# AdhavanT/ATRay

Measured on AMD Instinct MI355X. Metric: Mrays/sec on Dragon.obj 1920x1080 @ 1/2/4/8 GPU; % HBM roofline, higher is better.
Workload: dtype f32

## Files before the change

atray_amd/csrc/capi.cpp:

```cpp
#include <hip/hip_runtime.h>

#include <algorithm>
#include <chrono>
#include <cmath>
#include <cstdio>
#include <cstdlib>
#include <cstring>
#include <type_traits>
#include <fcntl.h>
#include <unistd.h>
#include <cerrno>
#include <memory>
#include <mutex>
#include <new>
#include <string>
#include <thread>
#include <vector>

#include "engine.h"
#include "host_scene.h"
#include "launch.h"
#ifdef ATR_DIAG
#include "../../include/atray_diag.h"
#endif
// ... 112 lines not shown
        std::stable_sort(out.begin(), out.end(), [&](const DBlock& a, const DBlock& b) {
            return (cplan[size_t(a.y0 / 8) * size_t(cw) + size_t(a.x0 / 8)] & kPlanClassMask) >
                   (cplan[size_t(b.y0 / 8) * size_t(cw) + size_t(b.x0 / 8)] & kPlanClassMask);
        });
    }
    for (size_t i = 0; i < out.size(); ++i) out[i].base = int32_t(i);
}

int32_t default_parse_threads() {
    const unsigned hw = std::thread::hardware_concurrency();
    return int32_t(std::max(1u, std::min(16u, hw)));
}
#ifndef ATR_MAX_BATCH_LOG2
#define ATR_MAX_BATCH_LOG2 28
#endif
#ifndef ATR_PATH_SPLIT_DEFAULT
#define ATR_PATH_SPLIT_DEFAULT 0
#endif
atr_tuning default_tuning() {
    atr_tuning t;
    std::memset(&t, 0, sizeof(t));
    t.xcd_chunk = 16;
    t.frame_rotate = 0;
    t.hybrid_a = 2;
    t.hybrid_b = 0;
    t.path_batch_log2 = 28;
    t.cluster_size = kMaxClusterSize;
    t.frame_plan = 1;
    t.path_sort_bits = 5;
    t.path_split = ATR_PATH_SPLIT_DEFAULT;
    return t;
}
constexpr int kSchedPaths = 10;
constexpr int kMaxPathBounces = 64;
constexpr int kQueueSlots = 32;
constexpr size_t kTraceBytes = 64 * 128;

}

struct atr_ctx {
    int device = 0;
    hipStream_t own_stream = nullptr;
    hipStream_t last_stream = nullptr;
    hipEvent_t ev_start = nullptr, ev_stop = nullptr, ev_last = nullptr;
    bool have_render = false;
    int32_t last_ntiles = 0;
    std::vector<DevBuf> scene_bufs;
    DScene* d_scene = nullptr;
    int64_t scene_bytes = 0;
    int32_t max_nodes = 0, max_depth = 0, nmodels = 0, max_inner = 0;
    float scene_box[6] = {0.f, 0.f, 0.f, 1.f, 1.f, 1.f};
    atr_tuning tune = default_tuning();
    int64_t nclusters = 0;
    std::vector<uint8_t> cplan;
    int32_t cplan_w = 0, cplan_h = 0;
    uint32_t cplan_gen = 0;
    static constexpr int kBlockSlots = 24;
    BlockSet blocks[kBlockSlots];
    uint64_t block_use[kBlockSlots] = {};
    uint64_t use_clock = 0;
    int32_t* d_error = nullptr;
    int ncu = 256;
    struct PathWS {
        hipStream_t stream = nullptr;
        DevBuf mem;
        int64_t cap = 0;
        int32_t levels = 0;
        int64_t sort_bins = 0;
        bool live = false;
        hipEvent_t ev = nullptr;
        uint64_t last_use = 0;
    };
    static constexpr size_t kMaxPathWS = 4;
    hipStream_t split_stream[2] = {};
    hipEvent_t split_fork = nullptr, split_join[2] = {};
    uint64_t ws_clock = 0;
    std::vector<PathWS> path_ws;
    void* tring = nullptr;
    hipEvent_t tev[kQueueSlots] = {};
    bool tused[kQueueSlots] = {};
    int tnext = 0;
    bool prog_active = false;
    std::vector<DevBuf> prog_blocks;
    std::vector<hipEvent_t> prog_ev;
    std::vector<int32_t> prog_end;
    std::vector<std::pair<hipStream_t, hipEvent_t>> stream_ev;
    int32_t wave_slots = 0;
    hipStream_t plan_side = nullptr;
    static constexpr int kAdaptSlots = 8;
    unsigned long long* adapt_info = nullptr;
    int adapt_next = 0, adapt_last = -1;
    struct PadSlot {
        DevBuf mem;
        uint64_t gen = 0;
        int32_t rows = 0;
        bool wide = false;
        float eye[kMaxFrameCams][3];
        hipEvent_t built = nullptr;
        hipStream_t built_on = nullptr;
        std::vector<std::pair<hipStream_t, hipEvent_t>> readers;
        uint64_t last_use = 0;
    };
    static constexpr int kPadSlots = 4;
    static constexpr size_t kPadMaxBytes = size_t(256) << 20;
    PadSlot pad_slot[kPadSlots];
    uint64_t pad_clock = 0, scene_gen = 0;
    bool camera_pads = true;
    bool facing_fold = true;
    bool wave_cull = true;
    struct QueryWS {
        DevBuf rays, bins;
        int64_t cap = 0, nbins = 0;
        hipEvent_t ev = nullptr;
        hipStream_t stream = nullptr;
        bool used = false;
    } query_ws;
    struct TexelWS {
        DevBuf mesh, map, aux;
    } tex_ws;
    struct ImageWS {
        DevBuf image, flags;
        hipEvent_t ev = nullptr;
        hipStream_t stream = nullptr;
        bool used = false;
    } img_ws;
    struct DenoiseWS {
        DevBuf color, guides;
        hipEvent_t ev = nullptr;
        hipStream_t stream = nullptr;
        bool used = false;
    } dn_ws;
};

namespace {

void apply_tuning(const atr_ctx* c, RenderParams& P) {
    P.xcd_chunk = c->tune.xcd_chunk;
    P.frame_rotate = 0;
    P.hyb_a = c->tune.hybrid_a;
    P.hyb_b = c->tune.hybrid_b;
    P.wave_cull = c->wave_cull ? 1 : 0;
}

int dev_upload(atr_ctx* c, const void* src, size_t bytes, void** out) {
    DevBuf b;
    b.n = bytes ? bytes : 16;
    HIPCHK(hipMalloc(&b.p, b.n));
    if (bytes) {
        const hipError_t e = hipMemcpy(b.p, src, bytes, hipMemcpyHostToDevice);
        if (e != hipSuccess) {
            (void)hipFree(b.p);
            return -(1000 + int(e));
        }
    }
    c->scene_bufs.push_back(b);
    c->scene_bytes += int64_t(b.n);
    *out = b.p;
    return ATR_OK;
}

int32_t shade_records(const HostMesh& M, std::vector<float>& shade) {
    const int32_t smooth = M.normals.empty() ? 0 : 1;
// ... 439 lines not shown
        Q.live.part = Q.live.group + cells;
        Q.live.ctl = reinterpret_cast<PathLiveCtl*>(lb + live_bytes(ws->cap) - 256);
    }
    const int occ_cam = c->tune.path_camera_occ;
    for (int64_t c0 = cbeg; c0 < cend; c0 += cells) {
        Q.cell0 = int32_t(c0);
        Q.ncells = int32_t(std::min<int64_t>(cells, cend - c0));
        if (live && (e = atr_launch_path_live(Q, s)) != hipSuccess) return e;
        if (bl > 0 && spp > 0) {
            if ((e = reset_path_batch(Q, levels, sort_bits, s)) != hipSuccess) return e;
            if ((e = live ? atr_launch_path_camera_adaptive(Q, c->ncu, s) : atr_launch_path_camera(Q, occ_cam, s)) !=
                hipSuccess)
                return e;
            if ((e = launch_bounce_levels(c, Q, bl, sort_bits, s)) != hipSuccess) return e;
        }
        if ((e = live ? atr_launch_path_resolve_adaptive(Q, s) : atr_launch_path_resolve(Q, s)) != hipSuccess) return e;
    }
    return hipEventRecord(ws->ev, s);
}

constexpr int64_t kSplitMinCells = 1024;
hipError_t launch_paths(atr_ctx* c, const RenderParams& P, hipStream_t s) {
    if (P.nblocks <= 0) return hipSuccess;
    const int64_t per_cell = 64 * std::max<int64_t>(P.cam.samples_per_pixel, 1);
    const int64_t batch = std::max<int64_t>(1, (int64_t(1) << c->tune.path_batch_log2) / per_cell);
    if (!c->tune.path_split || P.nblocks > batch || P.nblocks < kSplitMinCells || P.counters || P.block_cost ||
        P.sample_sum)
        return launch_paths_range(c, P, s, 0, P.nblocks);
    hipError_t e;
    if (!c->split_fork) {
        for (int i = 0; i < 2; ++i) {
            if ((e = hipStreamCreateWithFlags(&c->split_stream[i], hipStreamNonBlocking)) != hipSuccess) return e;
            if ((e = hipEventCreateWithFlags(&c->split_join[i], hipEventDisableTiming)) != hipSuccess) return e;
        }
        if ((e = hipEventCreateWithFlags(&c->split_fork, hipEventDisableTiming)) != hipSuccess) return e;
    }
    if ((e = hipEventRecord(c->split_fork, s)) != hipSuccess) return e;
    const int64_t half = (P.nblocks + 1) / 2;
    hipError_t r = hipSuccess;
    for (int i = 0; i < 2; ++i) {
        hipStream_t a = c->split_stream[i];
        if ((e = hipStreamWaitEvent(a, c->split_fork, 0)) != hipSuccess) return e;
        if (r == hipSuccess) r = launch_paths_range(c, P, a, i ? half : 0, i ? P.nblocks : half);
        if ((e = hipEventRecord(c->split_join[i], a)) != hipSuccess) return e;
        if ((e = hipStreamWaitEvent(s, c->split_join[i], 0)) != hipSuccess) return e;
    }
    return r;
}

hipError_t bind_pads(atr_ctx* c, RenderParams& P, int sched, hipStream_t s, atr_ctx::PadSlot** used) {
    *used = nullptr;
    P.pads = nullptr;
    P.pads_stride = 0;
    if (!c->camera_pads || c->nclusters <= 0 || c->nclusters > int64_t(1) << 30 || !atr_render_reads_pads(P, sched))
        return hipSuccess;
    const int32_t rows = P.nfcam > 0 ? P.nfcam : 1;
    if (rows > kMaxFrameCams) return hipSuccess;
    const int32_t stride = int32_t(c->nclusters);
    const bool wide = P.counters != nullptr;
    const size_t bytes = size_t(rows) * size_t(stride) * sizeof(float2_t) * (wide ? 2 : 1);
    if (bytes > atr_ctx::kPadMaxBytes) return hipSuccess;
    PadEyes eyes;
    std::memset(&eyes, 0, sizeof(eyes));
    for (int32_t f = 0; f < rows; ++f) {
        const atr_vec3& e = P.nfcam > 0 ? P.fcam[f].eye : P.cam.eye;
        eyes.e[f][0] = e.x, eyes.e[f][1] = e.y, eyes.e[f][2] = e.z;
    }
    hipError_t e;
    atr_ctx::PadSlot* sl = nullptr;
    atr_ctx::PadSlot* lru = &c->pad_slot[0];
    for (atr_ctx::PadSlot& q : c->pad_slot) {
        if (q.gen == c->scene_gen && q.rows == rows && q.wide == wide && std::memcmp(q.eye, eyes.e, sizeof(float) * 3 * size_t(rows)) == 0) {
            sl = &q;
            break;
        }
        if (q.last_use < lru->last_use) lru = &q;
    }
    if (sl) {
        if (sl->built_on != s && (e = hipStreamWaitEvent(s, sl->built, 0)) != hipSuccess) return e;
    } else {
        sl = lru;
        if (!sl->built && (e = hipEventCreateWithFlags(&sl->built, hipEventDisableTiming)) != hipSuccess) return e;
        if (sl->mem.n < bytes || !sl->mem.p) {
            if (sl->mem.p) {
                if ((e = wait_list(sl->readers)) != hipSuccess) return e;
                if ((e = hipEventSynchronize(sl->built)) != hipSuccess) return e;
                (void)hipFree(sl->mem.p);
            }
            sl->mem = DevBuf();
            sl->gen = 0;
            if (hipMalloc(&sl->mem.p, bytes) != hipSuccess) {
                (void)hipGetLastError();
                sl->mem = DevBuf();
                return hipSuccess;
            }
            sl->mem.n = bytes;
        } else {
            if (sl->gen && sl->built_on != s && (e = hipStreamWaitEvent(s, sl->built, 0)) != hipSuccess) return e;
            for (const auto& se : sl->readers)
                if (se.first != s && (e = hipStreamWaitEvent(s, se.second, 0)) != hipSuccess) return e;
        }
        sl->gen = 0;
        if ((e = atr_launch_camera_pads(c->d_scene, eyes, rows, stride, c->facing_fold, wide, static_cast<float2_t*>(sl->mem.p),
                                        nullptr, nullptr, nullptr, s)) != hipSuccess)
            return e;
        if ((e = hipEventRecord(sl->built, s)) != hipSuccess) return e;
        sl->built_on = s;
        sl->gen = c->scene_gen;
        sl->rows = rows;
        sl->wide = wide;
        std::memcpy(sl->eye, eyes.e, sizeof(eyes.e));
    }
    sl->last_use = ++c->pad_clock;
    P.pads = static_cast<const float2_t*>(sl->mem.p);
    P.pads_stride = stride;
    *used = sl;
    return hipSuccess;
}

hipError_t launch_kernels(atr_ctx* c, RenderParams& P, int sched, hipStream_t s, const PathLive* live = nullptr) {
    if (live) return launch_paths_range(c, P, s, 0, P.nblocks, live);
    if (sched == kSchedPaths) {
        hipError_t e = launch_paths(c, P, s);
        if (e != hipErrorOutOfMemory) return e;
        if (P.traced_rays && (e = hipMemsetAsync(P.traced_rays, 0, kTraceBytes, s)) != hipSuccess) return e;
        sched = sched_of(ATR_KERNEL_FLAT);
    }
    atr_ctx::PadSlot* pads = nullptr;
    hipError_t e = bind_pads(c, P, sched, s, &pads);
    if (e != hipSuccess) return e;
    e = atr_launch_render(P, sched, c->tune.primary_occ, s);
    if (e == hipSuccess && pads) e = note_stream(pads->readers, s);
    return e;
}

hipError_t launch_render(atr_ctx* c, RenderParams& P, int sched, hipStream_t s, hipEvent_t* done,
                         const PathLive* live) {
    if (done) *done = nullptr;
    if (!P.traced_rays) return launch_kernels(c, P, sched, s, live);
    int k = -1;
    unsigned long long* caller = P.traced_rays;
    hipError_t e = ring_take(c, s, k, P.traced_rays);
    if (e != hipSuccess) return e;
    e = launch_kernels(c, P, sched, s, live);
    if (e == hipSuccess) e = atr_launch_traced_finish(P.traced_rays, caller, s);
    P.traced_rays = caller;
    if (e != hipSuccess) return e;
    if ((e = ring_done(c, s, k)) != hipSuccess) return e;
    if (done) *done = c->tev[k];
    return hipSuccess;
}

}

#define ATR_ABI_CATCH                                    \
    catch (const std::bad_alloc&) { return ATR_E_NOMEM; } \
    catch (...) { return ATR_E_INVALID; }

extern "C" {

const char* atr_version(void) { return "atray-mi355x 0.2 (gfx950)"; }

int atr_mesh_parse_obj_threaded(const char* text, size_t len, int32_t threads, atr_mesh** out) try {
    if (!text || !out || threads < 0) return ATR_E_INVALID;
    if (threads == 0) threads = default_parse_threads();
    std::unique_ptr<atr_mesh> own(new (std::nothrow) atr_mesh());
    atr_mesh* m = own.get();
    if (!m) return ATR_E_NOMEM;
// ... 193 lines not shown
    put_le(d + 48, 0x000000FFu, 4);
    put_le(d + 52, 0, 4);
    std::string path;
    int fd = -1;
    for (uint32_t id = 0; id < 100 && fd < 0; ++id) {
        path = std::string(name) + "_" + std::to_string(id) + ".bmp";
        fd = ::open(path.c_str(), O_WRONLY | O_CREAT | O_EXCL, 0644);
        if (fd < 0 && errno != EEXIST) return ATR_E_IO;
    }
    if (fd < 0) return ATR_E_IO;
    bool ok = ::write(fd, hdr, sizeof(hdr)) == ssize_t(sizeof(hdr));
    const uint8_t* src = reinterpret_cast<const uint8_t*>(pixels);
    for (uint64_t off = 0; ok && off < bytes;) {
        const ssize_t w = ::write(fd, src + off, size_t(std::min<uint64_t>(bytes - off, 1ull << 30)));
        ok = w > 0;
        off += ok ? uint64_t(w) : 0;
    }
    ok = (::close(fd) == 0) && ok;
    if (!ok) return ATR_E_IO;
    if (out_path && out_cap > 0) {
        std::strncpy(out_path, path.c_str(), size_t(out_cap) - 1);
        out_path[out_cap - 1] = 0;
    }
    return ATR_OK;
} ATR_ABI_CATCH

int32_t atr_make_tiles(int32_t w, int32_t h, int32_t threads, atr_tile* out, int32_t cap) try {
    return reference_tiles(w, h, threads, out, out ? cap : 0);
} ATR_ABI_CATCH

int32_t atr_make_shard_tiles(int32_t w, int32_t h, int32_t side, int32_t rank, int32_t world, atr_tile* out,
                             int32_t cap) try {
    return shard_tiles(w, h, side, rank, world, out, out ? cap : 0);
} ATR_ABI_CATCH

int32_t atr_balance_shard_tiles(int32_t w, int32_t h, int32_t side, int32_t world, const int64_t* costs,
                                int64_t rank0_extra, int32_t* owner_out) try {
    return balance_shard_tiles(w, h, side, world, costs, rank0_extra, owner_out);
} ATR_ABI_CATCH

int atr_create(int device, atr_ctx** out) try {
    if (!out) return ATR_E_INVALID;
    int n = 0;
    HIPCHK(hipGetDeviceCount(&n));
    if (device < 0 || device >= n) return ATR_E_INVALID;
    HIPCHK(hipSetDevice(device));
    atr_ctx* c = new (std::nothrow) atr_ctx();
    if (!c) return ATR_E_NOMEM;
    struct Owner { atr_ctx* c; ~Owner() { if (c) atr_destroy(c); } } own{c};
    c->device = device;
    if (const char* v = std::getenv("ATR_CAMERA_PADS")) c->camera_pads = !(v[0] == '0' && v[1] == '\0');
    if (const char* v = std::getenv("ATR_WAVE_CULL")) c->wave_cull = !(v[0] == '0' && v[1] == '\0');
    if (const char* v = std::getenv("ATR_FACING_FOLD")) c->facing_fold = !(v[0] == '0' && v[1] == '\0');
    const int rc = [&]() -> int {
        HIPCHK(hipStreamCreateWithFlags(&c->own_stream, hipStreamNonBlocking));
        HIPCHK(hipEventCreate(&c->ev_start));
        HIPCHK(hipEventCreate(&c->ev_stop));
        HIPCHK(hipMalloc(&c->d_error, 16));
        HIPCHK(hipMemset(c->d_error, 0, 16));
        HIPCHK(hipDeviceGetAttribute(&c->ncu, hipDeviceAttributeMultiprocessorCount, device));
        HIPCHK(hipMalloc(&c->tring, kQueueSlots * kTraceBytes));
        HIPCHK(hipMemset(c->tring, 0, kQueueSlots * kTraceBytes));
        for (hipEvent_t& e : c->tev) HIPCHK(hipEventCreate(&e));
        return ATR_OK;
    }();
    if (rc != ATR_OK) return rc;
    own.c = nullptr;
    *out = c;
    return ATR_OK;
} ATR_ABI_CATCH

void atr_default_tuning(atr_tuning* out) {
    if (out) *out = default_tuning();
}

int atr_set_tuning(atr_ctx* c, const atr_tuning* t) try {
    if (!c || !t) return ATR_E_INVALID;
    if (t->xcd_chunk < 0 || t->xcd_chunk > 4096 || t->frame_rotate < 0 || t->frame_rotate > 1024 ||
        t->hybrid_a < -4096 || t->hybrid_a > 4096 || t->hybrid_b < -4096 || t->hybrid_b > 4096 ||
        t->path_batch_log2 < 12 || t->path_batch_log2 > ATR_MAX_BATCH_LOG2 || t->cluster_size < 1 || t->cluster_size > kMaxClusterSize ||
        t->frame_plan < 0 || t->frame_plan > 1 || (t->path_camera_occ != 0 && (t->path_camera_occ < 5 || t->path_camera_occ > 7)) ||
        (t->path_bounce_occ != 0 && (t->path_bounce_occ < 5 || t->path_bounce_occ > 7)) ||
        (t->primary_occ != 0 && (t->primary_occ < 6 || t->primary_occ > 8)) ||
        (t->path_sort_bits != 0 && (t->path_sort_bits < 2 || t->path_sort_bits > kMaxSortBits)) ||
        t->path_split < 0 || t->path_split > 1)
        return ATR_E_INVALID;
    for (int32_t r : t->reserved)
        if (r != 0) return ATR_E_INVALID;
    c->tune = *t;
    return ATR_OK;
} ATR_ABI_CATCH

int atr_get_tuning(atr_ctx* c, atr_tuning* out) try {
    if (!c || !out) return ATR_E_INVALID;
    *out = c->tune;
    return ATR_OK;
} ATR_ABI_CATCH

int atr_destroy(atr_ctx* c) try {
    if (!c) return ATR_E_INVALID;
    (void)hipSetDevice(c->device);
    (void)hipDeviceSynchronize();
    free_scene(c);
    for (BlockSet& b : c->blocks) {
        if (b.dev.p) (void)hipFree(b.dev.p);
        if (b.dev_tiles.p) (void)hipFree(b.dev_tiles.p);
// ... 43 lines not shown
    delete c;
    return ATR_OK;
} ATR_ABI_CATCH

int atr_scene_upload(atr_ctx* c, const atr_material* mats, int32_t nmats, const atr_model* models,
                     int32_t nmodels, const atr_sphere* spheres, int32_t nspheres, const atr_plane* planes,
                     int32_t nplanes) try {
    if (!c || !mats || nmats <= 0 || nmats > kMaxMaterials || nmodels < 0 || nmodels > kMaxModels ||
        (nmodels && !models) || nspheres < 0 || nplanes < 0 || (nspheres && !spheres) || (nplanes && !planes))
        return ATR_E_INVALID;
    for (int32_t i = 0; i < nspheres; ++i)
        if (spheres[i].material < 0 || spheres[i].material >= nmats) return ATR_E_INVALID;
    for (int32_t i = 0; i < nplanes; ++i)
        if (planes[i].material < 0 || planes[i].material >= nmats) return ATR_E_INVALID;
    for (int32_t i = 0; i < nmodels; ++i) {
        const atr_model& md = models[i];
        if (!md.mesh || md.material < 0 || md.material >= nmats) return ATR_E_INVALID;
        if (md.tree) {
            for (int32_t d : md.tree->t.depth)
                if (d >= kMaskLevels) return ATR_E_TREE_DEPTH;
        }
    }
    std::vector<PackedTree> packed(size_t(nmodels), PackedTree{});
    int64_t total_clusters = 0;
    for (int32_t i = 0; i < nmodels; ++i) {
        const atr_model& md = models[i];
        if (md.tree) {
            if (const int rc = pack_tree(md.tree->t, c->tune.cluster_size, packed[size_t(i)])) return rc;
            total_clusters += int64_t(packed[size_t(i)].nclusters);
            if (total_clusters > int64_t(UINT32_MAX)) return ATR_E_INVALID;
        } else {
            const HostMesh& M = md.mesh->m;
            for (int32_t vi : M.face_v)
                if (vi < 0 || size_t(vi) >= M.vertices.size()) return ATR_E_INVALID;
        }
    }
    HIPCHK(hipSetDevice(c->device));
    HIPCHK(wait_all(c));
    free_scene(c);
    ++c->scene_gen;
    DScene S;
    std::memset(&S, 0, sizeof(S));
    for (int32_t i = 0; i < nmats; ++i) {
        const atr_material& m = mats[i];
        S.mats[i] = DMaterial{m.emission.x, m.emission.y, m.emission.z, m.reflection.x, m.reflection.y,
                              m.reflection.z, m.scatter, 0.f};
    }
    S.nmats = nmats;
    S.nmodels = nmodels;
    c->max_nodes = 0;
    c->max_depth = 0;
    c->max_inner = 0;
    c->nclusters = 0;
    float box[6] = {INFINITY, INFINITY, INFINITY, -INFINITY, -INFINITY, -INFINITY};
    for (int32_t i = 0; i < nmodels; ++i)
        for (const V3& v : models[i].mesh->m.vertices) {
            box[0] = std::min(box[0], v.x), box[1] = std::min(box[1], v.y), box[2] = std::min(box[2], v.z);
            box[3] = std::max(box[3], v.x), box[4] = std::max(box[4], v.y), box[5] = std::max(box[5], v.z);
        }
    for (int32_t i = 0; i < nspheres; ++i) {
        const atr_sphere& sp = spheres[i];
        const float r = std::fabs(sp.radius);
        box[0] = std::min(box[0], sp.center.x - r), box[1] = std::min(box[1], sp.center.y - r);
        box[2] = std::min(box[2], sp.center.z - r), box[3] = std::max(box[3], sp.center.x + r);
        box[4] = std::max(box[4], sp.center.y + r), box[5] = std::max(box[5], sp.center.z + r);
    }
    const float unit[6] = {0.f, 0.f, 0.f, 1.f, 1.f, 1.f};
    const bool finite = std::isfinite(box[0]) && std::isfinite(box[1]) && std::isfinite(box[2]) &&
                        std::isfinite(box[3]) && std::isfinite(box[4]) && std::isfinite(box[5]);
    std::memcpy(c->scene_box, finite && box[0] <= box[3] && box[1] <= box[4] && box[2] <= box[5] ? box : unit,
                sizeof(box));
    for (int32_t i = 0; i < nmodels; ++i) {
        const atr_model& md = models[i];
        const HostMesh& M = md.mesh->m;
        DModel& dm = S.models[i];
        std::memset(&dm, 0, sizeof(dm));
        const size_t nf = M.nfaces();
        dm.nfaces = uint32_t(nf);
        dm.material = md.material;
        std::memcpy(dm.aabb, md.surrounding_aabb, sizeof(dm.aabb));
        std::vector<float> shade;
        dm.smooth = shade_records(M, shade);
        void* p = nullptr;
        int rc = dev_upload(c, shade.data(), shade.size() * sizeof(float), &p);
        if (rc) return rc;
        dm.shade = static_cast<const float*>(p);
        if (md.tree) {
            const HostTree& T = md.tree->t;
            PackedTree PT = std::move(packed[size_t(i)]);
            c->max_depth = std::max(c->max_depth, PT.max_depth);
            auto up = [&](const auto& v, auto*& dst) {
                void* q = nullptr;
                const int r = dev_upload(c, v.data(), v.size() * sizeof(v[0]), &q);
                dst = static_cast<std::remove_reference_t<decltype(dst)>>(q);
                return r;
            };
            dm.ninner = PT.ninner;
            if (dm.ninner > c->max_inner) c->max_inner = dm.ninner;
            if ((rc = up(PT.inner, dm.inner)) || (rc = up(PT.t0, dm.t0)) || (rc = up(PT.t1, dm.t1)) ||
                (rc = up(PT.t2, dm.t2)) || (rc = up(PT.tface, dm.tface)))
                return rc;
            const float4_t* clus = nullptr;
            if ((rc = up(PT.clus, clus))) return rc;
            dm.clus = clus;
            dm.cnrm = reinterpret_cast<const uint4_t*>(dm.clus + 2);
            if ((rc = up(PT.cl_range, dm.cl_range)) || (rc = up(PT.prim, dm.prim))) return rc;
            if (c->nclusters + int64_t(PT.nclusters) > int64_t(UINT32_MAX)) return ATR_E_INVALID;
            dm.cl_base = uint32_t(c->nclusters);
            dm.cl_count = uint32_t(PT.nclusters);
            c->nclusters += int64_t(PT.nclusters);
            if ((rc = up(PT.nodes, dm.nodes)) || (rc = up(PT.leaf_range, dm.leaf_range))) return rc;
            if (PT.tris.empty()) PT.tris.resize(1);
            if ((rc = up(PT.tris, dm.tris))) return rc;
            dm.has_tree = 1;
            dm.root_leaf = T.children[0] == 0;
            dm.near_ok = PT.near_ok;
            if (T.nnodes > c->max_nodes) c->max_nodes = T.nnodes;
        } else {
            std::vector<DTri> tris(nf);
            for (size_t f = 0; f < nf; ++f) {
                float v[9];
                for (int k = 0; k < 3; ++k) {
                    const int32_t vi = M.face_v[3 * f + size_t(k)];
                    if (vi < 0 || size_t(vi) >= M.vertices.size()) return ATR_E_INVALID;
                    const V3 q = M.vertices[size_t(vi)];
                    v[3 * k] = q.x; v[3 * k + 1] = q.y; v[3 * k + 2] = q.z;
                }
                tris[f] = make_tri(v, uint32_t(f));
            }
            if ((rc = dev_upload(c, tris.data(), tris.size() * sizeof(DTri), &p))) return rc;
            dm.tris = static_cast<const DTri*>(p);
            dm.has_tree = 0;
        }
    }
    {
        std::vector<DSphere> sp(size_t(nspheres) + 1);
        for (int32_t i = 0; i < nspheres; ++i)
            sp[size_t(i)] = DSphere{spheres[i].center.x, spheres[i].center.y, spheres[i].center.z,
                                    spheres[i].radius, spheres[i].material, 0, 0, 0};
        std::vector<DPlane> pl(size_t(nplanes) + 1);
        for (int32_t i = 0; i < nplanes; ++i)
            pl[size_t(i)] = DPlane{planes[i].normal.x, planes[i].normal.y, planes[i].normal.z,
                                   planes[i].distance, planes[i].material, 0, 0, 0};
        void* p = nullptr;
        int rc;
        if ((rc = dev_upload(c, sp.data(), sp.size() * sizeof(DSphere), &p))) return rc;
        S.spheres = static_cast<const DSphere*>(p);
        if ((rc = dev_upload(c, pl.data(), pl.size() * sizeof(DPlane), &p))) return rc;
        S.planes = static_cast<const DPlane*>(p);
        S.nspheres = nspheres;
        S.nplanes = nplanes;
        if ((rc = dev_upload(c, &S, sizeof(S), &p))) return rc;
        c->d_scene = static_cast<DScene*>(p);
    }
    c->nmodels = nmodels;
    return ATR_OK;
} ATR_ABI_CATCH

int atr_scene_info(atr_ctx* c, int64_t* bytes, int32_t* max_nodes, int32_t* max_depth) try {
    if (!c) return ATR_E_INVALID;
    if (bytes) *bytes = c->scene_bytes;
    if (max_nodes) *max_nodes = c->max_nodes;
// ... 650 lines not shown
    return ATR_OK;
}
}

int atr_render_start_frames(atr_ctx* c, const atr_camera* cam, const atr_tile* tiles, int32_t ntiles,
                            const atr_frame* fr, int32_t nframes, int64_t frame_stride, uint64_t seed, void* stream,
                            int32_t variant) try {
    return start_frames(c, cam, 1, tiles, ntiles, fr, nframes, frame_stride, seed, stream, variant);
} ATR_ABI_CATCH

int atr_render_start_cameras(atr_ctx* c, const atr_camera* cams, int32_t nframes, const atr_tile* tiles,
                             int32_t ntiles, const atr_frame* fr, int64_t frame_stride, uint64_t seed, void* stream,
                             int32_t variant) try {
    return start_frames(c, cams, nframes, tiles, ntiles, fr, nframes, frame_stride, seed, stream, variant);
} ATR_ABI_CATCH

#ifdef ATR_DIAG
int atr_render_wave_trace(atr_ctx* c, const atr_camera* cam, const atr_tile* tiles, int32_t ntiles,
                          uint64_t seed, int32_t variant, uint64_t* out, int64_t cap, int64_t* nblocks) try {
    if (!c || !cam || !nblocks || ntiles < 0 || (ntiles && !tiles)) return ATR_E_INVALID;
    if (!c->d_scene) return ATR_E_NOSCENE;
    HIPCHK(hipSetDevice(c->device));
    int rc = ATR_OK;
    BlockSet* bs = get_blocks(c, tiles, ntiles, cam->width, cam->height, rc);
    if (!bs) return rc;
    const size_t nb = bs->host.size();
    *nblocks = int64_t(nb);
    if (!out || cap < int64_t(3 * nb)) return ATR_OK;
    DevTmp fb;
    DevTmp tr;
    HIPCHK(hipMalloc(&fb.p, std::max<size_t>(1, size_t(bs->packed_pixels)) * 4));
    HIPCHK(hipMalloc(&tr.p, std::max<size_t>(1, 3 * nb) * sizeof(unsigned long long)));
    RenderParams P;
    std::memset(&P, 0, sizeof(P));
    P.cam = *cam;
    P.scene = c->d_scene;
    P.seed = seed;
    P.blocks = static_cast<const DBlock*>(bs->dev.p);
    P.nblocks = int32_t(nb);
    P.layout = ATR_LAYOUT_PACKED;
    P.framebuffer = static_cast<uint32_t*>(fb.p);
    P.error_flag = c->d_error;
    P.wave_trace = static_cast<unsigned long long*>(tr.p);
    apply_tuning(c, P);
    const int ts = sched_of(variant);
    HIPCHK(atr_launch_render(P, ts < 0 || ts == kSchedPaths ? 7 : ts, 0, nullptr));
    HIPCHK(hipDeviceSynchronize());
    if (nb) HIPCHK(hipMemcpy(out, tr.p, 3 * nb * sizeof(unsigned long long), hipMemcpyDeviceToHost));
    return ATR_OK;
} ATR_ABI_CATCH

#endif

constexpr int kCounterSlots = 32;
static int count_launch(atr_ctx* c, const atr_camera* cam, const atr_tile* tiles, int32_t ntiles, uint64_t seed,
                        int32_t variant, unsigned long long h[kCounterSlots]) {
    if (!c || !cam || ntiles < 0 || (ntiles && !tiles)) return ATR_E_INVALID;
    if (!c->d_scene) return ATR_E_NOSCENE;
    HIPCHK(hipSetDevice(c->device));
    int rc = ATR_OK;
    BlockSet* bs = get_blocks(c, tiles, ntiles, cam->width, cam->height, rc);
    if (!bs) return rc;
    DevTmp fb;
    DevTmp ctr;
    HIPCHK(hipMalloc(&fb.p, size_t(cam->width) * size_t(cam->height) * 4));
    HIPCHK(hipMalloc(&ctr.p, kCounterSlots * sizeof(unsigned long long)));
    HIPCHK(hipMemset(ctr.p, 0, kCounterSlots * sizeof(unsigned long long)));
    RenderParams P;
    std::memset(&P, 0, sizeof(P));
    P.cam = *cam;
    P.scene = c->d_scene;
    P.seed = seed;
    P.blocks = static_cast<const DBlock*>(bs->dev.p);
    P.nblocks = int32_t(bs->host.size());
    P.layout = ATR_LAYOUT_IMAGE;
    P.framebuffer = static_cast<uint32_t*>(fb.p);
    P.error_flag = c->d_error;
    P.counters = static_cast<unsigned long long*>(ctr.p);
    apply_tuning(c, P);
    const int sc = auto_sched(variant, *cam);
    if (sc < 0) return ATR_E_INVALID;
    HIPCHK(launch_render(c, P, sc, nullptr));
    HIPCHK(hipDeviceSynchronize());
    HIPCHK(hipMemcpy(h, ctr.p, kCounterSlots * sizeof(unsigned long long), hipMemcpyDeviceToHost));
    return ATR_OK;
}

int atr_render_counters(atr_ctx* c, const atr_camera* cam, const atr_tile* tiles, int32_t ntiles,
                        uint64_t seed, int32_t variant, int64_t out[10]) try {
    if (!out) return ATR_E_INVALID;
    unsigned long long h[kCounterSlots];
    const int rc = count_launch(c, cam, tiles, ntiles, seed, variant, h);
    if (rc != ATR_OK) return rc;
    for (int k = 0; k < 10; ++k) out[k] = int64_t(h[k]);
    return ATR_OK;
} ATR_ABI_CATCH

int atr_render_cull_counters(atr_ctx* c, const atr_camera* cam, const atr_tile* tiles, int32_t ntiles,
                             uint64_t seed, int32_t variant, int64_t out[5]) try {
    if (!out) return ATR_E_INVALID;
    unsigned long long h[kCounterSlots];
    const int rc = count_launch(c, cam, tiles, ntiles, seed, variant, h);
    if (rc != ATR_OK) return rc;
    out[4] = int64_t(h[29]);
    out[0] = int64_t(h[27]);
    out[1] = int64_t(h[28]);
    out[2] = int64_t(h[25]);
    out[3] = int64_t(h[26]);
    return ATR_OK;
} ATR_ABI_CATCH

int atr_render_fold_counters(atr_ctx* c, const atr_camera* cam, const atr_tile* tiles, int32_t ntiles,
                             uint64_t seed, int32_t variant, int64_t out[2]) try {
    if (!out) return ATR_E_INVALID;
    unsigned long long h[kCounterSlots];
    const int rc = count_launch(c, cam, tiles, ntiles, seed, variant, h);
    if (rc != ATR_OK) return rc;
    out[0] = int64_t(h[30]);
    out[1] = int64_t(h[31]);
    return ATR_OK;
} ATR_ABI_CATCH

int64_t atr_camera_pads_row(atr_ctx* c, const float eye[3], float* row, float* boxes, float* edges, int64_t cap) try {
    if (!c || !eye || cap < 0) return ATR_E_INVALID;
    if (!c->d_scene) return ATR_E_NOSCENE;
    const int64_t n = c->nclusters;
    if (n <= 0 || n > int64_t(1) << 30) return n <= 0 ? 0 : ATR_E_INVALID;
    if (!row || cap < n) return n;
    HIPCHK(hipSetDevice(c->device));
    PadEyes eyes;
    std::memset(&eyes, 0, sizeof(eyes));
    eyes.e[0][0] = eye[0], eyes.e[0][1] = eye[1], eyes.e[0][2] = eye[2];
    const size_t nn = size_t(n);
    DevTmp d_tab, d_info, d_box, d_edge, d_tab2;
    HIPCHK(hipMalloc(&d_tab.p, nn * sizeof(float2_t)));
    HIPCHK(hipMalloc(&d_info.p, nn * sizeof(float2_t)));
    HIPCHK(hipMalloc(&d_box.p, nn * 3 * sizeof(float4_t)));
    HIPCHK(hipMalloc(&d_edge.p, nn * 96 * sizeof(float)));
    HIPCHK(hipMemset(d_tab.p, 0, nn * sizeof(float2_t)));
    HIPCHK(hipMemset(d_info.p, 0, nn * sizeof(float2_t)));
    HIPCHK(hipMemset(d_box.p, 0, nn * 3 * sizeof(float4_t)));
    HIPCHK(hipMemset(d_edge.p, 0, nn * 96 * sizeof(float)));
    float2_t* const tab = static_cast<float2_t*>(d_tab.p);
    float2_t* const info = static_cast<float2_t*>(d_info.p);
    float4_t* const box = static_cast<float4_t*>(d_box.p);
    float* const edge = static_cast<float*>(d_edge.p);
    if (c->facing_fold) {
        HIPCHK(atr_launch_camera_pads(c->d_scene, eyes, 1, int32_t(n), 1, 0, tab, info, box, edge, nullptr));
    } else {
        HIPCHK(atr_launch_camera_pads(c->d_scene, eyes, 1, int32_t(n), 0, 0, tab, nullptr, nullptr, nullptr, nullptr));
        HIPCHK(hipMalloc(&d_tab2.p, nn * sizeof(float2_t)));
        HIPCHK(atr_launch_camera_pads(c->d_scene, eyes, 1, int32_t(n), 0, 0, static_cast<float2_t*>(d_tab2.p), info, box,
                                      edge, nullptr));
    }
    HIPCHK(hipDeviceSynchronize());
    std::vector<float2_t> h_tab(nn), h_info(nn);
    HIPCHK(hipMemcpy(h_tab.data(), d_tab.p, nn * sizeof(float2_t), hipMemcpyDeviceToHost));
    HIPCHK(hipMemcpy(h_info.data(), d_info.p, nn * sizeof(float2_t), hipMemcpyDeviceToHost));
    for (size_t i = 0; i < nn; ++i) {
        row[4 * i] = h_tab[i].x, row[4 * i + 1] = h_tab[i].y;
        row[4 * i + 2] = h_info[i].x, row[4 * i + 3] = h_info[i].y;
    }
    if (boxes) HIPCHK(hipMemcpy(boxes, d_box.p, nn * 3 * sizeof(float4_t), hipMemcpyDeviceToHost));
    if (edges) HIPCHK(hipMemcpy(edges, d_edge.p, nn * 96 * sizeof(float), hipMemcpyDeviceToHost));
    return n;
} ATR_ABI_CATCH

#ifdef ATR_DIAG
int atr_render_phase_clocks(atr_ctx* c, const atr_camera* cam, const atr_tile* tiles, int32_t ntiles,
                            uint64_t seed, int32_t variant, int64_t out[6]) try {
    if (!out) return ATR_E_INVALID;
    unsigned long long h[kCounterSlots];
    const int rc = count_launch(c, cam, tiles, ntiles, seed, variant, h);
// ... 750 lines not shown
```

atray_amd/csrc/cluster.h:

```cpp
#pragma once
#include "trace.h"

namespace atr {

constexpr float kTau = 3e-3f;
constexpr float kEps = 5.9604645e-8f;
constexpr float kPadRel = 36.0f * kEps, kPadAbs = 12.0f * kEps;

__device__ __forceinline__ void load_prim(const DModel& m, uint32_t k, float4_t& a0, float4_t& a1, float4_t& a2) {
    a0 = m.prim[3 * size_t(k)];
    a1 = m.prim[3 * size_t(k) + 1];
    a2 = m.prim[3 * size_t(k) + 2];
}

typedef _Float16 h2_t __attribute__((ext_vector_type(2)));

#ifndef ATR_EARLY_NRM
#define ATR_EARLY_NRM 13
#endif

struct ScreenRay {
    float ax, ay, az, sd;
    h2_t dxy, dz_lo, dz_hi;
};
// ... 79 lines not shown
    const float fx = fmaxf(fabsf(lo.x - o.x), fabsf(hi.x - o.x));
    const float fy = fmaxf(fabsf(lo.y - o.y), fabsf(hi.y - o.y));
    const float fz = fmaxf(fabsf(lo.z - o.z), fabsf(hi.z - o.z));
    const float W = (__builtin_amdgcn_sqrtf(fx * fx + fy * fy + fz * fz) + 1.0842022e-19f) * 1.0000005f + (ex + ey + ez);
    const float P = lo.w;
    const float gf = W * (P * (kPadRel / (0.9f * delta)) + kPadAbs);
    return fminf(fmaxf(gf, g.y), g.x);
}

__device__ __forceinline__ bool cluster_pads(const Ray& r, const ScreenRay& sr, float4_t lo, float4_t hi, float2_t g,
                                             float best, float& dlo, float& dhi) {
    const float gl = g.x, gt = g.y;
    const float P = lo.w;
    const float x0 = (lo.x - r.o.x) * r.inv.x, x1 = (hi.x - r.o.x) * r.inv.x;
    const float y0 = (lo.y - r.o.y) * r.inv.y, y1 = (hi.y - r.o.y) * r.inv.y;
    const float z0 = (lo.z - r.o.z) * r.inv.z, z1 = (hi.z - r.o.z) * r.inv.z;
    const float nx = fminf(x0, x1), fx1 = fmaxf(x0, x1), ny = fminf(y0, y1), fy1 = fmaxf(y0, y1),
                nz = fminf(z0, z1), fz1 = fmaxf(z0, z1);
    float tn = fmaxf(fmaxf(nx - gl * sr.ax, ny - gl * sr.ay), nz - gl * sr.az);
    float tf = fminf(fminf(fx1 + gl * sr.ax, fy1 + gl * sr.ay), fz1 + gl * sr.az);
    if (tn > tf || tf < 0.f || tn > best) return false;
    tn = fmaxf(fmaxf(nx - gt * sr.ax, ny - gt * sr.ay), nz - gt * sr.az);
    tf = fminf(fminf(fx1 + gt * sr.ax, fy1 + gt * sr.ay), fz1 + gt * sr.az);
    const bool tight = !(tn > tf || tf < 0.f || tn > best);
    const float q = hi.w;
    const float mq = sr.sd * (q * (0.51f + 511.0f * (4.8828125e-4f + 8.0f * kEps))) +
                     q * (16.0f * kEps * 511.0f + 9.5367432e-7f) + 16.0f * kEps * P;
    dlo = kTol - mq;
    dhi = tight ? __builtin_inff() : kTau + mq;
    return true;
}

struct WaveHull {
    float lx, hx, ly, hy, lz, hz;
    bool ok;
};

__device__ __forceinline__ bool cluster_hull_keep(V3 o, const WaveHull& hl, float4_t lo, float4_t hi, float gl) {
    const float ax = lo.x - o.x, bx = hi.x - o.x, ay = lo.y - o.y, by = hi.y - o.y, az = lo.z - o.z, bz = hi.z - o.z;
    const float x0 = ax * hl.lx, x1 = ax * hl.hx, x2 = bx * hl.lx, x3 = bx * hl.hx;
    const float y0 = ay * hl.ly, y1 = ay * hl.hy, y2 = by * hl.ly, y3 = by * hl.hy;
    const float z0 = az * hl.lz, z1 = az * hl.hz, z2 = bz * hl.lz, z3 = bz * hl.hz;
    const float nx = fminf(fminf(x0, x1), fminf(x2, x3)), fx = fmaxf(fmaxf(x0, x1), fmaxf(x2, x3));
    const float ny = fminf(fminf(y0, y1), fminf(y2, y3)), fy = fmaxf(fmaxf(y0, y1), fmaxf(y2, y3));
    const float nz = fminf(fminf(z0, z1), fminf(z2, z3)), fz = fmaxf(fmaxf(z0, z1), fmaxf(z2, z3));
    const float gx = gl * fmaxf(fabsf(hl.lx), fabsf(hl.hx)), gy = gl * fmaxf(fabsf(hl.ly), fabsf(hl.hy)),
                gz = gl * fmaxf(fabsf(hl.lz), fabsf(hl.hz));
    const float tn = fmaxf(fmaxf(nx - gx, ny - gy), nz - gz);
    const float tf = fminf(fminf(fx + gx, fy + gy), fz + gz);
    const bool cull = tn > tf || tf < 0.f;
    return !cull || !(fmaxf(fmaxf(gx, gy), gz) < __builtin_inff());
}

#ifndef ATR_SCREEN_TWO_CMP
__device__ __forceinline__ void screen_band(float blo, float ahi, float& mid, float& half) {
    const float lo = fmaxf(blo, -1600.0f), hi = fminf(ahi, 1600.0f);
    mid = 0.5f * (lo + hi);
    half = 0.5f * (hi - lo) * 1.000001f + (fabsf(mid) + 2048.0f) * 4.7683716e-7f;
}
__device__ __forceinline__ uint32_t screen8(const ScreenRay& sr, float nmid, float half, uint4_t a0, uint4_t a1,
                                            uint4_t z) {
    const uint32_t xy[8] = {a0.x, a0.y, a0.z, a0.w, a1.x, a1.y, a1.z, a1.w};
    const uint32_t zz[4] = {z.x, z.y, z.z, z.w};
    uint32_t gc = 0;
#pragma unroll
    for (int j = 0; j < 8; ++j) {
        const h2_t pxy = __builtin_bit_cast(h2_t, xy[j]), pz = __builtin_bit_cast(h2_t, zz[j / 2]);
        float dz;
        asm("v_dot2_f32_f16 %0, %1, %2, %3" : "=v"(dz) : "v"((j & 1) ? sr.dz_hi : sr.dz_lo), "v"(pz), "v"(nmid));
        const float e = __builtin_amdgcn_fdot2(sr.dxy, pxy, dz, false);
        if (fabsf(e) <= half) gc |= 1u << j;
    }
    return gc;
}
#else
__device__ __forceinline__ uint32_t screen8(const ScreenRay& sr, float blo, float ahi, uint4_t a0, uint4_t a1,
                                            uint4_t z) {
    const uint32_t xy[8] = {a0.x, a0.y, a0.z, a0.w, a1.x, a1.y, a1.z, a1.w};
    const uint32_t zz[4] = {z.x, z.y, z.z, z.w};
    uint32_t gc = 0;
#pragma unroll
    for (int j = 0; j < 8; ++j) {
        const h2_t pxy = __builtin_bit_cast(h2_t, xy[j]), pz = __builtin_bit_cast(h2_t, zz[j / 2]);
        float dz;
        asm("v_dot2_f32_f16 %0, %1, %2, 0" : "=v"(dz) : "v"((j & 1) ? sr.dz_hi : sr.dz_lo), "v"(pz));
        const float e = __builtin_amdgcn_fdot2(sr.dxy, pxy, dz, false);
        if (e > blo && e <= ahi) gc |= 1u << j;
    }
    return gc;
}
#endif

template <bool COUNT>
__device__ __forceinline__ size_t pads_entry(size_t c) { return COUNT ? 2 * c : c; }

template <bool COUNT, bool EARLY = true, bool PADS = false>
__device__ __forceinline__ uint32_t cluster_cands(const Ray& r, const DModel& m, uint32_t c, float4_t lo, float4_t hi,
                                                  float best, Ctr& ct, const float2_t* pads = nullptr) {
    float2_t g;
    if constexpr (PADS) g = pads[pads_entry<COUNT>(c)];
    Ray rr = r;
    asm volatile("" : "+v"(rr.d.x), "+v"(rr.d.y), "+v"(rr.d.z), "+v"(rr.inv.x), "+v"(rr.inv.y), "+v"(rr.inv.z));
    const ScreenRay sr = screen_ray(rr);
    const uint4_t* nb = m.cnrm + kClusterBlock * size_t(c);
    uint4_t e0, e1, ez;
    if constexpr (EARLY) {
        e0 = nb[0], e1 = nb[1], ez = nb[kMaxClusterSize / 4];
    }
    [[maybe_unused]] float2_t gfold;
    if constexpr (PADS && COUNT) gfold = float2_t{pads[pads_entry<COUNT>(c) + 1].x, g.y};
    if constexpr (!PADS) g = cluster_grow(r.o, lo, hi);
    float dlo, dhi;
    if (!cluster_pads(r, sr, lo, hi, g, best, dlo, dhi)) return 0;
    const uint32_t n = (__float_as_uint(lo.w) & 31u) + 1u;
    if constexpr (COUNT) ct.screen += n;
    if constexpr (PADS && COUNT) {
        float fl, fh;
        if (!cluster_pads(r, sr, lo, hi, gfold, best, fl, fh)) { ct.fold_box += 1; ct.fold_screen += n; }
    }
    const uint32_t slots = (2u << (n - 1)) - 1u;
    const float q = hi.w;
    if (!(q >= 1.1754944e-38f)) return slots;
    const float rq = __builtin_amdgcn_rcpf(q);
    const float a = -dlo * rq, b = -dhi * rq;
    const float ahi = a + fabsf(a) * 9.5367432e-7f + 1.1754944e-38f;
    const float blo = b - fabsf(b) * 9.5367432e-7f - 1.1754944e-38f;
    uint32_t cand = 0;
#ifndef ATR_SCREEN_TWO_CMP
    float mid, half;
    screen_band(blo, ahi, mid, half);
    if constexpr (EARLY) {
        cand = screen8(sr, -mid, half, e0, e1, ez);
        if (n > 8) cand |= screen8(sr, -mid, half, nb[2], nb[3], nb[kMaxClusterSize / 4 + 1]) << 8;
    } else {
        for (uint32_t g = 0; g < n; g += 8)
            cand |= screen8(sr, -mid, half, nb[g / 4], nb[g / 4 + 1], nb[kMaxClusterSize / 4 + g / 8]) << g;
    }
#else
    for (uint32_t g = 0; g < n; g += 8)
        cand |= screen8(sr, blo, ahi, nb[g / 4], nb[g / 4 + 1], nb[kMaxClusterSize / 4 + g / 8]) << g;
#endif
    return cand & slots;
}

}
```

atray_amd/csrc/engine.h:

```cpp
#pragma once
#include <math.h>
#include <stdint.h>

#include "../../include/atray.h"

#ifdef __HIPCC__
#include <hip/hip_runtime.h>
#define ATR_HD __host__ __device__ __forceinline__
#else
#define ATR_HD inline
#endif

namespace atr {

struct alignas(16) float4_t { float x, y, z, w; };
struct alignas(16) uint4_t { uint32_t x, y, z, w; };
struct alignas(8) float2_t { float x, y; };
struct alignas(8) uint2_t { uint32_t x, y; };

constexpr float kMaxFloat = 3.402823466e+38F;
constexpr float kInvU32Max = 2.328306437e-10F;
constexpr float kTol = 0.0001f;
constexpr int kMaskLevels = 16;
constexpr int kMaxMaterials = 32;
// ... 33 lines not shown
ATR_HD float rand_bi(uint64_t& state, uint64_t stream) {
    float rd = (float)pcg_next(state, stream) * kInvU32Max;
    return -1.0f + 2.0f * rd;
}
ATR_HD void path_stream(uint64_t seed, int64_t pixel, uint32_t sample, uint64_t& state, uint64_t& stream) {
    uint64_t x = seed ^ (uint64_t)pixel ^ ((uint64_t)sample << 40);
    x += 0x9E3779B97F4A7C15ULL;
    x = (x ^ (x >> 30)) * 0xBF58476D1CE4E5B9ULL;
    x = (x ^ (x >> 27)) * 0x94D049BB133111EBULL;
    state = x ^ (x >> 31);
    stream = ((uint64_t)pixel << 1) | 1ULL;
}

struct alignas(16) DNode {
    float lo_x, lo_y, lo_z, hi_x;
    float hi_y, hi_z;
    int32_t children;
    int32_t parent;
};
static_assert(sizeof(DNode) == 32, "DNode layout");

struct alignas(16) DTri {
    float ax, ay, az, abx;
    float aby, abz, acx, acy;
    float acz;
    uint32_t face;
    float pad0, pad1;
};
static_assert(sizeof(DTri) == 48, "DTri layout");

struct DModel {
    const DNode* nodes;
    const float4_t* inner;
    int32_t ninner;
    const uint32_t* leaf_range;
    const DTri* tris;
    const float4_t* t0;
    const float4_t* t1;
    const float* t2;
    const uint32_t* tface;
    const float4_t* clus;
    const uint32_t* cl_range;
    const uint4_t* cnrm;
    const float4_t* prim;
    const float* shade;
    uint32_t nfaces;
    int32_t has_tree;
    int32_t root_leaf;
    int32_t near_ok;
    int32_t smooth;
    int32_t material;
    float aabb[6];
    uint32_t cl_base, cl_count;
};

struct DMaterial { float ex, ey, ez, rx, ry, rz, scatter, pad; };
struct DSphere { float cx, cy, cz, r; int32_t material, pad0, pad1, pad2; };
struct DPlane { float nx, ny, nz, d; int32_t material, pad0, pad1, pad2; };

struct DScene {
    DMaterial mats[kMaxMaterials];
    DModel models[kMaxModels];
    int32_t nmats, nmodels, nspheres, nplanes;
    const DSphere* spheres;
    const DPlane* planes;
};

struct alignas(16) DBlock {
    int32_t x0, y0;
    uint32_t mask_lo, mask_hi;
    int32_t out_base;
    int32_t flags;
    int32_t base;
    int32_t pad;
};
static_assert(sizeof(DBlock) == 32, "DBlock layout");
constexpr int32_t kBlockPrio = 1;
constexpr int kPlanClassShift = 4;
constexpr uint8_t kPlanClassMask = 0x70, kPlanPrio = 0x80;

struct RenderParams {
    atr_camera cam;
    const DScene* scene;
    uint64_t seed;
    const DBlock* blocks;
    int32_t nblocks;
    int32_t layout;
    uint32_t* framebuffer;
    uint32_t* hit_face;
    float* hit_t;
    float* rgb;
    uint32_t* ray_casts;
    unsigned long long* traced_rays;
    int32_t* error_flag;
    unsigned long long* counters;
    unsigned long long* block_cost;
    unsigned long long* wave_trace;
    int32_t xcd_chunk;
    int32_t frame_blocks;
    int64_t frame_stride;
    int32_t frame_rotate;
    int32_t hyb_a, hyb_b;
    int32_t nfcam;
    atr_camera fcam[kMaxFrameCams];
    uint32_t first_sample;
    float* sample_sum;
    const float2_t* pads;
    int32_t pads_stride;
    int32_t wave_cull;
};

struct PadEyes {
    float e[kMaxFrameCams][3];
};

constexpr int kPathPlanes = 4;
struct PathCtl {
    uint32_t tail;
    uint32_t head;
};
#ifndef ATR_SORT_DIRS
#define ATR_SORT_DIRS 16
#endif
constexpr int kSortDirs = ATR_SORT_DIRS;
constexpr int kMaxSortBits = 7;
constexpr int64_t kSortBinsMax = int64_t(1) << 26;
constexpr int32_t kSortChunk = 4096;
static_assert((kSortDirs * kSortDirs << 6) % kSortChunk == 0, "the fewest bins (2 bits per axis) fill whole scan blocks");
static_assert((kSortBinsMax / kSortChunk) <= 32768, "path_sort_part_scan: one workgroup, 32 sums per lane");
struct PathSort {
    int32_t bits;
    int32_t nbins;
    float lo[3], sc[3];
    uint2_t* kr;
    uint32_t* perm;
    uint32_t* hist;
    uint32_t* start;
    uint32_t* part;
};

constexpr int32_t kLiveChunk = 64;
struct PathLiveCtl {
    uint32_t groups;
    uint32_t claim;
};
struct PathLive {
    uint32_t* count;
    float tolerance;
    uint2_t* mask;
    uint32_t* first;
    uint32_t* group;
    uint32_t* part;
    PathLiveCtl* ctl;
    unsigned long long* info;
};

struct PathParams {
    atr_camera cam;
    const DScene* scene;
    uint64_t seed;
    const DBlock* blocks;
    int32_t frame_blocks;
// ... 164 lines not shown
```

atray_amd/csrc/host_scene.cpp:

```cpp
#include <algorithm>
#include <cmath>
#include <cstdio>
#include <cstring>
#include <new>
#include <string>
#include <utility>
#include <vector>

#include "engine.h"
#include "host_scene.h"
#include "refs_budget.h"

using namespace atr;


void atr::mesh_aabb(const HostMesh& m, float out[6]) {
    float lo[3] = {kMaxFloat, kMaxFloat, kMaxFloat}, hi[3] = {-kMaxFloat, -kMaxFloat, -kMaxFloat};
    for (const V3& v : m.vertices) {
        const float c[3] = {v.x, v.y, v.z};
        for (int a = 0; a < 3; ++a) {
            hi[a] = pl_max(hi[a], c[a]);
            lo[a] = pl_min(lo[a], c[a]);
        }
    }
// ... 412 lines not shown
}

atr::DTri atr::make_tri(const float* v, uint32_t face) {
    DTri t;
    std::memset(&t, 0, sizeof(t));
    const V3 a = mk(v[0], v[1], v[2]), b = mk(v[3], v[4], v[5]), c = mk(v[6], v[7], v[8]);
    const V3 ab = sub(b, a), ac = sub(c, a);
    t.ax = a.x; t.ay = a.y; t.az = a.z;
    t.abx = ab.x; t.aby = ab.y; t.abz = ab.z;
    t.acx = ac.x; t.acy = ac.y; t.acz = ac.z;
    t.face = face;
    return t;
}

int atr::pack_tree(const HostTree& T, int cluster_size, PackedTree& P) {
    P = PackedTree();
    if (T.nnodes <= 0 || T.bounds.size() != 6 * size_t(T.nnodes) || T.children.size() != size_t(T.nnodes) ||
        T.parent.size() != size_t(T.nnodes) || T.depth.size() != size_t(T.nnodes) ||
        T.leaf_first.size() != size_t(T.nnodes) || T.leaf_count.size() != size_t(T.nnodes) ||
        T.prim_vertices.size() != 9 * T.prim_face.size())
        return ATR_E_INVALID;
    const size_t nprims = T.prim_face.size();
    P.nodes.resize(size_t(T.nnodes));
    std::vector<uint32_t> range(2 * size_t(T.nnodes), 0);
    for (int32_t n = 0; n < T.nnodes; ++n) {
        DNode& d = P.nodes[size_t(n)];
        const float* b = &T.bounds[6 * size_t(n)];
        d.lo_x = b[0]; d.lo_y = b[1]; d.lo_z = b[2];
        d.hi_x = b[3]; d.hi_y = b[4]; d.hi_z = b[5];
        d.children = T.children[size_t(n)];
        d.parent = T.parent[size_t(n)];
        if (!T.children[size_t(n)] && uint64_t(T.leaf_first[size_t(n)]) + T.leaf_count[size_t(n)] > nprims)
            return ATR_E_INVALID;
        range[2 * size_t(n)] = T.leaf_first[size_t(n)];
        range[2 * size_t(n) + 1] = T.children[size_t(n)] ? 0u : T.leaf_count[size_t(n)];
        P.max_depth = std::max(P.max_depth, T.depth[size_t(n)]);
    }
    std::vector<int32_t> leaf_rank;
    int rc;
    if ((rc = inner_table(T, P.inner, leaf_rank))) return rc;
    P.ninner = int32_t(P.inner.size() / 3);
    if (P.inner.empty()) P.inner.assign(3, float4_t{0.f, 0.f, 0.f, 0.f});
    auto by_rank = [&](const std::vector<uint32_t>& per_node) {
        std::vector<uint32_t> out(std::max<size_t>(2, per_node.size()), 0u);
        for (int32_t n = 0; n < T.nnodes; ++n) {
            const int32_t k = leaf_rank[size_t(n)];
            if (k < 0) continue;
            out[2 * size_t(k)] = per_node[2 * size_t(n)];
            out[2 * size_t(k) + 1] = per_node[2 * size_t(n) + 1];
        }
        return out;
    };
    P.leaf_range = by_rank(range);
    P.tris.resize(nprims);
    for (size_t k = 0; k < nprims; ++k) P.tris[k] = make_tri(&T.prim_vertices[9 * k], T.prim_face[k]);
    const size_t np = nprims ? nprims : 1;
    P.t0.assign(np, float4_t{0.f, 0.f, 0.f, 0.f});
    P.t1.assign(np, float4_t{0.f, 0.f, 0.f, 0.f});
    P.t2.assign(np, 0.f);
    P.tface.assign(np, 0u);
    for (size_t k = 0; k < nprims; ++k) {
        const DTri& t = P.tris[k];
        P.t0[k] = float4_t{t.ax, t.ay, t.az, t.abx};
        P.t1[k] = float4_t{t.aby, t.abz, t.acx, t.acy};
        P.t2[k] = t.acz;
        P.tface[k] = t.face;
    }
    LeafClusters C;
    if ((rc = leaf_clusters(T, cluster_size, C))) return rc;
    const size_t ncl = C.rec.size() / 8;
    P.nclusters = ncl;
    const size_t ns = std::max<size_t>(1, ncl) * kMaxClusterSize;
    P.prim.assign(3 * ns, float4_t{0.f, 0.f, 0.f, 0.f});
    std::vector<uint32_t> nw(std::max<size_t>(1, ncl) * kNormWords, 0u);
    for (size_t cl = 0; cl < ncl; ++cl) {
        uint32_t pw, first;
        std::memcpy(&pw, &C.rec[8 * cl + 3], 4);
        std::memcpy(&first, &C.rec[8 * cl + 7], 4);
        const uint32_t n = (pw & 31u) + 1u;
        if (n > uint32_t(kMaxClusterSize) || size_t(first) + n > C.order.size()) return ATR_E_INVALID;
        double mx = 0.0;
        for (uint32_t k = first; k < first + n; ++k)
            for (int a = 0; a < 3; ++a) mx = std::max(mx, std::fabs(double(C.normal[3 * size_t(k) + size_t(a)])));
        float q = float(mx / 511.0);
        while (double(q) * 511.0 < mx) q = std::nextafter(q, INFINITY);
        if (!(q > 0.f)) q = 1e-30f;
        C.rec[8 * cl + 7] = q;
        for (uint32_t i = 0; i < n; ++i) {
            const size_t k = first + i, slot = cl * kMaxClusterSize + i;
            if (C.order[k] >= nprims) return ATR_E_INVALID;
            const DTri& t = P.tris[C.order[k]];
            float rk, fc;
            std::memcpy(&rk, &C.rank[k], 4);
            std::memcpy(&fc, &t.face, 4);
            P.prim[3 * slot] = float4_t{t.ax, t.ay, t.az, t.abx};
            P.prim[3 * slot + 1] = float4_t{t.aby, t.abz, t.acx, t.acy};
            P.prim[3 * slot + 2] = float4_t{t.acz, rk, fc, 0.f};
            uint16_t h[3];
            for (int a = 0; a < 3; ++a) {
                const double r = double(C.normal[3 * k + size_t(a)]) / double(q);
                long v = std::isfinite(r) ? std::lround(std::max(-1e6, std::min(1e6, r))) : 0L;
                v = std::max(-511L, std::min(511L, v));
                h[a] = half_of_int(int32_t(v));
            }
            nw[kNormWords * cl + i] = uint32_t(h[0]) | (uint32_t(h[1]) << 16);
            nw[kNormWords * cl + kMaxClusterSize + i / 2] |= uint32_t(h[2]) << (16 * (i & 1));
// ... 13 lines not shown
```

atray_amd/csrc/host_scene.h:

```cpp
#pragma once
#include <cstddef>
#include <cstdint>
#include <vector>

#include "engine.h"

namespace atr {

struct HostMesh {
    std::vector<V3> vertices, normals, texcoords;
    std::vector<int32_t> face_v, face_t, face_n;
    size_t nfaces() const { return face_v.size() / 3; }
};

struct HostTree {
    int32_t nnodes = 0;
    std::vector<float> bounds;
    std::vector<int32_t> children;
    std::vector<int32_t> parent;
    std::vector<int32_t> depth;
    std::vector<uint32_t> leaf_first, leaf_count;
    std::vector<float> prim_vertices;
    std::vector<uint32_t> prim_face;
};

struct LeafClusters {
    std::vector<uint32_t> order;
    std::vector<uint32_t> rank;
    std::vector<float> rec;
    std::vector<float> normal;
    std::vector<uint32_t> range;
    float max_abs = 0.f;
};
int leaf_clusters(const HostTree& T, int size, LeafClusters& C);

int inner_table(const HostTree& T, std::vector<float4_t>& out, std::vector<int32_t>& leaf_rank);

struct PackedTree {
    std::vector<DNode> nodes;
    std::vector<uint32_t> leaf_range;
    std::vector<float4_t> inner;
    int32_t ninner = 0;
    std::vector<DTri> tris;
    std::vector<float4_t> t0, t1;
    std::vector<float> t2;
    std::vector<uint32_t> tface;
    size_t nclusters = 0;
    std::vector<uint32_t> clus;
    std::vector<uint32_t> cl_range;
    std::vector<float4_t> prim;
    int32_t max_depth = 0;
    bool near_ok = false;
};
int pack_tree(const HostTree& T, int cluster_size, PackedTree& P);
DTri make_tri(const float* v9, uint32_t face);

int parse_obj_text(const char* text, size_t len, HostMesh& m, int threads = 1);
void mesh_aabb(const HostMesh& m, float out[6]);
void mesh_translate(HostMesh& m, float box[6], V3 c);
int octree_build(const HostMesh& m, uint32_t max_faces, HostTree& T);
int octree_build_device(const HostMesh& m, uint32_t max_faces, int device, HostTree& T, float* ms_out);
int octree_finish(HostTree& T);
void octree_stats(const HostTree& T, int64_t s[7]);
void camera_set(atr_camera& cm, V3 eye, V3 facing, int32_t w, int32_t h, int32_t aa, uint32_t spp,
                int32_t bounces, float h_fov);
int32_t reference_tiles(int32_t W, int32_t H, int32_t threads, atr_tile* out, int32_t cap);
int32_t balance_shard_tiles(int32_t W, int32_t H, int32_t side, int32_t world, const int64_t* costs,
                            int64_t rank0_extra, int32_t* owner);
int32_t shard_tiles(int32_t W, int32_t H, int32_t side, int32_t rank, int32_t world, atr_tile* out,
                    int32_t cap);

}

struct atr_mesh { atr::HostMesh m; };
struct atr_octree { atr::HostTree t; };
```

atray_amd/csrc/launch.h:

```cpp
#pragma once
#include <hip/hip_runtime.h>

#include "denoise.h"
#include "engine.h"
#include "texels.h"

extern "C" {
hipError_t atr_launch_render(const atr::RenderParams& P, int sched, int primary_occ, hipStream_t s);
int atr_render_reads_pads(const atr::RenderParams& P, int sched);
hipError_t atr_launch_camera_pads(const atr::DScene* scene, const atr::PadEyes& eyes, int32_t nrows, int32_t stride,
                                  int fold, int wide, atr::float2_t* table, atr::float2_t* info, atr::float4_t* boxes,
                                  float* edges, hipStream_t s);
hipError_t atr_launch_traced_finish(unsigned long long* slots, unsigned long long* out, hipStream_t s);
hipError_t atr_launch_unpack(const atr::DBlock* blocks, int32_t nblocks, int32_t width, const uint32_t* packed,
                             uint32_t* image, hipStream_t s);
hipError_t atr_launch_tile_casts(const atr_tile* tiles, int32_t ntiles, int32_t width, const uint32_t* casts,
                                 int64_t* out, hipStream_t s);
hipError_t atr_launch_packed_tile_casts(const int32_t* slot_tile, int64_t nslots, const uint32_t* casts,
                                        int64_t frame_stride, int32_t nframes, int32_t ntiles,
                                        unsigned long long* out, hipStream_t s);
hipError_t atr_launch_path_camera(const atr::PathParams& P, int occ, hipStream_t s);
hipError_t atr_launch_path_bounce(const atr::PathParams& P, int ncu, int occ, hipStream_t s);
hipError_t atr_launch_path_resolve(const atr::PathParams& P, hipStream_t s);
hipError_t atr_launch_path_sort(const atr::PathParams& P, int ncu, hipStream_t s);
hipError_t atr_launch_path_live(const atr::PathParams& P, hipStream_t s);
hipError_t atr_launch_path_camera_adaptive(const atr::PathParams& P, int ncu, hipStream_t s);
hipError_t atr_launch_path_resolve_adaptive(const atr::PathParams& P, hipStream_t s);
hipError_t atr_launch_sort_bins(const atr::PathSort& so, hipStream_t s);
hipError_t atr_launch_query_sort(const atr::QueryParams& P, int ncu, hipStream_t s);
hipError_t atr_launch_query(const atr::QueryParams& P, int lane, int ncu, hipStream_t s);
hipError_t atr_launch_occlusion(const atr::OcclParams& P, int lane, int ncu, hipStream_t s);
hipError_t atr_launch_gather(const atr::GatherParams& P, int lane, int ncu, hipStream_t s);
hipError_t atr_launch_radiance_entry(const atr::RadianceParams& P, int ncu, hipStream_t s);
hipError_t atr_launch_radiance_resolve(const atr::RadianceParams& P, hipStream_t s);
hipError_t atr_launch_gather_radiance_entry(const atr::GatherRadianceParams& P, int ncu, hipStream_t s);
hipError_t atr_launch_gather_radiance_resolve(const atr::GatherRadianceParams& P, hipStream_t s);
hipError_t atr_launch_texel_classify(const atr::TexelParams& P, hipStream_t s);
hipError_t atr_launch_texel_big(const atr::TexelParams& P, uint32_t nbig, hipStream_t s);
hipError_t atr_launch_texel_scan(const atr::TexelParams& P, hipStream_t s);
hipError_t atr_launch_texel_write(const atr::TexelParams& P, hipStream_t s);
hipError_t atr_launch_texel_scatter(const float* values, const int32_t* texel, int64_t n, int64_t ntexels, float* image,
                                    uint8_t* flag, hipStream_t s);
hipError_t atr_launch_texel_dilate(const atr::TexelImageParams& P, hipStream_t s);
hipError_t atr_launch_texel_fill(const atr::TexelImageParams& P, hipStream_t s);
hipError_t atr_launch_denoise_pack(const atr::DenoisePack& P, hipStream_t s);
hipError_t atr_launch_denoise_pass(const atr::DenoisePass& P, int normal, int position, int colour, hipStream_t s);
hipError_t atr_launch_plan(const atr::DBlock* base, int32_t nb, unsigned long long* cost,
                           unsigned long long* cost_last, void* work, atr::DBlock* out, int32_t max_split,
                           float split2, float split4, hipStream_t s);
size_t atr_plan_work_bytes(int32_t nb);
hipError_t atr_launch_pack_bgr(const uint32_t* src, int64_t n, uint8_t* dst, hipStream_t s);
int64_t atr_masked_chunks(int64_t n);
int atr_unpack_max_sources();
hipError_t atr_launch_unpack_masked_multi(int32_t n, const atr::DBlock* const* blocks, const int32_t* nblocks,
                                          const int64_t* own, const uint8_t* const* in, const int32_t* raw,
                                          int32_t width, int32_t nframes, uint32_t* image, int64_t image_stride,
                                          hipStream_t s);
hipError_t atr_launch_unpack_masked(const atr::DBlock* blocks, int32_t nblocks, int32_t width, const uint8_t* in,
                                    int32_t nframes, int64_t own, uint32_t* image, int64_t image_stride,
                                    hipStream_t s);
hipError_t atr_launch_pack_bgr_masked(const uint32_t* src, int64_t n, uint32_t bg, uint8_t* out, int64_t* nbytes,
                                      hipStream_t s);
hipError_t atr_launch_scatter_bgr_masked(const uint8_t* in, int64_t n, const int64_t* dst_index, uint32_t* image,
                                         hipStream_t s);
hipError_t atr_launch_scatter_bgr(const uint8_t* src, int64_t n, const int64_t* dst_index, uint32_t* image,
// ... 3 lines not shown
```

atray_amd/csrc/render.hip:

```cpp
#include <hip/hip_runtime.h>

#include "launch.h"
#include "scan.h"

namespace atr {

constexpr bool sched_stash(int sc) { return sc == SCHED_FLAT || sc == SCHED_HYBRID; }

constexpr int kStash = 16;

template <int SCHED, bool COUNT>
__device__ __forceinline__ V3 cast_ray(const DScene* __restrict__ S, V3 o, V3 d, int32_t bounce_limit,
                                       bool active, uint64_t& st, uint64_t stream, uint32_t& casts,
                                       uint32_t& traced, bool record, uint32_t& hit_face, float& hit_t,
                                       int& err, Ctr& ct, int32_t hyb_a, int32_t hyb_b, V3& acc) {
    constexpr bool STASH = sched_stash(SCHED);
    constexpr bool PRIV = SCHED == SCHED_FLAT;
    __shared__ uint32_t s_stash[STASH && !PRIV ? 4 : 1][PRIV ? 1 : kStash][64];
    uint32_t pstash[PRIV ? kStash : 1];
    uint32_t* const L = &s_stash[(STASH && !PRIV) ? threadIdx.x >> 6 : 0][0][threadIdx.x & 63];
#define stash_put(k, v) do { if constexpr (PRIV) pstash[k] = (v); else L[64 * (k)] = (v); } while (0)
#define stash_get(k) (PRIV ? pstash[(PRIV ? (k) : 0)] : L[64 * (k)])
    V3 ret = mk(0.f, 0.f, 0.f), w = mk(1.f, 1.f, 1.f);
    int32_t i = 0;
// ... 61 lines not shown

template <int SCHED, bool COUNT, bool PRIMARY, int OCC = 4, bool ACCUM = false, bool PADS = false>
__global__ __launch_bounds__(256, OCC) void render_kernel(RenderParams P) {
    static_assert(!ACCUM || (SCHED == SCHED_FLAT && !PRIMARY && !COUNT), "sample passes run on FLAT");
    static_assert(!PADS || (SCHED == SCHED_HYBRID && PRIMARY), "the table serves HYBRID's primary flavour");
    const int wave = __builtin_amdgcn_readfirstlane(int(threadIdx.x >> 6)), lane = threadIdx.x & 63;
    const int b = remap_xcd(blockIdx.x, gridDim.x, P.xcd_chunk) * 4 + wave;
    if (b >= P.nblocks) return;
    const int32_t nf = P.frame_blocks > 0 ? P.nblocks / P.frame_blocks : 1;
    const int32_t fidx = b % nf;
    int32_t bi = b / nf;
    if (P.frame_rotate && nf > 1)
        bi = int32_t((int64_t(bi) + int64_t(P.frame_blocks) * fidx * P.frame_rotate / (1024 * int64_t(nf))) %
                     P.frame_blocks);
    const DBlock blk = P.blocks[bi];
    const uint64_t mask = uint64_t(blk.mask_lo) | (uint64_t(blk.mask_hi) << 32);
    const bool active = (mask >> lane) & 1;
    const int32_t x = blk.x0 + (lane & 7), y = blk.y0 + (lane >> 3);
    if (__builtin_amdgcn_readfirstlane(blk.flags) & kBlockPrio) __builtin_amdgcn_s_setprio(2);
    const uint64_t clk0 = P.block_cost ? clock64() : 0;
    uint64_t clk1 = 0;
    if constexpr (COUNT) clk1 = clock64();
#ifdef ATR_DIAG
    const uint64_t rt0 = P.wave_trace ? __builtin_amdgcn_s_memrealtime() : 0;
#endif
    const atr_camera& cm = P.nfcam > 0 ? P.fcam[__builtin_amdgcn_readfirstlane(fidx)] : P.cam;
    const DScene* S = uniform_global(P.scene);
    int err = 0;
    Ctr ct;
    uint32_t casts = 0, traced = 0, hit_face = 0xFFFFFFFFu;
    float hit_t = kMaxFloat;
    V3 col = mk(0.f, 0.f, 0.f);
    const int64_t pix = int64_t(y) * cm.width + x;
    if constexpr (ACCUM) {
        if (active && P.first_sample > 0) {
            size_t o;
            if (P.layout == ATR_LAYOUT_PACKED) o = size_t(blk.out_base) + __popcll(mask & ((uint64_t(1) << lane) - 1));
            else o = size_t(y) * size_t(cm.width) + size_t(x);
            col = mk(P.sample_sum[3 * o], P.sample_sum[3 * o + 1], P.sample_sum[3 * o + 2]);
            if (P.ray_casts) casts = P.ray_casts[o];
        }
    }
    const float film_y = -1.0f + 2.0f * (float(y) / float(cm.height));
    const float film_x = ((-1.0f + 2.0f * (float(x) / float(cm.width))) * cm.h_fov) * cm.aspect_ratio;
    const V3 eye = from(cm.eye), fc = from(cm.frame_center), cx = from(cm.camera_x), cy = from(cm.camera_y);
    V3 dir = mk(0.f, 0.f, 1.f);
    if (!cm.anti_aliasing) dir = unit(sub(add(add(fc, scale(cx, film_x)), scale(cy, film_y)), eye));
    if constexpr (PRIMARY) {
        Isect id;
        id.type = T_NONE;
        if constexpr (PADS) {
            const int32_t row = P.nfcam > 0 ? __builtin_amdgcn_readfirstlane(fidx) : 0;
            const float2_t* pads = uniform_global(P.pads) + pads_entry<COUNT>(size_t(int64_t(row) * P.pads_stride));
            intersect_scene<SCHED, FlavPrimaryPads, COUNT>(S, eye, dir, active, id, err, ct, P.hyb_a, P.hyb_b, pads,
                                                           P.wave_cull);
        } else {
            intersect_scene<SCHED, FlavPrimary, COUNT>(S, eye, dir, active, id, err, ct, P.hyb_a, P.hyb_b, nullptr,
                                                       P.wave_cull);
        }
        if (active) {
            const DMaterial& mat = S->mats[id.material];
            col = add(col, mk(mat.ex, mat.ey, mat.ez));
            hit_face = id.face;
            hit_t = id.t;
            casts = id.type == T_SKY ? 0u : 1u;
            traced = 1;
        }
    } else {
        for (uint32_t s = 0; s < cm.samples_per_pixel; ++s) {
            uint64_t st, stream;
            uint32_t fs = s;
            if constexpr (ACCUM) fs += P.first_sample;
            path_stream(P.seed, pix, fs, st, stream);
            if (cm.anti_aliasing) {
                const float xo = rand_bi(st, stream) * cm.half_pixel_width + film_x;
                const float yo = rand_bi(st, stream) * cm.half_pixel_height + film_y;
                dir = unit(sub(add(add(fc, scale(cx, xo)), scale(cy, yo)), eye));
            }
            col = add(col, cast_ray<SCHED, COUNT>(S, eye, dir, cm.bounce_limit, active, st, stream, casts, traced,
                                                 fs == 0, hit_face, hit_t, err, ct, P.hyb_a, P.hyb_b, col));
        }
    }
    DBlock ob = blk;
    __asm__ volatile("" ::: "memory");
    ob = P.blocks[bi];
    int olane = int(threadIdx.x);
    __asm__ volatile("" : "+v"(olane));
    olane &= 63;
    const uint64_t omask = uint64_t(ob.mask_lo) | (uint64_t(ob.mask_hi) << 32);
    if ((omask >> olane) & 1) {
        [[maybe_unused]] const V3 sum = col;
        if constexpr (ACCUM) col = divs(col, float(P.first_sample + cm.samples_per_pixel));
        else col = divs(col, float(cm.samples_per_pixel));
        const float cr = pl_max(0.0f, pl_min(col.x, 1.0f));
        const float cg = pl_max(0.0f, pl_min(col.y, 1.0f));
        const float cb = pl_max(0.0f, pl_min(col.z, 1.0f));
        const uint32_t r8 = uint32_t(cr * 255.0f) & 0xFFu, g8 = uint32_t(cg * 255.0f) & 0xFFu,
                       b8 = uint32_t(cb * 255.0f) & 0xFFu;
        size_t o;
        if (P.layout == ATR_LAYOUT_PACKED) o = size_t(ob.out_base) + __popcll(omask & ((uint64_t(1) << olane) - 1));
        else o = size_t(ob.y0 + (olane >> 3)) * size_t(cm.width) + size_t(ob.x0 + (olane & 7));
        o += size_t(fidx) * size_t(P.frame_stride);
        P.framebuffer[o] = b8 | (g8 << 8) | (r8 << 16);
        if (!ACCUM || P.first_sample == 0) {
            if (P.hit_face) P.hit_face[o] = hit_face;
            if (P.hit_t) P.hit_t[o] = hit_t;
        }
        if constexpr (ACCUM) { P.sample_sum[3 * o] = sum.x; P.sample_sum[3 * o + 1] = sum.y; P.sample_sum[3 * o + 2] = sum.z; }
// ... 19 lines not shown
#pragma unroll
        for (int k = 0; k < 6; ++k) {
            uint32_t t = v[k];
#pragma unroll
            for (int off = 32; off > 0; off >>= 1) t += __shfl_xor(t, off);
            if (lane == 0 && t) atomicAdd(C + 1 + k, (unsigned long long)t);
        }
        uint32_t t = traced;
#pragma unroll
        for (int off = 32; off > 0; off >>= 1) t += __shfl_xor(t, off);
        if (lane == 0) { atomicAdd(C + 0, (unsigned long long)t); atomicAdd(C + 7, 1ull); }
        uint32_t w[2] = {ct.cbox, ct.screen};
#pragma unroll
        for (int k = 0; k < 2; ++k) {
            uint32_t x2 = w[k];
#pragma unroll
            for (int off = 32; off > 0; off >>= 1) x2 += __shfl_xor(x2, off);
            if (lane == 0 && x2) atomicAdd(C + 8 + k, (unsigned long long)x2);
        }
#pragma unroll
        for (int k = 0; k < 3; ++k) {
            uint32_t a = ct.steps[k], q = ct.active[k];
#pragma unroll
            for (int off = 32; off > 0; off >>= 1) { a += __shfl_xor(a, off); q += __shfl_xor(q, off); }
            if (lane == 0 && a) atomicAdd(C + 16 + k, (unsigned long long)a);
            if (lane == 0 && q) atomicAdd(C + 19 + k, (unsigned long long)q);
        }
        {
            uint32_t e[5] = {ct.cand_wave, ct.node_wave, ct.node_lane, ct.round_wave, ct.round_items};
#pragma unroll
            for (int k = 0; k < 5; ++k) {
                uint32_t x2 = e[k];
#pragma unroll
                for (int off = 32; off > 0; off >>= 1) x2 += __shfl_xor(x2, off);
                if (lane == 0 && x2) atomicAdd(C + 22 + k, (unsigned long long)x2);
            }
        }
        if constexpr (SCHED == SCHED_HYBRID && PRIMARY) {
            if (lane == 0 && ct.culled) atomicAdd(C + 27, (unsigned long long)ct.culled);
            if (lane == 0 && ct.lp_wave) atomicAdd(C + 28, (unsigned long long)ct.lp_wave);
            uint32_t x2 = ct.ctest;
#pragma unroll
            for (int off = 32; off > 0; off >>= 1) x2 += __shfl_xor(x2, off);
            if (lane == 0 && x2) atomicAdd(C + 29, (unsigned long long)x2);
        }
        if constexpr (PADS) {
            uint32_t f[2] = {ct.fold_box, ct.fold_screen};
#pragma unroll
            for (int k = 0; k < 2; ++k) {
                uint32_t x2 = f[k];
#pragma unroll
                for (int off = 32; off > 0; off >>= 1) x2 += __shfl_xor(x2, off);
                if (lane == 0 && x2) atomicAdd(C + 30 + k, (unsigned long long)x2);
            }
        }
        if (lane == 0) {
            atomicAdd(C + 10, (unsigned long long)ct.t_pass);
            atomicAdd(C + 11, (unsigned long long)ct.t_lp);
            atomicAdd(C + 12, (unsigned long long)ct.t_deal);
            atomicAdd(C + 13, (unsigned long long)(clock64() - clk1));
            atomicAdd(C + 14, (unsigned long long)ct.t_prep);
            atomicAdd(C + 15, (unsigned long long)ct.t_scan);
        }
    }
}

template __global__ void render_kernel<SCHED_LANE, false, false>(RenderParams);
template __global__ void render_kernel<SCHED_LANE, true, false>(RenderParams);
template __global__ void render_kernel<SCHED_LANE, true, true>(RenderParams);
template __global__ void render_kernel<SCHED_LANE, false, true, 5>(RenderParams);
template __global__ void render_kernel<SCHED_HYBRID, false, true, 6>(RenderParams);
template __global__ void render_kernel<SCHED_HYBRID, false, true, 7>(RenderParams);
template __global__ void render_kernel<SCHED_HYBRID, false, true, 8>(RenderParams);
template __global__ void render_kernel<SCHED_HYBRID, false, false>(RenderParams);
template __global__ void render_kernel<SCHED_HYBRID, true, true>(RenderParams);
template __global__ void render_kernel<SCHED_HYBRID, true, false>(RenderParams);
template __global__ void render_kernel<SCHED_FLAT, false, false, 6>(RenderParams);
template __global__ void render_kernel<SCHED_FLAT, false, false, 7>(RenderParams);
template __global__ void render_kernel<SCHED_FLAT, true, false>(RenderParams);
template __global__ void render_kernel<SCHED_FLAT, false, false, 6, true>(RenderParams);
template __global__ void render_kernel<SCHED_HYBRID, false, true, 6, false, true>(RenderParams);
template __global__ void render_kernel<SCHED_HYBRID, false, true, 7, false, true>(RenderParams);
template __global__ void render_kernel<SCHED_HYBRID, false, true, 8, false, true>(RenderParams);
template __global__ void render_kernel<SCHED_HYBRID, true, true, 4, false, true>(RenderParams);

template <bool WIDE>
__global__ __launch_bounds__(256) void camera_pads_kernel(const DScene* __restrict__ S, PadEyes eyes, int32_t stride,
                                                          float2_t* __restrict__ table) {
    const uint32_t x = blockIdx.x * 256u + threadIdx.x;
    if (x >= uint32_t(stride)) return;
    const int32_t f = __builtin_amdgcn_readfirstlane(int32_t(blockIdx.y));
    const V3 eye = mk(eyes.e[f][0], eyes.e[f][1], eyes.e[f][2]);
    const int32_t nmodels = S->nmodels;
    for (int32_t i = 0; i < nmodels; ++i) {
        const DModel& m = S->models[i];
        const uint32_t c = x - m.cl_base;
        if (!m.has_tree || c >= m.cl_count) continue;
        const float2_t g = cluster_grow(eye, m.clus[kClusterBlock * size_t(c)], m.clus[kClusterBlock * size_t(c) + 1]);
        const size_t e = size_t(f) * size_t(stride) + x;
        if constexpr (WIDE) {
            table[2 * e] = g;
            table[2 * e + 1] = float2_t{g.x, kTol};
        } else {
            table[e] = g;
        }
        return;
// ... 8 lines not shown
    static_assert(kMaxClusterSize == 16, "sixteen lanes per cluster");
    const uint32_t x = blockIdx.x * 16u + (threadIdx.x >> 4), j = threadIdx.x & 15u;
    if (x >= uint32_t(stride)) return;
    const int32_t nmodels = S->nmodels;
    for (int32_t i = 0; i < nmodels; ++i) {
        const DModel& m = S->models[i];
        const uint32_t c = x - m.cl_base;
        if (!m.has_tree || c >= m.cl_count) continue;
        const float4_t lo = m.clus[kClusterBlock * size_t(c)], hi = m.clus[kClusterBlock * size_t(c) + 1];
        const uint32_t n = (__float_as_uint(lo.w) & 31u) + 1u;
        const bool have = j < n;
        float4_t a0 = {0.f, 0.f, 0.f, 0.f}, a1 = a0, a2 = a0;
        if (have) load_prim(m, kMaxClusterSize * c + j, a0, a1, a2);
        for (int32_t f = 0; f < nrows; ++f) {
            const V3 eye = mk(eyes.e[f][0], eyes.e[f][1], eyes.e[f][2]);
            const float2_t g = cluster_grow(eye, lo, hi);
            const FoldBox b = fold_box(eye, lo, hi, g.x);
            double lower = double(__builtin_inff());
            bool rej = false;
            if (have) {
                rej = fold_prim(b, lo.w, a0, a1, a2, lower);
                if (rej) lower = double(__builtin_inff());
            }
            const uint32_t mask = uint32_t(__ballot(rej) >> (threadIdx.x & 48u)) & 0xFFFFu;
#pragma unroll
            for (int off = 8; off > 0; off >>= 1) lower = fmin(lower, __shfl_xor(lower, off));
            const bool folded = fold && b.ok;
            const float delta = folded ? fold_delta(lower) : kTol;
            const float gf = cluster_grow_fold(eye, lo, hi, delta, g);
            if (j == 0) {
                const size_t e = size_t(f) * size_t(stride) + x;
                if constexpr (WIDE) {
                    table[2 * e] = g;
                    table[2 * e + 1] = float2_t{gf, delta};
                } else {
                    table[e] = float2_t{gf, g.y};
                }
                if (info) info[x] = float2_t{delta, __uint_as_float(folded ? mask : 0u)};
                if (boxes) {
                    boxes[3 * size_t(x)] = lo;
                    boxes[3 * size_t(x) + 1] = hi;
                    boxes[3 * size_t(x) + 2] = float4_t{g.x, 0.f, 0.f, 0.f};
                }
            }
        }
        if (edges) {
            float* o = edges + 6 * (size_t(kMaxClusterSize) * x + j);
            o[0] = a0.w, o[1] = a1.x, o[2] = a1.y, o[3] = a1.z, o[4] = a1.w, o[5] = a2.x;
        }
        return;
    }
}

__global__ __launch_bounds__(64) void traced_finish_kernel(unsigned long long* __restrict__ slots,
                                                          unsigned long long* __restrict__ out) {
    const int lane = threadIdx.x;
    unsigned long long v = slots[16 * lane];
    slots[16 * lane] = 0;
#pragma unroll
    for (int off = 32; off > 0; off >>= 1) v += __shfl_xor(v, off);
    if (lane == 0 && v) atomicAdd(out, v);
}

__global__ __launch_bounds__(256) void unpack_kernel(const DBlock* __restrict__ blocks, int32_t nblocks,
                                                     int32_t width, const uint32_t* __restrict__ packed,
                                                     uint32_t* __restrict__ image) {
    const int b = blockIdx.x * 4 + (threadIdx.x >> 6), lane = threadIdx.x & 63;
    if (b >= nblocks) return;
    const DBlock blk = blocks[b];
    const uint64_t mask = uint64_t(blk.mask_lo) | (uint64_t(blk.mask_hi) << 32);
    if (!((mask >> lane) & 1)) return;
    const int32_t x = blk.x0 + (lane & 7), y = blk.y0 + (lane >> 3);
    image[size_t(y) * width + x] = packed[size_t(blk.out_base) + __popcll(mask & ((uint64_t(1) << lane) - 1))];
}

__global__ __launch_bounds__(256) void tile_casts_kernel(const atr_tile* __restrict__ tiles, int32_t width,
                                                         const uint32_t* __restrict__ casts,
                                                         int64_t* __restrict__ out) {
    const atr_tile t = tiles[blockIdx.x];
    const int32_t tw = t.max_x - t.min_x + 1, th = t.max_y - t.min_y + 1;
    int64_t acc = 0;
    for (int32_t i = threadIdx.x; i < tw * th; i += blockDim.x) {
        const int32_t x = t.min_x + i % tw, y = t.min_y + i / tw;
        acc += casts[size_t(y) * width + x];
    }
    __shared__ int64_t red[256];
    red[threadIdx.x] = acc;
    __syncthreads();
    for (int s = 128; s > 0; s >>= 1) {
        if (int(threadIdx.x) < s) red[threadIdx.x] += red[threadIdx.x + s];
        __syncthreads();
    }
    if (threadIdx.x == 0) out[blockIdx.x] = red[0];
}

__global__ __launch_bounds__(256) void packed_tile_casts_kernel(const int32_t* __restrict__ slot_tile,
                                                                int64_t nslots,
                                                                const uint32_t* __restrict__ casts,
                                                                int64_t frame_stride, int32_t ntiles,
                                                                unsigned long long* __restrict__ out) {
    const int64_t i = int64_t(blockIdx.x) * 256 + threadIdx.x;
    const int64_t f = blockIdx.y;
    int32_t t = -1;
    unsigned long long v = 0;
    if (i < nslots) {
        t = slot_tile[i];
// ... 4 lines not shown
#pragma unroll
        for (int off = 32; off > 0; off >>= 1) v += __shfl_xor(v, off);
        if ((threadIdx.x & 63) == 0 && t0 >= 0 && v) atomicAdd(&out[f * ntiles + t0], v);
    } else if (t >= 0 && v) {
        atomicAdd(&out[f * ntiles + t], v);
    }
}

}

template <int SC, bool C, bool PR, int OCC = 4, bool ACCUM = false, bool PADS = false>
static void launch_one(const atr::RenderParams& P, hipStream_t s) {
    const int grid = (P.nblocks + 3) / 4;
    hipLaunchKernelGGL((atr::render_kernel<SC, C, PR, OCC, ACCUM, PADS>), dim3(grid), dim3(256), 0, s, P);
}

static void launch_hybrid_primary(const atr::RenderParams& P, int occ, hipStream_t s) {
    using namespace atr;
    if (P.pads) {
        if (occ == 0) launch_one<SCHED_HYBRID, true, true, 4, false, true>(P, s);
        else if (occ == 8) launch_one<SCHED_HYBRID, false, true, 8, false, true>(P, s);
        else if (occ == 7) launch_one<SCHED_HYBRID, false, true, 7, false, true>(P, s);
        else launch_one<SCHED_HYBRID, false, true, 6, false, true>(P, s);
    } else {
        if (occ == 0) launch_one<SCHED_HYBRID, true, true>(P, s);
        else if (occ == 8) launch_one<SCHED_HYBRID, false, true, 8>(P, s);
        else if (occ == 7) launch_one<SCHED_HYBRID, false, true, 7>(P, s);
        else launch_one<SCHED_HYBRID, false, true, 6>(P, s);
    }
}

extern "C" int atr_render_reads_pads(const atr::RenderParams& P, int sched) {
    using namespace atr;
    const bool prim = P.cam.bounce_limit == 1 && !P.cam.anti_aliasing && P.cam.samples_per_pixel == 1;
    return prim && !P.sample_sum && (sched == SCHED_HYBRID || sched == SCHED_FLAT);
}

extern "C" hipError_t atr_launch_camera_pads(const atr::DScene* scene, const atr::PadEyes& eyes, int32_t nrows,
                                             int32_t stride, int fold, int wide, atr::float2_t* table,
                                             atr::float2_t* info, atr::float4_t* boxes, float* edges, hipStream_t s) {
    using namespace atr;
    if (nrows <= 0 || stride <= 0) return hipSuccess;
    if (nrows > kMaxFrameCams) return hipErrorInvalidValue;
    const bool side = info || boxes || edges;
    if (side && nrows != 1) return hipErrorInvalidValue;
    const dim3 gf(unsigned((stride + 15) / 16)), gp(unsigned((stride + 255) / 256), unsigned(nrows));
    if (fold || side) {
        if (wide) hipLaunchKernelGGL(camera_fold_kernel<true>, gf, dim3(256), 0, s, scene, eyes, nrows, stride, fold, table, info, boxes, edges);
        else hipLaunchKernelGGL(camera_fold_kernel<false>, gf, dim3(256), 0, s, scene, eyes, nrows, stride, fold, table, info, boxes, edges);
    } else {
        if (wide) hipLaunchKernelGGL(camera_pads_kernel<true>, gp, dim3(256), 0, s, scene, eyes, stride, table);
        else hipLaunchKernelGGL(camera_pads_kernel<false>, gp, dim3(256), 0, s, scene, eyes, stride, table);
    }
    return hipGetLastError();
}

extern "C" hipError_t atr_launch_render(const atr::RenderParams& P, int sched, int primary_occ, hipStream_t s) {
    using namespace atr;
    if (P.nblocks <= 0) return hipSuccess;
    if (P.traced_rays && P.counters) return hipErrorInvalidValue;
    const bool count = P.counters != nullptr;
    const bool prim = P.cam.bounce_limit == 1 && !P.cam.anti_aliasing && P.cam.samples_per_pixel == 1;
    const bool multi = P.frame_blocks > 0;
    if (P.sample_sum) {
        if (sched != SCHED_FLAT || count || multi) return hipErrorInvalidValue;
        launch_one<SCHED_FLAT, false, false, 6, true>(P, s);
        return hipGetLastError();
    }
    const int occ = primary_occ ? primary_occ : (multi ? 7 : 8);
    const bool prim7 = occ == 7;
    const bool prim8 = occ == 8;
    switch (sched) {
        case SCHED_HYBRID:
            if (count) { if (prim) launch_hybrid_primary(P, 0, s); else launch_one<SCHED_HYBRID, true, false>(P, s); }
            else if (!prim) launch_one<SCHED_HYBRID, false, false>(P, s);
            else launch_hybrid_primary(P, prim8 ? 8 : prim7 ? 7 : 6, s);
            break;
        case SCHED_FLAT:
            if (prim && !count) launch_hybrid_primary(P, 6, s);
            else if (count) { if (prim) launch_hybrid_primary(P, 0, s); else launch_one<SCHED_FLAT, true, false>(P, s); }
            else if (multi) launch_one<SCHED_FLAT, false, false, 7>(P, s);
            else launch_one<SCHED_FLAT, false, false, 6>(P, s);
            break;
        case SCHED_LANE:
            if (count) { if (prim) launch_one<SCHED_LANE, true, true>(P, s); else launch_one<SCHED_LANE, true, false>(P, s); }
            else if (prim) launch_one<SCHED_LANE, false, true, 5>(P, s);
            else launch_one<SCHED_LANE, false, false>(P, s);
            break;
        default:
            return hipErrorInvalidValue;
    }
    return hipGetLastError();
}

extern "C" hipError_t atr_launch_traced_finish(unsigned long long* slots, unsigned long long* out, hipStream_t s) {
    hipLaunchKernelGGL(atr::traced_finish_kernel, dim3(1), dim3(64), 0, s, slots, out);
    return hipGetLastError();
}

extern "C" hipError_t atr_launch_unpack(const atr::DBlock* blocks, int32_t nblocks, int32_t width,
                                        const uint32_t* packed, uint32_t* image, hipStream_t s) {
    const int grid = (nblocks + 3) / 4;
    if (grid <= 0) return hipSuccess;
    hipLaunchKernelGGL(atr::unpack_kernel, dim3(grid), dim3(256), 0, s, blocks, nblocks, width, packed, image);
    return hipGetLastError();
}
// ... 18 lines not shown
```

atray_amd/csrc/scan.h:

```cpp
#pragma once
#include <hip/hip_runtime.h>

#include "cluster.h"
#include "shade.h"
#include "trace.h"

namespace atr {

struct TriRegs { float4_t q0, q1; float q2; };

__device__ __forceinline__ void tri_fetch(const DModel& m, uint32_t i, TriRegs& t) {
    t.q0 = m.t0[i];
    t.q1 = m.t1[i];
    t.q2 = m.t2[i];
}

__device__ __forceinline__ void tri_test(const Ray& r, const TriRegs& t, uint32_t slot, float& best_t,
                                         uint32_t& best_slot, float& bu, float& bv, bool& improved) {
    float u = 0.f, v = 0.f;
    const float dist = tri_hit(r, mk(t.q0.x, t.q0.y, t.q0.z), mk(t.q0.w, t.q1.x, t.q1.y),
                               mk(t.q1.z, t.q1.w, t.q2), u, v);
    if (dist < best_t && dist > kTol) {
        best_t = dist;
        best_slot = slot;
// ... 125 lines not shown
    const float v = ln == 0 ? hl.lx : ln == 1 ? hl.hx : ln == 2 ? hl.ly : ln == 3 ? hl.hy : ln == 4 ? hl.lz : hl.hz;
    return hl.ok || ln != 0 ? v : __builtin_nanf("");
}
__device__ __forceinline__ WaveHull hull_unpack(float hv) {
    auto at = [&](int k) { return __int_as_float(__builtin_amdgcn_readlane(__float_as_int(hv), k)); };
    WaveHull hl;
    hl.lx = at(0); hl.hx = at(1); hl.ly = at(2); hl.hy = at(3); hl.lz = at(4); hl.hz = at(5);
    hl.ok = hl.lx == hl.lx;
    return hl;
}

__device__ __forceinline__ uint32_t nth_set_bit(uint32_t x, uint32_t j) {
    uint32_t b = 0, n;
    n = uint32_t(__popc(x & 0xFFFFu)); if (j >= n) { j -= n; x >>= 16; b += 16; }
    n = uint32_t(__popc(x & 0xFFu)); if (j >= n) { j -= n; x >>= 8; b += 8; }
    n = uint32_t(__popc(x & 0xFu)); if (j >= n) { j -= n; x >>= 4; b += 4; }
    n = uint32_t(__popc(x & 0x3u)); if (j >= n) { j -= n; x >>= 2; b += 2; }
    return b + (j >= (x & 1u) ? 1u : 0u);
}

#ifdef ATR_PHASE_CLOCKS
#define ATR_PCLK(...) __VA_ARGS__
#else
#define ATR_PCLK(...)
#endif

template <bool UV>
struct FlatUV {
    float u[4][64], v[4][64];
};
template <>
struct FlatUV<false> {};
template <int K = kLeafBuf, bool UV = true>
struct FlatLds : FlatUV<UV> {
    float lbd[4][K][64];
    int32_t lbl[4][K][64];
    unsigned long long key[4][64];
    uint32_t slot[4][64];
    int32_t mark[4][64];
};
template <int K = kLeafBuf, bool UV = true>
__device__ __forceinline__ FlatLds<K, UV>& flat_lds() {
    __shared__ FlatLds<K, UV> L;
    return L;
}

constexpr unsigned long long kKeyInit = (static_cast<unsigned long long>(0x7F7FFFFFu) << 32) | 0xFFFFFFFFull;

#ifndef ATR_BOUNCE_HYB
#define ATR_BOUNCE_HYB 0
#endif

struct FlavCamera      { static constexpr bool HYB = true,  LDSB = true,  UO = true,  UT = true,  UV = true,
                         NEAR = false, PADS = false, WCULL = false, SEED = false; static constexpr int EARLY = 2; };
struct FlavPrimary     { static constexpr bool HYB = true,  LDSB = true,  UO = true,  UT = true,  UV = false,
                         NEAR = false, PADS = false, WCULL = true,  SEED = false; static constexpr int EARLY = 1; };
struct FlavPrimaryPads { static constexpr bool HYB = true,  LDSB = true,  UO = true,  UT = true,  UV = false,
                         NEAR = false, PADS = true,  WCULL = true,  SEED = false; static constexpr int EARLY = 8; };
struct FlavHybBounce   { static constexpr bool HYB = true,  LDSB = false, UO = false, UT = false, UV = true,
                         NEAR = false, PADS = false, WCULL = false, SEED = false; static constexpr int EARLY = 4; };
struct FlavBounce      { static constexpr bool HYB = ATR_BOUNCE_HYB != 0, LDSB = true, UO = false, UT = false,
                         UV = true, NEAR = true, PADS = false, WCULL = false, SEED = false;
                         static constexpr int EARLY = 4; };
struct FlavOcclusion   { static constexpr bool HYB = false, LDSB = true,  UO = false, UT = false, UV = false,
                         NEAR = true,  PADS = false, WCULL = false, SEED = true;  static constexpr int EARLY = 1; };

template <class F, bool COUNT, int K = kLeafBuf>
__device__ __forceinline__ bool cand_test(const Ray& q, const DModel& m, int w, int32_t ow, uint32_t slot,
                                          unsigned long long& mine, float& u, float& v, Ctr& ct) {
    FlatLds<K, F::UV>& L = flat_lds<K, F::UV>();
    if constexpr (COUNT) ct.tri += 1;
    float4_t a0, a1, a2;
    load_prim(m, slot, a0, a1, a2);
    const float dist = tri_hit(q, mk(a0.x, a0.y, a0.z), mk(a0.w, a1.x, a1.y), mk(a1.z, a1.w, a2.x), u, v);
    if (dist > kTol && dist < kMaxFloat) {
        mine = (static_cast<unsigned long long>(__float_as_uint(dist)) << 32) | uint32_t(__float_as_int(a2.y));
        if (mine < L.key[w][ow]) {
            atomicMin(&L.key[w][ow], mine);
            return true;
        }
    }
    return false;
}

template <class F, bool COUNT, bool SELF, int K = kLeafBuf>
__device__ __forceinline__ void cand_rounds(const Ray& r, const DModel& m, int w, int ln, uint32_t cm,
                                            uint32_t cfirst, int32_t own, Ctr& ct) {
    FlatLds<K, F::UV>& L = flat_lds<K, F::UV>();
    const uint32_t cc = uint32_t(__popc(cm));
    constexpr bool kInPlace = SELF;
#ifndef ATR_INPLACE_FACTOR
#define ATR_INPLACE_FACTOR 2
#endif
    uint32_t cinc = 0, total = 0, most;
    bool inplace;
    if (kInPlace && __ballot(cc > 1u) == 0) {
        most = __ballot(cc != 0u) ? 1u : 0u;
        inplace = true;
    } else {
        cinc = wave_incl_add(cc);
        total = uint32_t(__builtin_amdgcn_readlane(int(cinc), 63));
        most = kInPlace ? uint32_t(__builtin_amdgcn_readlane(wave_incl_max(int32_t(cc)), 63)) : 64u;
        inplace = kInPlace && most < ATR_INPLACE_FACTOR * ((total + 63u) >> 6);
    }
    if (inplace) {
        Ray q;
        q.o = r.o;
        q.d = r.d;
        uint32_t x = cm;
        for (uint32_t it = 0; it < most; ++it) {
            const bool valid = x != 0;
            const uint32_t slot = cfirst + (valid ? uint32_t(__builtin_ctz(x)) : 0u);
            x &= x - 1u;
            if constexpr (COUNT) ct.cand_wave += ln == 0 ? 1u : 0u;
            unsigned long long mine = kKeyInit;
            bool imp = false;
            float u = 0.f, v = 0.f;
            if (valid) imp = cand_test<F, COUNT, K>(q, m, w, own, slot, mine, u, v, ct);
// ... 47 lines not shown
            load_prim(m, slot, a0, a1, a2);
            const float dist = tri_hit(q, mk(a0.x, a0.y, a0.z), mk(a0.w, a1.x, a1.y), mk(a1.z, a1.w, a2.x), u, v);
            if (dist > kTol && dist < kMaxFloat) {
                mine = (static_cast<unsigned long long>(__float_as_uint(dist)) << 32) | uint32_t(__float_as_int(a2.y));
                if (mine < L.key[w][ow]) {
                    atomicMin(&L.key[w][ow], mine);
                    imp = true;
                }
            }
        }
        __builtin_amdgcn_wave_barrier();
        if (imp && L.key[w][ow] == mine) {
            L.slot[w][ow] = slot;
            if constexpr (F::UV) {
                L.u[w][ow] = u;
                L.v[w][ow] = v;
            }
        }
        __builtin_amdgcn_wave_barrier();
    }
}


struct FlatQ {
    int32_t j, nb;
    bool done, need, more, rewalk;
};

template <class F, bool COUNT, int K = kLeafBuf>
__device__ __forceinline__ FlatQ flat_begin(const Ray& r, const DModel& m, bool active, int w, int ln, Ctr& ct,
                                            unsigned long long start = kKeyInit) {
    FlatLds<K, F::UV>& L = flat_lds<K, F::UV>();
    FlatQ q{0, 0, true, false, false, false};
    if constexpr (F::SEED) L.key[w][ln] = start;
    else L.key[w][ln] = kKeyInit;
    if (active) {
        const NodeBox root = load_node(m.nodes, 0);
        if constexpr (COUNT) { ct.box += 1; ct.box_all += 1; }
        if (box_check(r, root.lx, root.ly, root.lz, root.hx, root.hy, root.hz)) {
            q.done = false;
            if (root.children == 0) {
                L.lbl[w][0][ln] = 0;
                L.lbd[w][0][ln] = 0.f;
                q.nb = 1;
            } else {
                q.need = true;
            }
        }
    }
    return q;
}

template <class F, bool COUNT, int K = kLeafBuf>
__device__ __forceinline__ void flat_pass(const Ray& r, const DModel& m, int w, int ln, FlatQ& q, int& err, Ctr& ct) {
    FlatLds<K, F::UV>& L = flat_lds<K, F::UV>();
    const float bd = q.rewalk ? L.lbd[w][K - 1][ln] : -__builtin_inff();
    const int32_t bi = q.rewalk ? L.lbl[w][K - 1][ln] : -1;
    auto took = [&](int32_t n) {
        q.need = false;
        q.j = 0;
        if (n < 0) { err = 1; q.done = true; }
        else { q.nb = n < K ? n : K; q.more = n > K; if (q.nb == 0) q.done = true; }
    };
    if constexpr (F::UT) {
        if (__ballot(q.need)) {
            LdsLeafBuf<K> lb;
            lb.d = &L.lbd[w][0][ln];
            lb.leaf = &L.lbl[w][0][ln];
            const int32_t n = traverse_pass_wave<K, COUNT>(r, m.inner, lb, bd, bi, ct, q.need);
            if (q.need) took(n);
        }
    } else if (q.need) {
        int32_t n;
        if constexpr (F::LDSB) {
            LdsLeafBuf<K> lb;
            lb.d = &L.lbd[w][0][ln];
            lb.leaf = &L.lbl[w][0][ln];
            if (F::NEAR && m.near_ok) n = traverse_pass_near<K, COUNT>(r, m.inner, lb, bd, bi, ct);
            else n = traverse_pass<K, COUNT>(r, m.inner, lb, bd, bi, ct);
        } else {
            LeafBuf<K> lb;
            n = traverse_pass<K, COUNT>(r, m.inner, lb, bd, bi, ct);
#pragma unroll
            for (int t = 0; t < K; ++t) { L.lbd[w][t][ln] = lb.d[t]; L.lbl[w][t][ln] = lb.leaf[t]; }
        }
        took(n);
    }
}

template <class F, bool COUNT, int K = kLeafBuf>
__device__ __forceinline__ void flat_leaf_step(const Ray& r, const DModel& m, int w, int ln, bool live, FlatQ& q,
                                               Ctr& ct, int32_t hyb_a, int32_t hyb_b, const float2_t* pads = nullptr,
                                               float hv = 0.f, unsigned long long start = kKeyInit) {
    static_assert(!F::PADS || F::UO, "the table holds one origin per camera");
    static_assert(!F::WCULL || (F::UO && K >= 2), "the hull is of one origin's directions; sv's LDS slot");
    constexpr bool UO = F::UO, PADS = F::PADS, WCULL = F::WCULL;
    FlatLds<K, F::UV>& L = flat_lds<K, F::UV>();
    constexpr bool kEarly = (F::EARLY & ATR_EARLY_NRM) != 0;
    ATR_PCLK(const uint64_t tc2 = clock64());
    uint32_t cf = 0, cn = 0;
    if (live) {
        const uint2_t cr = load_range(m.cl_range, L.lbl[w][q.j][ln]);
        cf = cr.x;
        cn = cr.y;
        if constexpr (COUNT) { ct.leaf += 1; ct.cbox += cn; }
    }
    [[maybe_unused]] uint32_t sv = 0xFFFFFFFFu;
    if constexpr (WCULL) {
        const WaveHull hl = hull_unpack(hv);
        if (hl.ok) {
            const bool small = live && cn > 0 && cn <= 32u;
            unsigned long long todo = __ballot(small);
            while (todo) {
                const int la = __builtin_ctzll(todo);
                const uint32_t cfa = uint32_t(__builtin_amdgcn_readlane(int(cf), la));
                const uint32_t cna = uint32_t(__builtin_amdgcn_readlane(int(cn), la));
                const bool in_a = small && cf == cfa;
                todo &= ~__ballot(in_a);
                const bool two = todo != 0;
                const int lb = two ? __builtin_ctzll(todo) : la;
                const uint32_t cfb = uint32_t(__builtin_amdgcn_readlane(int(cf), lb));
                const uint32_t cnb = two ? uint32_t(__builtin_amdgcn_readlane(int(cn), lb)) : 0u;
                const bool in_b = two && small && cf == cfb;
                todo &= ~__ballot(in_b);
                const uint32_t i = uint32_t(ln) & 31u;
                const bool hi_half = ln >= 32;
                bool keep = false;
                if (i < (hi_half ? cnb : cna)) {
                    const uint32_t c = (hi_half ? cfb : cfa) + i;
                    const float4_t lo = m.clus[kClusterBlock * size_t(c)], hi = m.clus[kClusterBlock * size_t(c) + 1];
                    float gl;
                    if constexpr (PADS) gl = pads[pads_entry<COUNT>(c)].x;
                    else gl = cluster_grow(r.o, lo, hi).x;
                    keep = cluster_hull_keep(r.o, hl, lo, hi, gl);
                }
                const unsigned long long kept = __ballot(keep);
                if (in_a) sv = uint32_t(kept);
                if (in_b) sv = uint32_t(kept >> 32);
                if constexpr (COUNT)
                    ct.culled += ln == 0 ? cna + cnb - uint32_t(__popcll(kept)) : 0u;
            }
            if (small) cn = uint32_t(__popc(sv));
        }
        L.lbd[w][0][ln] = __uint_as_float(sv);
    }
    const uint32_t incl = wave_incl_add(cn);
    const uint32_t excl = incl - cn;
    const uint32_t total = uint32_t(__builtin_amdgcn_readlane(int(incl), 63));
    if constexpr (F::SEED) { if (live) L.key[w][ln] = start; }
    else { if (live) L.key[w][ln] = kKeyInit; }
    bool deal = true;
    if constexpr (F::HYB) {
        const uint32_t mx = uint32_t(__builtin_amdgcn_readlane(wave_incl_max(int32_t(cn)), 63));
        deal = int32_t(mx) > hyb_a * int32_t((total + 63u) >> 6) + hyb_b;
    }
    ATR_PCLK(const uint64_t tc1 = clock64());
    ATR_PCLK(ct.t_prep += uint32_t(tc1 - tc2));
    if (!deal) {
        const uint32_t mxc = uint32_t(__builtin_amdgcn_readlane(wave_incl_max(int32_t(cn)), 63));
        for (uint32_t i = 0; i < mxc; ++i) {
            uint32_t cm = 0, ci = i;
            if constexpr (COUNT && WCULL) ct.lp_wave += ln == 0 ? 1u : 0u;
            if constexpr (WCULL) {
                const uint32_t left = __float_as_uint(L.lbd[w][0][ln]);
                if (left) ci = uint32_t(__builtin_ctz(left));
                L.lbd[w][0][ln] = __uint_as_float(left & (left - 1u));
                __asm__ volatile("" ::: "memory");
            }
            if (i < cn) {
                const uint32_t c = cf + ci;
                if constexpr (COUNT && WCULL) ct.ctest += 1;
                const float bound = __uint_as_float(uint32_t(L.key[w][ln] >> 32));
                cm = cluster_cands<COUNT, kEarly, PADS>(r, m, c, m.clus[kClusterBlock * size_t(c)],
                                                m.clus[kClusterBlock * size_t(c) + 1], bound, ct, pads);
            }
            cand_rounds<F, COUNT, true, K>(r, m, w, ln, cm, kMaxClusterSize * (cf + ci), ln, ct);
        }
    }
    ATR_PCLK(if (!deal) ct.t_lp += uint32_t(clock64() - tc1));
    int32_t carry = -1;
    for (uint32_t base = 0; deal && base < total; base += 64) {
        L.mark[w][ln] = -1;
        __builtin_amdgcn_wave_barrier();
        if (cn > 0 && excl >= base && excl < base + 64u) L.mark[w][excl - base] = ln;
        __builtin_amdgcn_wave_barrier();
        int32_t own = wave_incl_max(L.mark[w][ln]);
        if (own < 0) own = carry;
        carry = __builtin_amdgcn_readlane(own, 63);
        const uint32_t k = base + uint32_t(ln);
        const bool valid = k < total;
        if constexpr (COUNT) { ct.round_wave += ln == 0 ? 1u : 0u; ct.round_items += valid ? 1u : 0u; }
        const int32_t src = valid ? own : ln;
        Ray qr;
        qr.o = UO ? r.o : mk(shfl_f(r.o.x, src), shfl_f(r.o.y, src), shfl_f(r.o.z, src));
        qr.d = mk(shfl_f(r.d.x, src), shfl_f(r.d.y, src), shfl_f(r.d.z, src));
        qr.inv = mk(shfl_f(r.inv.x, src), shfl_f(r.inv.y, src), shfl_f(r.inv.z, src));
        qr.s0 = qr.inv.x < 0;
        qr.s1 = qr.inv.y < 0;
        qr.s2 = qr.inv.z < 0;
        uint32_t ci = k - uint32_t(__shfl(int(excl), src));
        if constexpr (WCULL) {
            const uint32_t os = __float_as_uint(L.lbd[w][0][src]);
            if (ci < uint32_t(__popc(os))) ci = nth_set_bit(os, ci);
        }
        const uint32_t c = uint32_t(__shfl(int(cf), src)) + ci;
        uint32_t cm = 0;
        if (valid) {
            if constexpr (COUNT && WCULL) ct.ctest += 1;
            const float bound = __uint_as_float(uint32_t(L.key[w][own] >> 32));
            cm = cluster_cands<COUNT, kEarly, PADS>(qr, m, c, m.clus[kClusterBlock * size_t(c)],
                                                    m.clus[kClusterBlock * size_t(c) + 1], bound, ct, pads);
        }
        cand_rounds<F, COUNT, false, K>(r, m, w, ln, cm, kMaxClusterSize * c, own, ct);
    }
    ATR_PCLK(if (deal) ct.t_deal += uint32_t(clock64() - tc1));
    if (live) {
        bool improved;
        if constexpr (F::SEED) improved = L.key[w][ln] != start;
        else improved = L.key[w][ln] != kKeyInit;
        if (improved) {
            q.done = true;
        } else if (++q.j >= q.nb) {
            if (q.more) q.need = q.rewalk = true;
            else q.done = true;
        }
    }
    __builtin_amdgcn_wave_barrier();
}

template <class F, bool COUNT, int K = kLeafBuf>
__device__ __forceinline__ void flat_result(const DModel& m, bool active, int w, int ln, Hit& h) {
    FlatLds<K, F::UV>& L = flat_lds<K, F::UV>();
    h.t = kMaxFloat;
    h.face = 0;
    h.u = h.v = 0.f;
    const unsigned long long key = L.key[w][ln];
    if (active && key != kKeyInit) {
        h.t = __uint_as_float(uint32_t(key >> 32));
        if constexpr (F::UV) {
            h.u = L.u[w][ln];
            h.v = L.v[w][ln];
        }
        h.face = __float_as_uint(m.prim[3 * size_t(L.slot[w][ln]) + 2].z);
    }
}

template <class F, bool COUNT, int K = kLeafBuf>
__device__ __forceinline__ void flat_query(const Ray& r, const DModel& m, bool active, int w, int ln, int& err, Ctr& ct,
                                           int32_t hyb_a = 0, int32_t hyb_b = 0, const float2_t* pads = nullptr,
                                           int32_t wcull = 0, unsigned long long start = kKeyInit) {
    FlatQ q = flat_begin<F, COUNT, K>(r, m, active, w, ln, ct, start);
    [[maybe_unused]] float hv = __builtin_nanf("");
    if constexpr (F::WCULL) {
        if (wcull) hv = hull_pack(wave_hull(r, !q.done), ln);
    }
    for (;;) {
        ATR_PCLK(uint64_t tc0 = 0; if constexpr (!F::SEED) tc0 = clock64());
        flat_pass<F, COUNT, K>(r, m, w, ln, q, err, ct);
        ATR_PCLK(if constexpr (!F::SEED) ct.t_pass += uint32_t(clock64() - tc0));
        if (__ballot(!q.done) == 0) break;
        flat_leaf_step<F, COUNT, K>(r, m, w, ln, !q.done, q, ct, hyb_a, hyb_b, pads, hv, start);
    }
}

enum { SCHED_LANE = 0, SCHED_FLAT = 6, SCHED_HYBRID = 7 };

__device__ __forceinline__ DModel uniform_model(const DModel& src) {
    DModel m = src;
    m.nodes = uniform_global(m.nodes);
    m.inner = uniform_global(m.inner);
    m.leaf_range = uniform_global(m.leaf_range);
    m.tris = uniform_global(m.tris);
    m.t0 = uniform_global(m.t0);
    m.t1 = uniform_global(m.t1);
    m.t2 = uniform_global(m.t2);
    m.tface = uniform_global(m.tface);
    m.clus = uniform_global(m.clus);
    m.cl_range = uniform_global(m.cl_range);
    m.cnrm = uniform_global(m.cnrm);
    m.prim = uniform_global(m.prim);
    return m;
}

struct SceneHit {
    float best, fu, fv;
    uint32_t face;
    int32_t nm;
};

template <int SCHED, class F, bool COUNT, int KB = kLeafBuf>
__device__ __forceinline__ SceneHit intersect_models(const DScene* __restrict__ S, V3 o, V3 d, bool active, int& err,
                                                    Ctr& ct, int32_t hyb_a, int32_t hyb_b,
                                                    const float2_t* pads = nullptr, int32_t wcull = 0) {
    const Ray r = make_ray(o, d);
    SceneHit sh{kMaxFloat, 0.f, 0.f, 0u, -1};
    const int32_t nmodels = __builtin_amdgcn_readfirstlane(S->nmodels);
    for (int32_t i = 0; i < nmodels; ++i) {
        const DModel m = uniform_model(S->models[i]);
        if (m.has_tree) {
            Hit h;
            if constexpr (SCHED == SCHED_LANE) {
                if (active) tree_closest_lane<COUNT>(r, m, h, err, ct);
                else h.t = kMaxFloat;
            } else {
                const float2_t* mp = pads;
                if constexpr (F::PADS) mp = pads + pads_entry<COUNT>(__builtin_amdgcn_readfirstlane(m.cl_base));
                const int w = threadIdx.x >> 6, ln = threadIdx.x & 63;
                ATR_PCLK(uint64_t tcs = clock64());
                flat_query<F, COUNT, KB>(r, m, active, w, ln, err, ct, hyb_a, hyb_b, mp, wcull);
                flat_result<F, COUNT, KB>(m, active, w, ln, h);
                ATR_PCLK(ct.t_scan += uint32_t(clock64() - tcs));
            }
            if (h.t > kTol && h.t < sh.best) { sh.best = h.t; sh.face = h.face; sh.fu = h.u; sh.fv = h.v; sh.nm = i; }
        } else if (active) {
            if constexpr (COUNT) { ct.box += 1; ct.box_all += 1; }
            if (box_entry(r, m.aabb[0], m.aabb[1], m.aabb[2], m.aabb[3], m.aabb[4], m.aabb[5]) != 0) {
                if constexpr (COUNT) { ct.tri += m.nfaces; }
                for (uint32_t j = 0; j < m.nfaces; ++j) {
                    const DTri* t = m.tris + j;
                    float u = 0.f, v = 0.f;
                    const float tt = tri_hit(r, mk(t->ax, t->ay, t->az), mk(t->abx, t->aby, t->abz),
                                             mk(t->acx, t->acy, t->acz), u, v);
                    if (tt > kTol && tt < sh.best) { sh.best = tt; sh.fu = u; sh.fv = v; sh.face = j; sh.nm = i; }
                }
            }
        }
    }
    return sh;
}

template <int SCHED, class F, bool COUNT>
__device__ __forceinline__ void intersect_scene(const DScene* __restrict__ S, V3 o, V3 d, bool active, Isect& id,
                                                int& err, Ctr& ct, int32_t hyb_a, int32_t hyb_b,
                                                const float2_t* pads = nullptr, int32_t wcull = 0) {
    const SceneHit sh = intersect_models<SCHED, F, COUNT>(S, o, d, active, err, ct, hyb_a, hyb_b, pads, wcull);
    if (!active) return;
    scene_finish(S, o, d, sh.best, sh.face, sh.fu, sh.fv, sh.nm, id);
}

__device__ __forceinline__ void bounce_shade(const DMaterial& mat, const Isect& id, V3& o, V3& d, V3& ret, V3& w,
                                             uint64_t& st, uint64_t stream) {
    const V3 emission = mk(mat.ex, mat.ey, mat.ez);
    float att = dot(neg(d), id.normal);
    V3 n = id.normal;
    if (att < 0) { n = neg(n); att = 0; }
    V3 pure = sub(d, scale(n, (2 * dot(d, n))));
    pure = unit(pure);
    const float r0 = rand_bi(st, stream);
    const float r1 = rand_bi(st, stream);
    const float r2 = rand_bi(st, stream);
    V3 rnd = add(mk(r0, r1, r2), n);
    rnd = unit(rnd);
    o = add(o, scale(d, id.t));
    d = unit(lerp3(rnd, pure, mat.scatter));
    ret = add(ret, had(w, emission));
    w = had(w, scale(mk(mat.rx, mat.ry, mat.rz), att));
}

__device__ __forceinline__ int remap_xcd(int wg, int nwg, int chunk) {
    const int x = wg % 8;
    if (chunk > 0) {
        const int span = 8 * chunk, full = (nwg / span) * span;
        if (wg >= full) return wg;
        const int j = wg / 8;
        return ((j / chunk) * 8 + x) * chunk + j % chunk;
    }
    const int q = nwg / 8, rm = nwg % 8;
    return (x < rm ? x * (q + 1) : rm * (q + 1) + (x - rm) * q) + wg / 8;
}

__device__ __forceinline__ void add_traced(unsigned long long* slots, uint32_t t, int spread) {
#pragma unroll
    for (int off = 32; off > 0; off >>= 1) t += __shfl_xor(t, off);
    if ((threadIdx.x & 63) == 0 && t) atomicAdd(slots + 16 * (spread & 63), (unsigned long long)t);
}

}
```

atray_amd/csrc/trace.h:

```cpp
#pragma once
#include "engine.h"

namespace atr {

struct Ctr {
    uint32_t box = 0, box_all = 0, tri = 0, leaf = 0, wave_tri = 0, pass = 0;
    uint32_t cbox = 0, screen = 0;
    uint32_t t_pass = 0, t_lp = 0, t_deal = 0, t_prep = 0, t_scan = 0;
    uint32_t steps[3] = {0, 0, 0}, active[3] = {0, 0, 0};
    uint32_t cand_wave = 0, node_wave = 0, node_lane = 0, round_wave = 0, round_items = 0;
    uint32_t culled = 0, lp_wave = 0, ctest = 0;
    uint32_t fold_box = 0, fold_screen = 0;
};

__device__ __forceinline__ uint32_t first_active_lane() {
    return (threadIdx.x & 63) == uint32_t(__builtin_ctzll(__ballot(1))) ? 1u : 0u;
}

template <class T>
__device__ __forceinline__ T* as_global(T* p) {
    using G = __attribute__((address_space(1))) T;
    return (T*)(reinterpret_cast<G*>(reinterpret_cast<uint64_t>(p)));
}
template <class T>
__device__ __forceinline__ T* uniform_global(T* p) {
    const uint64_t v = reinterpret_cast<uint64_t>(p);
    const uint32_t lo = __builtin_amdgcn_readfirstlane(uint32_t(v)), hi = __builtin_amdgcn_readfirstlane(uint32_t(v >> 32));
    using G = __attribute__((address_space(1))) T;
    return (T*)(reinterpret_cast<G*>((uint64_t(hi) << 32) | lo));
}

struct Ray {
    V3 o, d, inv;
    int s0, s1, s2;
};

__device__ __forceinline__ Ray make_ray(V3 o, V3 d) {
    Ray r;
    r.o = o;
    r.d = d;
    r.inv = mk(1 / d.x, 1 / d.y, 1 / d.z);
    r.s0 = r.inv.x < 0;
    r.s1 = r.inv.y < 0;
    r.s2 = r.inv.z < 0;
    return r;
}

struct NodeBox { float lx, ly, lz, hx, hy, hz; int32_t children, parent; };

__device__ __forceinline__ NodeBox load_node(const DNode* __restrict__ nodes, int32_t i) {
    const float4* p = reinterpret_cast<const float4*>(nodes + i);
    const float4 a = p[0], b = p[1];
    NodeBox n;
    n.lx = a.x; n.ly = a.y; n.lz = a.z; n.hx = a.w;
    n.hy = b.x; n.hz = b.y;
    n.children = __float_as_int(b.z);
    n.parent = __float_as_int(b.w);
    return n;
}

__device__ __forceinline__ bool box_check(const Ray& r, float lx, float ly, float lz, float hx,
                                          float hy, float hz) {
    float tmin = ((r.s0 ? hx : lx) - r.o.x) * r.inv.x;
    float tmax = ((r.s0 ? lx : hx) - r.o.x) * r.inv.x;
    const float tymin = ((r.s1 ? hy : ly) - r.o.y) * r.inv.y;
// ... 188 lines not shown
    if (b.n == K) b.thr = b.d[64 * (K - 1)];
}

template <int K>
__device__ __forceinline__ int32_t lb_leaf(const LeafBuf<K>& b, int j) {
    int32_t r = b.leaf[0];
#pragma unroll
    for (int q = 1; q < K; ++q) r = (j == q) ? b.leaf[q] : r;
    return r;
}

struct Inner {
    float lx, ly, lz, vx, vy, vz, hx, hy, hz;
    int32_t leaf0;
    int32_t parent;
    uint32_t bm;
};

__device__ __forceinline__ Inner load_inner(const float4_t* __restrict__ tab, int32_t i) {
    const float4_t a = tab[3 * i], b = tab[3 * i + 1], c = tab[3 * i + 2];
    Inner n;
    n.lx = a.x; n.ly = a.y; n.lz = a.z; n.vx = a.w;
    n.vy = b.x; n.vz = b.y; n.hx = b.z; n.hy = b.w;
    n.hz = c.x;
    n.leaf0 = __float_as_int(c.y);
    n.parent = __float_as_int(c.z);
    n.bm = __float_as_uint(c.w);
    return n;
}

typedef uint32_t u32x8_t __attribute__((ext_vector_type(8)));
typedef uint32_t u32x4_t __attribute__((ext_vector_type(4)));
__device__ __forceinline__ Inner load_inner_uniform(const float4_t* __restrict__ tab, int32_t i) {
    const uint64_t a64 = reinterpret_cast<uint64_t>(tab + 3 * i);
    const uint64_t u64 = uint64_t(uint32_t(__builtin_amdgcn_readfirstlane(int32_t(uint32_t(a64))))) |
                         (uint64_t(uint32_t(__builtin_amdgcn_readfirstlane(int32_t(uint32_t(a64 >> 32))))) << 32);
    const float4_t* p = reinterpret_cast<const float4_t*>(u64);
    u32x8_t a;
    u32x4_t c;
    asm volatile("s_load_dwordx8 %0, %2, 0x0\n\ts_load_dwordx4 %1, %2, 0x20\n\ts_waitcnt lgkmcnt(0)"
                 : "=&s"(a), "=&s"(c)
                 : "s"(p));
    Inner n;
    n.lx = __uint_as_float(a[0]); n.ly = __uint_as_float(a[1]); n.lz = __uint_as_float(a[2]);
    n.vx = __uint_as_float(a[3]); n.vy = __uint_as_float(a[4]); n.vz = __uint_as_float(a[5]);
    n.hx = __uint_as_float(a[6]); n.hy = __uint_as_float(a[7]);
    n.hz = __uint_as_float(c[0]);
    n.leaf0 = int32_t(c[1]);
    n.parent = int32_t(c[2]);
    n.bm = c[3];
    return n;
}

template <int K, bool COUNT, class LB>
__device__ __forceinline__ uint32_t examine_inner(const Ray& r, const Inner& n, LB& lb,
                                                  int32_t& ncand, float bd, int32_t bi, Ctr& ct,
                                                  bool first_pass, bool cull = false) {
    const float X0 = (n.lx - r.o.x) * r.inv.x, X1 = (n.vx - r.o.x) * r.inv.x, X2 = (n.hx - r.o.x) * r.inv.x;
    const float Y0 = (n.ly - r.o.y) * r.inv.y, Y1 = (n.vy - r.o.y) * r.inv.y, Y2 = (n.hy - r.o.y) * r.inv.y;
    const float Z0 = (n.lz - r.o.z) * r.inv.z, Z1 = (n.vz - r.o.z) * r.inv.z, Z2 = (n.hz - r.o.z) * r.inv.z;
    const float nx0 = r.s0 ? X1 : X0, nx1 = r.s0 ? X2 : X1, fx0 = r.s0 ? X0 : X1, fx1 = r.s0 ? X1 : X2;
    const float ny0 = r.s1 ? Y1 : Y0, ny1 = r.s1 ? Y2 : Y1, fy0 = r.s1 ? Y0 : Y1, fy1 = r.s1 ? Y1 : Y2;
    const float nz0 = r.s2 ? Z1 : Z0, nz1 = r.s2 ? Z2 : Z1, fz0 = r.s2 ? Z0 : Z1, fz1 = r.s2 ? Z1 : Z2;
    uint32_t mask = 0;
    int nodes_hit = 0;
#pragma unroll
    for (int i = 0; i < 8; ++i) {
        if (nodes_hit > 4) break;
        if constexpr (COUNT) { ct.box_all += 1; ct.box += first_pass ? 1u : 0u; }
        float tmin = (i >> 2) ? nx1 : nx0, tmax = (i >> 2) ? fx1 : fx0;
        const float tymin = ((i >> 1) & 1) ? ny1 : ny0, tymax = ((i >> 1) & 1) ? fy1 : fy0;
        const float tzmin = (i & 1) ? nz1 : nz0, tzmax = (i & 1) ? fz1 : fz0;
        bool in = !((tmin > tymax) || (tymin > tmax));
        if (tymin > tmin) tmin = tymin;
        if (tymax < tmax) tmax = tymax;
        in = in && !((tmin > tzmax) || (tzmin > tmax));
        if (!((n.bm >> i) & 1u)) {
            if (in) {
                ++nodes_hit;
                const float tx = tzmax < tmax ? tzmax : tmax;
                const bool behind = (!COUNT || !first_pass) && tx <= 0.0f;
                if (!(cull && (behind || tx < bd))) mask |= 1u << i;
            }
        } else {
            if (tzmin > tmin) tmin = tzmin;
            if (tzmax < tmax) tmax = tzmax;
            const float dis = !in ? 0.0f : (tmin > 0 ? tmin : (tmax > 0 ? tmax : 0.0f));
            if (dis > 0.0f) {
                ++nodes_hit;
                const int32_t id = n.leaf0 + __popc(n.bm & ((1u << i) - 1u) & 0xFFu);
                if (dis > bd || (dis == bd && id > bi)) {
                    ++ncand;
                    lb_insert<K>(lb, dis, id);
                }
            }
        }
    }
    return mask;
}

template <int K, bool COUNT, class LB>
__device__ __forceinline__ int32_t traverse_pass(const Ray& r, const float4_t* __restrict__ tab,
                                                 LB& lb, float bd, int32_t bi, Ctr& ct) {
    const bool first_pass = bi < 0;
    if constexpr (COUNT) ct.pass += 1;
    lb_clear<K>(lb);
    int32_t ncand = 0;
#ifdef ATR_NO_CULL
    const bool cull = false;
#else
    const bool cull = isfinite(r.inv.x) && isfinite(r.inv.y) && isfinite(r.inv.z);
#endif
    Inner cur = load_inner(tab, 0);
    uint64_t lo = examine_inner<K, COUNT>(r, cur, lb, ncand, bd, bi, ct, first_pass, cull);
    uint64_t hi = 0;
    uint32_t bm = cur.bm;
    int32_t parent = -1, lvl = 0;
    for (;;) {
        if constexpr (COUNT) { ct.node_wave += first_active_lane(); ct.node_lane += 1; }
        const uint32_t m = lvl < 8 ? uint32_t(lo >> (8 * lvl)) & 0xFFu : uint32_t(hi >> (8 * (lvl - 8))) & 0xFFu;
        if (m) {
            const int s = 31 - __clz(m);
            if (lvl < 8) lo &= ~(uint64_t(1) << (8 * lvl + s));
            else hi &= ~(uint64_t(1) << (8 * (lvl - 8) + s));
            const uint32_t innerm = ~bm & ((1u << s) - 1u);
            const int32_t id = int32_t(bm >> 8) + __popc(innerm);
            cur = load_inner(tab, id);
            const uint64_t cm = examine_inner<K, COUNT>(r, cur, lb, ncand, bd, bi, ct, first_pass, cull);
            ++lvl;
            if (lvl >= kMaskLevels) return -1;
            if (lvl < 8) lo |= cm << (8 * lvl);
            else hi |= cm << (8 * (lvl - 8));
            bm = cur.bm;
            parent = cur.parent;
        } else {
            if (lvl == 0) break;
            --lvl;
            const float4_t t = tab[3 * parent + 2];
            bm = __float_as_uint(t.w);
            parent = __float_as_int(t.z);
        }
    }
    return ncand;
}
// ... 53 lines not shown

constexpr int kNearLevels = 8;
template <int K, bool COUNT>
__device__ __forceinline__ int32_t traverse_pass_near(const Ray& r, const float4_t* __restrict__ tab,
                                                      LdsLeafBuf<K>& lb, float bd, int32_t bi, Ctr& ct) {
    const bool first_pass = bi < 0;
    if constexpr (COUNT) ct.pass += 1;
    lb_clear<K>(lb);
    int32_t ncand = 0;
    const bool cull = isfinite(r.inv.x) && isfinite(r.inv.y) && isfinite(r.inv.z);
    const uint32_t sm = (uint32_t(r.s0) << 2) | (uint32_t(r.s1) << 1) | uint32_t(r.s2);
    bool skipped = false;
    Inner cur = load_inner(tab, 0);
    const uint32_t m0 = examine_near<K, COUNT>(r, cur, lb, ncand, bd, bi, ct, first_pass, cull, sm, skipped);
    uint64_t s0 = m0 ? uint64_t(m0 | ((cur.bm & 0xFFu) << 8) | ((cur.bm >> 8) << 16)) : 0, s1 = 0, s2 = 0, s3 = 0;
    int32_t depth = m0 ? 1 : 0;
    for (;;) {
        while (depth > 0 && (uint32_t(s0) & 0xFFu) == 0) {
            s0 = (s0 >> 32) | (s1 << 32);
            s1 = (s1 >> 32) | (s2 << 32);
            s2 = (s2 >> 32) | (s3 << 32);
            s3 >>= 32;
            --depth;
        }
        if (depth == 0) break;
        if constexpr (COUNT) { ct.node_wave += first_active_lane(); ct.node_lane += 1; }
        const uint32_t top = uint32_t(s0);
        const int sb = __builtin_ctz(top & 0xFFu);
        s0 &= ~uint64_t(1u << sb);
        const int s = sb ^ int(sm);
        const uint32_t innerm = ~(top >> 8) & ((1u << s) - 1u) & 0xFFu;
        const int32_t id = int32_t(top >> 16) + __popc(innerm);
        cur = load_inner(tab, id);
        if (cull && lb.n == K) {
            const float ex = r.s0 ? (cur.hx - r.o.x) * r.inv.x : (cur.lx - r.o.x) * r.inv.x;
            const float ey = r.s1 ? (cur.hy - r.o.y) * r.inv.y : (cur.ly - r.o.y) * r.inv.y;
            const float ez = r.s2 ? (cur.hz - r.o.z) * r.inv.z : (cur.lz - r.o.z) * r.inv.z;
            const float txy = ey > ex ? ey : ex;
            if ((ez > txy ? ez : txy) > lb.thr) { skipped = true; continue; }
        }
        const uint32_t cm = examine_near<K, COUNT>(r, cur, lb, ncand, bd, bi, ct, first_pass, cull, sm, skipped);
        if (cm) {
            if (depth >= kNearLevels) return -1;
            s3 = (s3 << 32) | (s2 >> 32);
            s2 = (s2 << 32) | (s1 >> 32);
            s1 = (s1 << 32) | (s0 >> 32);
            s0 = (s0 << 32) | uint64_t(cm | ((cur.bm & 0xFFu) << 8) | ((cur.bm >> 8) << 16));
            ++depth;
        }
    }
    return skipped && ncand <= K ? K + 1 : ncand;
}

template <int K, bool COUNT, class LB>
__device__ __forceinline__ int32_t traverse_pass_wave(const Ray& r, const float4_t* __restrict__ tab, LB& lb,
                                                      float bd, int32_t bi, Ctr& ct, bool part) {
    const bool first_pass = bi < 0;
    if constexpr (COUNT) { if (part) ct.pass += 1; }
    if (part) lb_clear<K>(lb);
    int32_t ncand = 0;
#ifdef ATR_NO_CULL
    const bool cull = false;
#else
    const bool cull = isfinite(r.inv.x) && isfinite(r.inv.y) && isfinite(r.inv.z);
#endif
    Inner cur = load_inner_uniform(tab, 0);
    uint64_t lo = part ? uint64_t(examine_inner<K, COUNT>(r, cur, lb, ncand, bd, bi, ct, first_pass, cull)) : 0;
    uint64_t hi = 0;
    uint32_t bm = cur.bm;
    int32_t parent = -1, lvl = 0;
    for (;;) {
        if constexpr (COUNT) { ct.node_wave += (threadIdx.x & 63) == 0 ? 1u : 0u; ct.node_lane += part ? 1u : 0u; }
        const uint32_t mine = lvl < 8 ? uint32_t(lo >> (8 * lvl)) & 0xFFu : uint32_t(hi >> (8 * (lvl - 8))) & 0xFFu;
        int s = -1;
        for (int b = 7; b >= 0; --b)
            if (__ballot((mine >> b) & 1u)) { s = b; break; }
        if (s >= 0) {
            const bool act = (mine >> s) & 1u;
            if (lvl < 8) lo &= ~(uint64_t(1) << (8 * lvl + s));
            else hi &= ~(uint64_t(1) << (8 * (lvl - 8) + s));
            const uint32_t innerm = ~bm & ((1u << s) - 1u);
            const int32_t id = int32_t(bm >> 8) + __popc(innerm);
            cur = load_inner_uniform(tab, id);
            const uint64_t cm = act ? uint64_t(examine_inner<K, COUNT>(r, cur, lb, ncand, bd, bi, ct, first_pass, cull)) : 0;
            ++lvl;
            if (lvl >= kMaskLevels) return -1;
            if (lvl < 8) lo |= cm << (8 * lvl);
            else hi |= cm << (8 * (lvl - 8));
            bm = cur.bm;
            parent = cur.parent;
        } else {
            if (lvl == 0) break;
            --lvl;
            const Inner p = load_inner_uniform(tab, parent);
            bm = p.bm;
            parent = p.parent;
        }
    }
    return part ? ncand : 0;
}

}
```

atray_amd/engine.py:

```python
from __future__ import annotations

import ctypes as C
import os

import numpy as np

HERE = os.path.dirname(os.path.abspath(__file__))
LIB_PATH = os.environ.get("ATRAY_LIB") or os.path.join(HERE, "_lib", "libatray_hip.so")

ATR_LAYOUT_IMAGE = 0
ATR_LAYOUT_PACKED = 1
ATR_PLAN_PRIO = 0x80


def plan_class(c):
    return (int(c) & 7) << 4
ATR_KERNEL_AUTO, ATR_KERNEL_LANE = 0, 1
ATR_KERNEL_FLAT = 8
ATR_KERNEL_HYBRID = 9
ATR_KERNEL_PATHS = 10
VARIANTS = (ATR_KERNEL_LANE, ATR_KERNEL_FLAT, ATR_KERNEL_HYBRID, ATR_KERNEL_PATHS)
MISS = 0xFFFFFFFF
ATR_SAMPLES_CONVERGED = 0x80000000
MAX_FLOAT = np.float32(3.402823466e38)
# ... 72 lines not shown
class atr_radiance_out(C.Structure):
    _fields_ = [("rgb", C.c_void_p), ("sum", C.c_void_p), ("ray_casts", C.c_void_p), ("invalid", C.c_void_p),
                ("traced_rays", C.c_void_p)]


class atr_gather_radiance_out(C.Structure):
    _fields_ = [("rgb", C.c_void_p), ("sum", C.c_void_p), ("samples", C.c_void_p), ("ray_casts", C.c_void_p),
                ("invalid", C.c_void_p), ("sample_rgb", C.c_void_p), ("dirs", C.c_void_p),
                ("traced_rays", C.c_void_p)]


class atr_texels_out(C.Structure):
    _fields_ = [("slot", C.c_void_p), ("texel", C.c_void_p), ("face", C.c_void_p), ("bary", C.c_void_p),
                ("point", C.c_void_p), ("normal", C.c_void_p)]


class atr_denoise_params(C.Structure):
    _fields_ = [("passes", C.c_int32), ("sigma_color", C.c_float), ("sigma_position", C.c_float),
                ("normal_power_log2", C.c_int32), ("reserved", C.c_int32 * 4)]


class atr_denoise_guides(C.Structure):
    _fields_ = [("normal", C.c_void_p), ("position", C.c_void_p), ("ident", C.c_void_p)]


class atr_tuning(C.Structure):
    _fields_ = [("xcd_chunk", C.c_int32), ("frame_rotate", C.c_int32), ("hybrid_a", C.c_int32),
                ("hybrid_b", C.c_int32), ("path_batch_log2", C.c_int32), ("cluster_size", C.c_int32),
                ("frame_plan", C.c_int32), ("path_camera_occ", C.c_int32), ("path_bounce_occ", C.c_int32),
                ("primary_occ", C.c_int32), ("path_sort_bits", C.c_int32), ("path_split", C.c_int32),
                ("reserved", C.c_int32 * 4)]


EXPORTS = [
    "atr_mesh_load_obj", "atr_mesh_parse_obj", "atr_mesh_from_arrays", "atr_mesh_free",
    "atr_mesh_info", "atr_mesh_aabb", "atr_mesh_translate_to", "atr_octree_build", "atr_octree_build_device",
    "atr_octree_from_nodes", "atr_octree_free", "atr_octree_export", "atr_octree_stats", "atr_camera_set",
    "atr_make_tiles", "atr_make_shard_tiles", "atr_create", "atr_destroy", "atr_version",
    "atr_scene_upload", "atr_scene_info", "atr_render_start", "atr_render_start_ex",
    "atr_render_counters", "atr_render_tile_costs", "atr_balance_shard_tiles",
    "atr_render_packed_size", "atr_packed_pixel_map", "atr_unpack", "atr_tile_ray_casts", "atr_render_wait",
    "atr_last_kernel_ms", "atr_device_alloc", "atr_device_free", "atr_memcpy_d2h", "atr_memcpy_h2d",
    "atr_memset_d", "atr_render_start_progressive", "atr_write_bmp", "atr_render_start_frames",
    "atr_render_start_cameras", "atr_mesh_load_obj_threaded", "atr_mesh_parse_obj_threaded",
    "atr_mesh_export", "atr_packed_tile_ray_casts", "atr_set_cell_plan", "atr_render_cell_costs",
    "atr_default_tuning", "atr_set_tuning", "atr_get_tuning", "atr_pack_bgr", "atr_scatter_bgr",
    "atr_pack_bgr_masked_bound", "atr_pack_bgr_masked", "atr_scatter_bgr_masked", "atr_unpack_masked",
    "atr_unpack_masked_ranks",
    "atr_render_plan_info", "atr_workspace_info", "atr_render_start_samples",
    "atr_render_start_adaptive", "atr_render_adaptive_info", "atr_render_cull_counters",
    "atr_trace_rays", "atr_occluded_rays", "atr_gather_occlusion", "atr_gather_directions",
    "atr_radiance_rays", "atr_gather_radiance", "atr_mesh_texels", "atr_texels_to_image",
    "atr_render_fold_counters", "atr_camera_pads_row", "atr_default_denoise_params", "atr_denoise",
]
DIAG_EXPORTS = ["atr_render_wave_trace", "atr_render_phase_clocks", "atr_render_path_counters",
                "atr_render_simd_counters"]

_lib = None


def lib():
    global _lib
    if _lib is not None:
        return _lib
    import torch
    if not os.path.exists(LIB_PATH):
        raise ImportError(f"atray HIP engine not built: {LIB_PATH} missing "
                          "(run __graft_entry__.build())")
    L = C.CDLL(LIB_PATH)
    P, vp, i32, u32, i64 = C.POINTER, C.c_void_p, C.c_int32, C.c_uint32, C.c_int64
    sig = {
        "atr_mesh_load_obj": ([C.c_char_p, P(vp)], C.c_int),
        "atr_mesh_parse_obj": ([C.c_char_p, C.c_size_t, P(vp)], C.c_int),
        "atr_mesh_load_obj_threaded": ([C.c_char_p, i32, P(vp)], C.c_int),
        "atr_mesh_parse_obj_threaded": ([C.c_char_p, C.c_size_t, i32, P(vp)], C.c_int),
        "atr_mesh_from_arrays": ([vp, u32, vp, u32, vp, u32, vp, P(vp)], C.c_int),
        "atr_mesh_free": ([vp], None),
        "atr_mesh_info": ([vp, P(u32), P(u32), P(u32)], C.c_int),
        "atr_mesh_export": ([vp, vp, vp, vp, P(u32), vp, vp, vp], C.c_int),
        "atr_mesh_aabb": ([vp, C.c_float * 6], C.c_int),
        "atr_mesh_translate_to": ([vp, C.c_float * 6, atr_vec3], C.c_int),
        "atr_octree_build": ([vp, u32, P(vp)], C.c_int),
        "atr_octree_build_device": ([vp, u32, i32, P(vp), vp], C.c_int),
        "atr_octree_from_nodes": ([i32, vp, vp, vp, vp, u32, vp, vp, P(vp)], C.c_int),
        "atr_octree_free": ([vp], None),
        "atr_octree_export": ([vp, vp, vp, vp, vp, vp, vp], C.c_int),
        "atr_octree_stats": ([vp, i64 * 7], C.c_int),
        "atr_camera_set": ([P(atr_camera), atr_vec3, atr_vec3, i32, i32, i32, u32, i32, C.c_float], C.c_int),
        "atr_make_tiles": ([i32, i32, i32, vp, i32], i32),
        "atr_make_shard_tiles": ([i32, i32, i32, i32, i32, vp, i32], i32),
        "atr_balance_shard_tiles": ([i32, i32, i32, i32, vp, i64, vp], i32),
        "atr_create": ([C.c_int, P(vp)], C.c_int),
        "atr_destroy": ([vp], C.c_int),
        "atr_version": ([], C.c_char_p),
        "atr_scene_upload": ([vp, vp, i32, vp, i32, vp, i32, vp, i32], C.c_int),
        "atr_scene_info": ([vp, P(i64), P(i32), P(i32)], C.c_int),
        "atr_workspace_info": ([vp, P(i32), P(i64)], C.c_int),
        "atr_render_start": ([vp, P(atr_camera), vp, i32, P(atr_frame), C.c_uint64, vp], C.c_int),
        "atr_render_start_ex": ([vp, P(atr_camera), vp, i32, P(atr_frame), C.c_uint64, vp, i32], C.c_int),
        "atr_render_start_samples": ([vp, P(atr_camera), vp, i32, P(atr_frame), C.c_uint64, vp, i32, u32, vp],
                                     C.c_int),
        "atr_render_start_adaptive": ([vp, P(atr_camera), vp, i32, P(atr_frame), C.c_uint64, vp, i32, u32, vp, vp,
                                       C.c_float], C.c_int),
        "atr_render_adaptive_info": ([vp, i64 * 4], C.c_int),
        "atr_trace_rays": ([vp, vp, vp, i64, P(atr_ray_hits), i32, i32, vp], C.c_int),
        "atr_occluded_rays": ([vp, vp, vp, vp, i64, vp, vp, i32, i32, vp], C.c_int),
        "atr_gather_occlusion": ([vp, vp, vp, vp, i64, i32, u32, i64, C.c_uint64, P(atr_gather_out), i32, vp],
                                 C.c_int),
        "atr_gather_directions": ([vp, i64, i32, u32, i64, C.c_uint64, vp, vp], C.c_int),
        "atr_radiance_rays": ([vp, vp, vp, i64, i32, u32, i64, i32, C.c_uint64, P(atr_radiance_out), i32, vp],
                              C.c_int),
        "atr_gather_radiance": ([vp, vp, vp, i64, i32, u32, i64, i32, C.c_uint64, P(atr_gather_radiance_out), i32,
                                 vp], C.c_int),
        "atr_mesh_texels": ([vp, vp, i32, i32, i32, i64, P(atr_texels_out), P(i64), vp], C.c_int),
        "atr_texels_to_image": ([vp, vp, vp, i64, i32, i32, i32, C.c_float * 3, vp, vp], C.c_int),
        "atr_default_denoise_params": ([P(atr_denoise_params)], None),
        "atr_denoise": ([vp, vp, P(atr_denoise_guides), i32, i32, P(atr_denoise_params), vp, vp, vp], C.c_int),
        "atr_render_packed_size": ([vp, i32], i64),
        "atr_render_counters": ([vp, P(atr_camera), vp, i32, C.c_uint64, i32, i64 * 10], C.c_int),
        "atr_render_cull_counters": ([vp, P(atr_camera), vp, i32, C.c_uint64, i32, i64 * 5], C.c_int),
        "atr_render_fold_counters": ([vp, P(atr_camera), vp, i32, C.c_uint64, i32, i64 * 2], C.c_int),
        "atr_camera_pads_row": ([vp, C.c_float * 3, vp, vp, vp, i64], i64),
        "atr_render_tile_costs": ([vp, P(atr_camera), vp, i32, C.c_uint64, vp], C.c_int),
        "atr_render_wave_trace": ([vp, P(atr_camera), vp, i32, C.c_uint64, i32, vp, i64, P(i64)], C.c_int),
        "atr_packed_pixel_map": ([vp, i32, i32, i32, vp, i64], i64),
        "atr_unpack": ([vp, vp, i32, i32, vp, vp, vp], C.c_int),
        "atr_tile_ray_casts": ([vp, vp, i32, i32, vp, vp, vp], C.c_int),
        "atr_packed_tile_ray_casts": ([vp, vp, i32, i32, i32, vp, i32, i64, vp, vp], C.c_int),
        "atr_set_cell_plan": ([vp, i32, i32, vp], C.c_int),
        "atr_render_phase_clocks": ([vp, P(atr_camera), vp, i32, C.c_uint64, i32, vp], C.c_int),
        "atr_default_tuning": ([P(atr_tuning)], None),
        "atr_set_tuning": ([vp, P(atr_tuning)], C.c_int),
        "atr_get_tuning": ([vp, P(atr_tuning)], C.c_int),
        "atr_pack_bgr": ([vp, vp, i64, vp, vp], C.c_int),
        "atr_render_plan_info": ([vp, vp, i32, i32, i32, vp, vp, i64, vp, P(i64)], C.c_int),
        "atr_scatter_bgr": ([vp, vp, i64, vp, vp, vp], C.c_int),
        "atr_pack_bgr_masked_bound": ([i64], i64),
        "atr_pack_bgr_masked": ([vp, vp, i64, u32, vp, vp, vp], C.c_int),
        "atr_scatter_bgr_masked": ([vp, vp, i64, vp, vp, vp], C.c_int),
        "atr_unpack_masked": ([vp, vp, i32, i32, i32, vp, i32, vp, i64, vp], C.c_int),
        "atr_unpack_masked_ranks": ([vp, i32, vp, vp, i32, i32, vp, vp, i32, vp, i64, vp], C.c_int),
        "atr_render_simd_counters": ([vp, P(atr_camera), vp, i32, C.c_uint64, i32, vp], C.c_int),
        "atr_render_path_counters": ([vp, P(atr_camera), vp, i32, C.c_uint64, i32, vp], C.c_int),
        "atr_render_cell_costs": ([vp, P(atr_camera), C.c_uint64, i32, vp], C.c_int),
        "atr_render_wait": ([vp, u32, P(i32)], C.c_int),
        "atr_render_start_progressive": ([vp, P(atr_camera), vp, i32, P(atr_frame), C.c_uint64, vp, i32, i32],
                                         C.c_int),
        "atr_write_bmp": ([vp, i32, i32, C.c_char_p, C.c_char_p, i32], C.c_int),
        "atr_render_start_frames": ([vp, P(atr_camera), vp, i32, P(atr_frame), i32, i64, C.c_uint64, vp, i32],
                                    C.c_int),
        "atr_render_start_cameras": ([vp, vp, i32, vp, i32, P(atr_frame), i64, C.c_uint64, vp, i32], C.c_int),
        "atr_last_kernel_ms": ([vp, P(C.c_float)], C.c_int),
        "atr_device_alloc": ([vp, C.c_size_t, P(vp)], C.c_int),
        "atr_device_free": ([vp, vp], C.c_int),
        "atr_memcpy_d2h": ([vp, vp, vp, C.c_size_t], C.c_int),
        "atr_memcpy_h2d": ([vp, vp, vp, C.c_size_t], C.c_int),
        "atr_memset_d": ([vp, vp, C.c_int, C.c_size_t], C.c_int),
    }
    for name in [n for n in DIAG_EXPORTS if not hasattr(L, n)]:
        del sig[name]
    for name, (args, res) in sig.items():
        f = getattr(L, name)
        f.argtypes = args
        f.restype = res
    global _sig
    _sig = sig
    _lib = L
    return L


_sig = None


def signatures():
    lib()
# ... 671 lines not shown
                                                 int(tiles_per_launch)), "progressive render start")

    def render_start_frames(self, cam, tiles, frame: atr_frame, nframes, frame_stride, seed, stream=None,
                            variant=ATR_KERNEL_AUTO):
        arr, n = tiles if isinstance(tiles, tuple) else tiles_array(tiles)
        check(lib().atr_render_start_frames(self.h, C.byref(cam), C.cast(arr, C.c_void_p), n, C.byref(frame),
                                            int(nframes), int(frame_stride), C.c_uint64(seed & (2**64 - 1)),
                                            C.c_void_p(stream) if stream else None, int(variant)),
              "render start frames")

    def render_start_cameras(self, cams, tiles, frame: atr_frame, frame_stride, seed, stream=None,
                             variant=ATR_KERNEL_AUTO):
        arr, n = tiles if isinstance(tiles, tuple) else tiles_array(tiles)
        ca = (atr_camera * len(cams))(*cams)
        check(lib().atr_render_start_cameras(self.h, C.cast(ca, C.c_void_p), len(cams), C.cast(arr, C.c_void_p), n,
                                             C.byref(frame), int(frame_stride), C.c_uint64(seed & (2**64 - 1)),
                                             C.c_void_p(stream) if stream else None, int(variant)),
              "render start cameras")

    def counters(self, cam, tiles, seed, variant=ATR_KERNEL_AUTO):
        arr, n = tiles if isinstance(tiles, tuple) else tiles_array(tiles)
        out = (C.c_int64 * 10)()
        check(lib().atr_render_counters(self.h, C.byref(cam), C.cast(arr, C.c_void_p), n,
                                        C.c_uint64(seed & (2**64 - 1)), int(variant), out), "counters")
        keys = ["n_rays", "n_box", "n_tri", "n_leaf", "wave_tri_iters", "passes", "box_all", "waves",
                "cluster_boxes", "screened"]
        return dict(zip(keys, [int(x) for x in out]))

    def cull_counters(self, cam, tiles, seed, variant=ATR_KERNEL_AUTO):
        arr, n = tiles if isinstance(tiles, tuple) else tiles_array(tiles)
        out = (C.c_int64 * 5)()
        check(lib().atr_render_cull_counters(self.h, C.byref(cam), C.cast(arr, C.c_void_p), n,
                                             C.c_uint64(seed & (2**64 - 1)), int(variant), out), "cull counters")
        return dict(zip(["culled", "lane_private_iters", "dealt_rounds", "dealt_items", "cluster_tests"], [int(x) for x in out]))

    def fold_counters(self, cam, tiles, seed, variant=ATR_KERNEL_AUTO):
        arr, n = tiles if isinstance(tiles, tuple) else tiles_array(tiles)
        out = (C.c_int64 * 2)()
        check(lib().atr_render_fold_counters(self.h, C.byref(cam), C.cast(arr, C.c_void_p), n,
                                             C.c_uint64(seed & (2**64 - 1)), int(variant), out), "fold counters")
        return {"loose_passes_removed": int(out[0]), "screened_removed": int(out[1])}

    def camera_pads_row(self, eye):
        e = (C.c_float * 3)(*[float(x) for x in eye])
        n = int(lib().atr_camera_pads_row(self.h, e, None, None, None, 0))
        check(min(n, 0), "camera pads row")
        row, boxes = np.zeros((n, 4), np.float32), np.zeros((n, 12), np.float32)
        edges = np.zeros((n, 16, 6), np.float32)
        if n:
            check(min(int(lib().atr_camera_pads_row(self.h, e, row.ctypes.data, boxes.ctypes.data,
                                                    edges.ctypes.data, n)), 0), "camera pads row")
        return row, boxes, edges

    def tile_costs(self, cam, tiles, seed):
        arr, n = tiles if isinstance(tiles, tuple) else tiles_array(tiles)
        out = np.zeros(max(1, n), np.int64)
        check(lib().atr_render_tile_costs(self.h, C.byref(cam), C.cast(arr, C.c_void_p), n,
                                          C.c_uint64(seed & (2**64 - 1)), out.ctypes.data), "tile costs")
        return out[:n]

    def wave_trace(self, cam, tiles, seed, variant=0):
        arr, n = tiles if isinstance(tiles, tuple) else tiles_array(tiles)
        nb = C.c_int64()
        args = (self.h, C.byref(cam), C.cast(arr, C.c_void_p), n, C.c_uint64(seed & (2**64 - 1)), int(variant))
        check(lib().atr_render_wave_trace(*args, None, 0, C.byref(nb)), "wave trace")
        out = np.zeros((max(1, nb.value), 3), np.uint64)
        check(lib().atr_render_wave_trace(*args, out.ctypes.data, out.size, C.byref(nb)), "wave trace")
        return out[:nb.value]

    def wait(self, timeout_ms=0xFFFFFFFF):
        done = C.c_int32()
        rc = check(lib().atr_render_wait(self.h, int(timeout_ms), C.byref(done)), "render wait")
        return rc, done.value

    def last_kernel_ms(self):
        ms = C.c_float()
        check(lib().atr_last_kernel_ms(self.h, C.byref(ms)))
        return ms.value

    def unpack(self, tiles, width, packed_ptr, image_ptr, stream=None):
        arr, n = tiles if isinstance(tiles, tuple) else tiles_array(tiles)
        check(lib().atr_unpack(self.h, C.cast(arr, C.c_void_p), n, int(width), C.c_void_p(packed_ptr),
                               C.c_void_p(image_ptr), C.c_void_p(stream) if stream else None), "unpack")

    def tile_ray_casts(self, tiles, width, casts_ptr, out_ptr, stream=None):
        arr, n = tiles if isinstance(tiles, tuple) else tiles_array(tiles)
        check(lib().atr_tile_ray_casts(self.h, C.cast(arr, C.c_void_p), n, int(width),
                                       C.c_void_p(casts_ptr), C.c_void_p(out_ptr),
                                       C.c_void_p(stream) if stream else None), "tile casts")

    def packed_tile_ray_casts(self, tiles, width, height, casts_ptr, nframes, frame_stride, out_ptr, stream=None):
        arr, n = tiles if isinstance(tiles, tuple) else tiles_array(tiles)
        check(lib().atr_packed_tile_ray_casts(self.h, C.cast(arr, C.c_void_p), n, int(width), int(height),
                                              C.c_void_p(casts_ptr), int(nframes), int(frame_stride),
                                              C.c_void_p(out_ptr), C.c_void_p(stream) if stream else None),
              "packed tile casts")

    def set_cell_plan(self, width, height, plan=None):
        if plan is None:
            check(lib().atr_set_cell_plan(self.h, int(width), int(height), None), "cell plan")
            return
        plan = np.ascontiguousarray(plan, np.uint8)
        assert plan.size == ((width + 7) // 8) * ((height + 7) // 8)
        check(lib().atr_set_cell_plan(self.h, int(width), int(height), plan.ctypes.data), "cell plan")

    def phase_clocks(self, cam, tiles, seed, variant=ATR_KERNEL_AUTO):
# ... 122 lines not shown
```

include/atray.h:

```cpp
#ifndef ATRAY_H
#define ATRAY_H
#include <stddef.h>
#include <stdint.h>

#ifdef __cplusplus
extern "C" {
#endif

#define ATR_ABI_VERSION 2

enum {
    ATR_OK = 0,
    ATR_E_INVALID = -1,
    ATR_E_IO = -2,
    ATR_E_NOMEM = -3,
    ATR_E_NOSCENE = -4,
    ATR_E_TREE_DEPTH = -5,
    ATR_E_TREE_LAYOUT = -6,
    ATR_E_HIP = -1000
};

typedef struct { float x, y, z; } atr_vec3;

typedef struct { atr_vec3 emission, reflection; float scatter; } atr_material;
// ... 86 lines not shown
                     int32_t nspheres, const atr_plane* planes, int32_t nplanes);
int atr_scene_info(atr_ctx* ctx, int64_t* device_bytes, int32_t* max_nodes, int32_t* max_depth);
int atr_workspace_info(atr_ctx* ctx, int32_t* workspaces, int64_t* device_bytes);

enum { ATR_LAYOUT_IMAGE = 0, ATR_LAYOUT_PACKED = 1 };

typedef struct {
    int32_t layout;
    uint32_t* framebuffer;
    uint32_t* hit_face;
    float* hit_t;
    float* rgb;
    uint32_t* ray_casts;
    unsigned long long* traced_rays;
} atr_frame;

enum { ATR_KERNEL_AUTO = 0,
       ATR_KERNEL_LANE = 1 ,
       ATR_KERNEL_FLAT = 8 ,
       ATR_KERNEL_HYBRID = 9 ,
       ATR_KERNEL_PATHS = 10  };

int atr_render_start(atr_ctx* ctx, const atr_camera* cam, const atr_tile* tiles, int32_t ntiles,
                     const atr_frame* frame, uint64_t seed, void* stream);
int atr_render_start_progressive(atr_ctx* ctx, const atr_camera* cam, const atr_tile* tiles, int32_t ntiles,
                                 const atr_frame* frame, uint64_t seed, void* stream, int32_t variant,
                                 int32_t tiles_per_launch);
int atr_render_start_ex(atr_ctx* ctx, const atr_camera* cam, const atr_tile* tiles, int32_t ntiles,
                        const atr_frame* frame, uint64_t seed, void* stream, int32_t variant);
int atr_render_start_samples(atr_ctx* ctx, const atr_camera* cam, const atr_tile* tiles, int32_t ntiles,
                             const atr_frame* frame, uint64_t seed, void* stream, int32_t variant,
                             uint32_t first_sample, float* sample_sum);
#define ATR_SAMPLES_CONVERGED 0x80000000u
int atr_render_start_adaptive(atr_ctx* ctx, const atr_camera* cam, const atr_tile* tiles, int32_t ntiles,
                              const atr_frame* frame, uint64_t seed, void* stream, int32_t variant,
                              uint32_t first_sample, float* sample_sum, uint32_t* sample_count,
                              float tolerance);
int atr_render_adaptive_info(atr_ctx* ctx, int64_t info_out[4]);
int atr_render_start_frames(atr_ctx* ctx, const atr_camera* cam, const atr_tile* tiles, int32_t ntiles,
                            const atr_frame* frame, int32_t nframes, int64_t frame_stride, uint64_t seed,
                            void* stream, int32_t variant);
int atr_render_start_cameras(atr_ctx* ctx, const atr_camera* cams, int32_t nframes, const atr_tile* tiles,
                             int32_t ntiles, const atr_frame* frame, int64_t frame_stride, uint64_t seed,
                             void* stream, int32_t variant);
int atr_render_tile_costs(atr_ctx* ctx, const atr_camera* cam, const atr_tile* tiles, int32_t ntiles,
                          uint64_t seed, int64_t* cost_out);
int atr_render_counters(atr_ctx* ctx, const atr_camera* cam, const atr_tile* tiles, int32_t ntiles,
                        uint64_t seed, int32_t variant, int64_t counters_out[10]);
int atr_render_cull_counters(atr_ctx* ctx, const atr_camera* cam, const atr_tile* tiles, int32_t ntiles,
                             uint64_t seed, int32_t variant, int64_t counters_out[5]);
int atr_render_fold_counters(atr_ctx* ctx, const atr_camera* cam, const atr_tile* tiles, int32_t ntiles,
                             uint64_t seed, int32_t variant, int64_t counters_out[2]);
int64_t atr_camera_pads_row(atr_ctx* ctx, const float eye[3], float* row, float* boxes, float* edges, int64_t cap);
int64_t atr_render_packed_size(const atr_tile* tiles, int32_t ntiles);
int64_t atr_packed_pixel_map(const atr_tile* tiles, int32_t ntiles, int32_t width, int32_t height,
                             int64_t* out, int64_t cap);
int atr_unpack(atr_ctx* ctx, const atr_tile* tiles, int32_t ntiles, int32_t width,
               const uint32_t* packed, uint32_t* image, void* stream);
int atr_tile_ray_casts(atr_ctx* ctx, const atr_tile* tiles, int32_t ntiles, int32_t width,
                       const uint32_t* ray_casts_image, int64_t* out, void* stream);
int atr_packed_tile_ray_casts(atr_ctx* ctx, const atr_tile* tiles, int32_t ntiles, int32_t width,
                              int32_t height, const uint32_t* packed_ray_casts, int32_t nframes,
                              int64_t frame_stride, int64_t* out, void* stream);
int atr_pack_bgr(atr_ctx* ctx, const uint32_t* framebuffer, int64_t npixels, uint8_t* out, void* stream);
int atr_scatter_bgr(atr_ctx* ctx, const uint8_t* packed, int64_t npixels, const int64_t* dst_index, uint32_t* image,
                    void* stream);
int64_t atr_pack_bgr_masked_bound(int64_t npixels);
int atr_pack_bgr_masked(atr_ctx* ctx, const uint32_t* framebuffer, int64_t npixels, uint32_t background, uint8_t* out,
                        int64_t* nbytes, void* stream);
int atr_scatter_bgr_masked(atr_ctx* ctx, const uint8_t* packed, int64_t npixels, const int64_t* dst_index,
                           uint32_t* image, void* stream);
int atr_unpack_masked(atr_ctx* ctx, const atr_tile* tiles, int32_t ntiles, int32_t width, int32_t height,
                      const uint8_t* packed, int32_t nframes, uint32_t* image, int64_t image_stride, void* stream);
int atr_unpack_masked_ranks(atr_ctx* ctx, int32_t nsrc, const atr_tile* const* tiles, const int32_t* ntiles,
                            int32_t width, int32_t height, const uint8_t* const* packed, const int32_t* raw,
                            int32_t nframes, uint32_t* image, int64_t image_stride, void* stream);
#define ATR_PLAN_CLASS(c) ((uint8_t)(((c) & 7) << 4))
enum { ATR_PLAN_PRIO = 0x80 };
int atr_set_cell_plan(atr_ctx* ctx, int32_t width, int32_t height, const uint8_t* plan);
int atr_render_plan_info(atr_ctx* ctx, const atr_tile* tiles, int32_t ntiles, int32_t width, int32_t height,
                         int32_t* base_out, uint32_t* mask_hi_lo_out, int64_t cap, uint64_t* cost_out,
                         int64_t* nplanned);
int atr_render_cell_costs(atr_ctx* ctx, const atr_camera* cam, uint64_t seed, int32_t variant,
                          int64_t* out);
enum { ATR_RAY_SKY = 0, ATR_RAY_TRI = 1, ATR_RAY_SPHERE = 2, ATR_RAY_PLANE = 3, ATR_RAY_INVALID = 4 };
typedef struct {
    float* t;
    uint32_t* face;
    int32_t* model;
    float* uv;
    int32_t* kind;
    int32_t* material;
    float* normal;
    unsigned long long* traced_rays;
} atr_ray_hits;
int atr_trace_rays(atr_ctx* ctx, const float* origins, const float* directions, int64_t nrays,
                   const atr_ray_hits* hits, int32_t variant, int32_t sort_bits, void* stream);

enum { ATR_OCCL_VISIBLE = 0, ATR_OCCL_OCCLUDED = 1, ATR_OCCL_INVALID = 2 };
int atr_occluded_rays(atr_ctx* ctx, const float* origins, const float* directions, const float* t_max,
                      int64_t nrays, uint8_t* occluded, unsigned long long* traced_rays,
                      int32_t variant, int32_t sort_bits, void* stream);

typedef struct {
    uint32_t* visible;
    uint32_t* occluded;
// ... 83 lines not shown
```

Baseline: 10630.

## Add per-camera conservative leaf boxes to cull BVH leaves before candidate insertion

Measured after the change: 11510 (median of 6 runs). 1.08x the previous value.

```diff
diff --git a/atray_amd/csrc/capi.cpp b/atray_amd/csrc/capi.cpp
--- a/atray_amd/csrc/capi.cpp
+++ b/atray_amd/csrc/capi.cpp
@@ -188,6 +188,8 @@
     float scene_box[6] = {0.f, 0.f, 0.f, 1.f, 1.f, 1.f};
     atr_tuning tune = default_tuning();
     int64_t nclusters = 0;
+    int64_t nleaves = 0;
+    std::vector<uint32_t> leaf_clusters;
     std::vector<uint8_t> cplan;
     int32_t cplan_w = 0, cplan_h = 0;
     uint32_t cplan_gen = 0;
@@ -231,6 +233,7 @@
         uint64_t gen = 0;
         int32_t rows = 0;
         bool wide = false;
+        size_t lbox_off = 0;
         float eye[kMaxFrameCams][3];
         hipEvent_t built = nullptr;
         hipStream_t built_on = nullptr;
@@ -244,6 +247,7 @@
     bool camera_pads = true;
     bool facing_fold = true;
     bool wave_cull = true;
+    bool leaf_box = true;
     struct QueryWS {
         DevBuf rays, bins;
         int64_t cap = 0, nbins = 0;
@@ -789,13 +793,18 @@
     *used = nullptr;
     P.pads = nullptr;
     P.pads_stride = 0;
+    P.lbox = nullptr;
+    P.lbox_stride = 0;
     if (!c->camera_pads || c->nclusters <= 0 || c->nclusters > int64_t(1) << 30 || !atr_render_reads_pads(P, sched))
         return hipSuccess;
     const int32_t rows = P.nfcam > 0 ? P.nfcam : 1;
     if (rows > kMaxFrameCams) return hipSuccess;
     const int32_t stride = int32_t(c->nclusters);
     const bool wide = P.counters != nullptr;
-    const size_t bytes = size_t(rows) * size_t(stride) * sizeof(float2_t) * (wide ? 2 : 1);
+    const size_t pbytes = size_t(rows) * size_t(stride) * sizeof(float2_t) * (wide ? 2 : 1);
+    const bool boxes = c->leaf_box && c->nleaves > 0 && c->nleaves <= int64_t(1) << 30;
+    const size_t lbox_off = boxes ? (pbytes + 31) / 32 * 32 : 0;
+    const size_t bytes = boxes ? lbox_off + size_t(rows) * size_t(c->nleaves) * 2 * sizeof(float4_t) : pbytes;
     if (bytes > atr_ctx::kPadMaxBytes) return hipSuccess;
     PadEyes eyes;
     std::memset(&eyes, 0, sizeof(eyes));
@@ -841,16 +850,26 @@
         if ((e = atr_launch_camera_pads(c->d_scene, eyes, rows, stride, c->facing_fold, wide, static_cast<float2_t*>(sl->mem.p),
                                         nullptr, nullptr, nullptr, s)) != hipSuccess)
             return e;
+        if (boxes && (e = atr_launch_camera_leaf_boxes(c->d_scene, eyes, rows, stride, wide, static_cast<const float2_t*>(sl->mem.p),
+                                                       int32_t(c->nleaves),
+                                                       reinterpret_cast<float4_t*>(static_cast<char*>(sl->mem.p) + lbox_off),
+                                                       s)) != hipSuccess)
+            return e;
         if ((e = hipEventRecord(sl->built, s)) != hipSuccess) return e;
         sl->built_on = s;
         sl->gen = c->scene_gen;
         sl->rows = rows;
         sl->wide = wide;
+        sl->lbox_off = lbox_off;
         std::memcpy(sl->eye, eyes.e, sizeof(eyes.e));
     }
     sl->last_use = ++c->pad_clock;
     P.pads = static_cast<const float2_t*>(sl->mem.p);
     P.pads_stride = stride;
+    if (sl->lbox_off) {
+        P.lbox = reinterpret_cast<const float4_t*>(static_cast<const char*>(sl->mem.p) + sl->lbox_off);
+        P.lbox_stride = int32_t(c->nleaves);
+    }
     *used = sl;
     return hipSuccess;
 }
@@ -1150,6 +1169,7 @@
     if (const char* v = std::getenv("ATR_CAMERA_PADS")) c->camera_pads = !(v[0] == '0' && v[1] == '\0');
     if (const char* v = std::getenv("ATR_WAVE_CULL")) c->wave_cull = !(v[0] == '0' && v[1] == '\0');
     if (const char* v = std::getenv("ATR_FACING_FOLD")) c->facing_fold = !(v[0] == '0' && v[1] == '\0');
+    if (const char* v = std::getenv("ATR_LEAF_BOX")) c->leaf_box = !(v[0] == '0' && v[1] == '\0');
     const int rc = [&]() -> int {
         HIPCHK(hipStreamCreateWithFlags(&c->own_stream, hipStreamNonBlocking));
         HIPCHK(hipEventCreate(&c->ev_start));
@@ -1299,6 +1319,8 @@
     c->max_depth = 0;
     c->max_inner = 0;
     c->nclusters = 0;
+    c->nleaves = 0;
+    c->leaf_clusters.clear();
     float box[6] = {INFINITY, INFINITY, INFINITY, -INFINITY, -INFINITY, -INFINITY};
     for (int32_t i = 0; i < nmodels; ++i)
         for (const V3& v : models[i].mesh->m.vertices) {
@@ -1355,6 +1377,14 @@
             if (c->nclusters + int64_t(PT.nclusters) > int64_t(UINT32_MAX)) return ATR_E_INVALID;
             dm.cl_base = uint32_t(c->nclusters);
             dm.cl_count = uint32_t(PT.nclusters);
+            if (c->nleaves + int64_t(PT.nleaves) > int64_t(UINT32_MAX)) return ATR_E_INVALID;
+            dm.lf_base = uint32_t(c->nleaves);
+            dm.lf_count = uint32_t(PT.nleaves);
+            for (size_t k = 0; k < PT.nleaves; ++k) {
+                c->leaf_clusters.push_back(dm.cl_base + PT.cl_range[2 * k]);
+                c->leaf_clusters.push_back(PT.cl_range[2 * k + 1]);
+            }
+            c->nleaves += int64_t(PT.nleaves);
             c->nclusters += int64_t(PT.nclusters);
             if ((rc = up(PT.nodes, dm.nodes)) || (rc = up(PT.leaf_range, dm.leaf_range))) return rc;
             if (PT.tris.empty()) PT.tris.resize(1);
@@ -2111,7 +2141,7 @@
 
 #endif
 
-constexpr int kCounterSlots = 32;
+constexpr int kCounterSlots = 34;
 static int count_launch(atr_ctx* c, const atr_camera* cam, const atr_tile* tiles, int32_t ntiles, uint64_t seed,
                         int32_t variant, unsigned long long h[kCounterSlots]) {
     if (!c || !cam || ntiles < 0 || (ntiles && !tiles)) return ATR_E_INVALID;
@@ -2178,6 +2208,43 @@
     out[0] = int64_t(h[30]);
     out[1] = int64_t(h[31]);
     return ATR_OK;
+} ATR_ABI_CATCH
+
+int atr_render_leaf_box_counters(atr_ctx* c, const atr_camera* cam, const atr_tile* tiles, int32_t ntiles,
+                                 uint64_t seed, int32_t variant, int64_t out[2]) try {
+    if (!out) return ATR_E_INVALID;
+    unsigned long long h[kCounterSlots];
+    const int rc = count_launch(c, cam, tiles, ntiles, seed, variant, h);
+    if (rc != ATR_OK) return rc;
+    out[0] = int64_t(h[32]);
+    out[1] = int64_t(h[33]);
+    return ATR_OK;
+} ATR_ABI_CATCH
+
+int64_t atr_camera_leaf_boxes_row(atr_ctx* c, const float eye[3], float* row, int32_t* ranges, int64_t cap) try {
+    if (!c || !eye || cap < 0) return ATR_E_INVALID;
+    if (!c->d_scene) return ATR_E_NOSCENE;
+    const int64_t n = c->nleaves, ncl = c->nclusters;
+    if (n <= 0 || ncl <= 0) return 0;
+    if (n > int64_t(1) << 30 || ncl > int64_t(1) << 30) return ATR_E_INVALID;
+    if (!row || cap < n) return n;
+    HIPCHK(hipSetDevice(c->device));
+    PadEyes eyes;
+    std::memset(&eyes, 0, sizeof(eyes));
+    eyes.e[0][0] = eye[0], eyes.e[0][1] = eye[1], eyes.e[0][2] = eye[2];
+    DevTmp d_tab, d_box;
+    HIPCHK(hipMalloc(&d_tab.p, size_t(ncl) * sizeof(float2_t)));
+    HIPCHK(hipMalloc(&d_box.p, size_t(n) * 2 * sizeof(float4_t)));
+    HIPCHK(hipMemset(d_tab.p, 0, size_t(ncl) * sizeof(float2_t)));
+    HIPCHK(hipMemset(d_box.p, 0, size_t(n) * 2 * sizeof(float4_t)));
+    HIPCHK(atr_launch_camera_pads(c->d_scene, eyes, 1, int32_t(ncl), c->facing_fold, 0, static_cast<float2_t*>(d_tab.p),
+                                  nullptr, nullptr, nullptr, nullptr));
+    HIPCHK(atr_launch_camera_leaf_boxes(c->d_scene, eyes, 1, int32_t(ncl), 0, static_cast<const float2_t*>(d_tab.p),
+                                        int32_t(n), static_cast<float4_t*>(d_box.p), nullptr));
+    HIPCHK(hipDeviceSynchronize());
+    HIPCHK(hipMemcpy(row, d_box.p, size_t(n) * 2 * sizeof(float4_t), hipMemcpyDeviceToHost));
+    if (ranges) std::memcpy(ranges, c->leaf_clusters.data(), size_t(n) * 2 * sizeof(uint32_t));
+    return n;
 } ATR_ABI_CATCH
 
 int64_t atr_camera_pads_row(atr_ctx* c, const float eye[3], float* row, float* boxes, float* edges, int64_t cap) try {
diff --git a/atray_amd/csrc/cluster.h b/atray_amd/csrc/cluster.h
--- a/atray_amd/csrc/cluster.h
+++ b/atray_amd/csrc/cluster.h
@@ -155,6 +155,51 @@
     return !cull || !(fmaxf(fmaxf(gx, gy), gz) < __builtin_inff());
 }
 
+
+__device__ __forceinline__ float f32_below(float x) {
+    const uint32_t u = __float_as_uint(x);
+    if (x > 0.f) return __uint_as_float(u - 1u);
+    if (x < 0.f) return __uint_as_float(u + 1u);
+    return x == 0.f ? __uint_as_float(0x80000001u) : x;
+}
+__device__ __forceinline__ float f32_above(float x) { return -f32_below(-x); }
+
+struct LeafBox {
+    float lo[3], hi[3];
+    bool bad;
+};
+__device__ __forceinline__ void leaf_box_init(LeafBox& b) {
+#pragma unroll
+    for (int a = 0; a < 3; ++a) { b.lo[a] = __builtin_inff(); b.hi[a] = -__builtin_inff(); }
+    b.bad = false;
+}
+__device__ __forceinline__ void leaf_box_add(LeafBox& b, V3 eye, float4_t lo, float4_t hi, float gl) {
+    constexpr float inf = __builtin_inff();
+    const float l[3] = {lo.x, lo.y, lo.z}, h[3] = {hi.x, hi.y, hi.z}, e[3] = {eye.x, eye.y, eye.z};
+    const float g = gl * 1.0009765625f;
+#pragma unroll
+    for (int a = 0; a < 3; ++a) {
+        const float F = fmaxf(fabsf(l[a] - e[a]), fabsf(h[a] - e[a]));
+        const float slack = g + 9.5367432e-7f * F;
+        const float x0 = f32_below(l[a] - slack), x1 = f32_above(h[a] + slack);
+        if (!(slack < inf) || !(fabsf(x0) < inf) || !(fabsf(x1) < inf)) b.bad = true;
+        b.lo[a] = fminf(b.lo[a], x0);
+        b.hi[a] = fmaxf(b.hi[a], x1);
+    }
+}
+__device__ __forceinline__ void leaf_box_entry(const LeafBox& b, uint32_t n, V3 eye, float4_t& e0, float4_t& e1) {
+    constexpr float inf = __builtin_inff();
+    const float e[3] = {eye.x, eye.y, eye.z};
+    bool bad = b.bad;
+#pragma unroll
+    for (int a = 0; a < 3; ++a)
+        if (!(fabsf(b.lo[a] - e[a]) < inf) || !(fabsf(b.hi[a] - e[a]) < inf)) bad = true;
+    const uint32_t flag = n == 0 ? kLeafBoxEmpty : bad ? kLeafBoxKeep : kLeafBoxTest;
+    const bool box = flag == kLeafBoxTest;
+    e0 = float4_t{box ? b.lo[0] : 0.f, box ? b.lo[1] : 0.f, box ? b.lo[2] : 0.f, __uint_as_float(flag)};
+    e1 = float4_t{box ? b.hi[0] : 0.f, box ? b.hi[1] : 0.f, box ? b.hi[2] : 0.f, 0.f};
+}
+
 #ifndef ATR_SCREEN_TWO_CMP
 __device__ __forceinline__ void screen_band(float blo, float ahi, float& mid, float& half) {
     const float lo = fmaxf(blo, -1600.0f), hi = fminf(ahi, 1600.0f);
@@ -199,7 +244,8 @@
 
 template <bool COUNT, bool EARLY = true, bool PADS = false>
 __device__ __forceinline__ uint32_t cluster_cands(const Ray& r, const DModel& m, uint32_t c, float4_t lo, float4_t hi,
-                                                  float best, Ctr& ct, const float2_t* pads = nullptr) {
+                                                  float best, Ctr& ct, const float2_t* pads = nullptr,
+                                                  [[maybe_unused]] bool wskip = false) {
     float2_t g;
     if constexpr (PADS) g = pads[pads_entry<COUNT>(c)];
     Ray rr = r;
@@ -220,6 +266,7 @@
     if constexpr (PADS && COUNT) {
         float fl, fh;
         if (!cluster_pads(r, sr, lo, hi, gfold, best, fl, fh)) { ct.fold_box += 1; ct.fold_screen += n; }
+        else if (wskip) ct.lb_unsound += 1;
     }
     const uint32_t slots = (2u << (n - 1)) - 1u;
     const float q = hi.w;
diff --git a/atray_amd/csrc/engine.h b/atray_amd/csrc/engine.h
--- a/atray_amd/csrc/engine.h
+++ b/atray_amd/csrc/engine.h
@@ -109,6 +109,7 @@
     int32_t material;
     float aabb[6];
     uint32_t cl_base, cl_count;
+    uint32_t lf_base, lf_count;
 };
 
 struct DMaterial { float ex, ey, ez, rx, ry, rz, scatter, pad; };
@@ -165,6 +166,8 @@
     const float2_t* pads;
     int32_t pads_stride;
     int32_t wave_cull;
+    const float4_t* lbox;
+    int32_t lbox_stride;
 };
 
 struct PadEyes {
diff --git a/atray_amd/csrc/host_scene.cpp b/atray_amd/csrc/host_scene.cpp
--- a/atray_amd/csrc/host_scene.cpp
+++ b/atray_amd/csrc/host_scene.cpp
@@ -488,6 +488,7 @@
         return out;
     };
     P.leaf_range = by_rank(range);
+    for (int32_t n = 0; n < T.nnodes; ++n) P.nleaves = std::max(P.nleaves, size_t(leaf_rank[size_t(n)] + 1));
     P.tris.resize(nprims);
     for (size_t k = 0; k < nprims; ++k) P.tris[k] = make_tri(&T.prim_vertices[9 * k], T.prim_face[k]);
     const size_t np = nprims ? nprims : 1;
diff --git a/atray_amd/csrc/host_scene.h b/atray_amd/csrc/host_scene.h
--- a/atray_amd/csrc/host_scene.h
+++ b/atray_amd/csrc/host_scene.h
@@ -48,6 +48,7 @@
     size_t nclusters = 0;
     std::vector<uint32_t> clus;
     std::vector<uint32_t> cl_range;
+    size_t nleaves = 0;
     std::vector<float4_t> prim;
     int32_t max_depth = 0;
     bool near_ok = false;
diff --git a/atray_amd/csrc/launch.h b/atray_amd/csrc/launch.h
--- a/atray_amd/csrc/launch.h
+++ b/atray_amd/csrc/launch.h
@@ -11,6 +11,9 @@
 hipError_t atr_launch_camera_pads(const atr::DScene* scene, const atr::PadEyes& eyes, int32_t nrows, int32_t stride,
                                   int fold, int wide, atr::float2_t* table, atr::float2_t* info, atr::float4_t* boxes,
                                   float* edges, hipStream_t s);
+hipError_t atr_launch_camera_leaf_boxes(const atr::DScene* scene, const atr::PadEyes& eyes, int32_t nrows, int32_t stride,
+                                        int wide, const atr::float2_t* pads, int32_t lstride, atr::float4_t* lbox,
+                                        hipStream_t s);
 hipError_t atr_launch_traced_finish(unsigned long long* slots, unsigned long long* out, hipStream_t s);
 hipError_t atr_launch_unpack(const atr::DBlock* blocks, int32_t nblocks, int32_t width, const uint32_t* packed,
                              uint32_t* image, hipStream_t s);
diff --git a/atray_amd/csrc/render.hip b/atray_amd/csrc/render.hip
--- a/atray_amd/csrc/render.hip
+++ b/atray_amd/csrc/render.hip
@@ -137,8 +137,10 @@
         if constexpr (PADS) {
             const int32_t row = P.nfcam > 0 ? __builtin_amdgcn_readfirstlane(fidx) : 0;
             const float2_t* pads = uniform_global(P.pads) + pads_entry<COUNT>(size_t(int64_t(row) * P.pads_stride));
+            const float4_t* lbox = uniform_global(P.lbox);
+            if (lbox) lbox += 2 * size_t(int64_t(row) * P.lbox_stride);
             intersect_scene<SCHED, FlavPrimaryPads, COUNT>(S, eye, dir, active, id, err, ct, P.hyb_a, P.hyb_b, pads,
-                                                           P.wave_cull);
+                                                           P.wave_cull, lbox);
         } else {
             intersect_scene<SCHED, FlavPrimary, COUNT>(S, eye, dir, active, id, err, ct, P.hyb_a, P.hyb_b, nullptr,
                                                        P.wave_cull);
@@ -264,6 +266,16 @@
 #pragma unroll
                 for (int off = 32; off > 0; off >>= 1) x2 += __shfl_xor(x2, off);
                 if (lane == 0 && x2) atomicAdd(C + 30 + k, (unsigned long long)x2);
+            }
+        }
+        if constexpr (PADS) {
+            uint32_t f[2] = {ct.lb_skip, ct.lb_unsound};
+#pragma unroll
+            for (int k = 0; k < 2; ++k) {
+                uint32_t x2 = f[k];
+#pragma unroll
+                for (int off = 32; off > 0; off >>= 1) x2 += __shfl_xor(x2, off);
+                if (lane == 0 && x2) atomicAdd(C + 32 + k, (unsigned long long)x2);
             }
         }
         if (lane == 0) {
@@ -378,6 +390,37 @@
     }
 }
 
+template <bool WIDE>
+__global__ __launch_bounds__(256) void camera_leaf_box_kernel(const DScene* __restrict__ S, PadEyes eyes,
+                                                              int32_t stride, const float2_t* __restrict__ pads,
+                                                              int32_t lstride, float4_t* __restrict__ lbox) {
+    const uint32_t x = blockIdx.x * 256u + threadIdx.x;
+    if (x >= uint32_t(lstride)) return;
+    const int32_t f = __builtin_amdgcn_readfirstlane(int32_t(blockIdx.y));
+    const V3 eye = mk(eyes.e[f][0], eyes.e[f][1], eyes.e[f][2]);
+    const int32_t nmodels = S->nmodels;
+    for (int32_t i = 0; i < nmodels; ++i) {
+        const DModel& m = S->models[i];
+        const uint32_t lf = x - m.lf_base;
+        if (!m.has_tree || lf >= m.lf_count) continue;
+        const uint2_t cr = load_range(m.cl_range, int32_t(lf));
+        LeafBox b;
+        leaf_box_init(b);
+        for (uint32_t k = 0; k < cr.y; ++k) {
+            const uint32_t c = cr.x + k;
+            const size_t e = size_t(f) * size_t(stride) + m.cl_base + c;
+            const float gl = WIDE ? pads[2 * e + 1].x : pads[e].x;
+            leaf_box_add(b, eye, m.clus[kClusterBlock * size_t(c)], m.clus[kClusterBlock * size_t(c) + 1], gl);
+        }
+        float4_t e0, e1;
+        leaf_box_entry(b, cr.y, eye, e0, e1);
+        const size_t o = 2 * (size_t(f) * size_t(lstride) + x);
+        lbox[o] = e0;
+        lbox[o + 1] = e1;
+        return;
+    }
+}
+
 __global__ __launch_bounds__(64) void traced_finish_kernel(unsigned long long* __restrict__ slots,
                                                           unsigned long long* __restrict__ out) {
     const int lane = threadIdx.x;
@@ -488,6 +531,18 @@
         if (wide) hipLaunchKernelGGL(camera_pads_kernel<true>, gp, dim3(256), 0, s, scene, eyes, stride, table);
         else hipLaunchKernelGGL(camera_pads_kernel<false>, gp, dim3(256), 0, s, scene, eyes, stride, table);
     }
+    return hipGetLastError();
+}
+
+extern "C" hipError_t atr_launch_camera_leaf_boxes(const atr::DScene* scene, const atr::PadEyes& eyes, int32_t nrows,
+                                                   int32_t stride, int wide, const atr::float2_t* pads, int32_t lstride,
+                                                   atr::float4_t* lbox, hipStream_t s) {
+    using namespace atr;
+    if (nrows <= 0 || lstride <= 0) return hipSuccess;
+    if (nrows > kMaxFrameCams || stride <= 0 || !pads || !lbox) return hipErrorInvalidValue;
+    const dim3 g(unsigned((lstride + 255) / 256), unsigned(nrows));
+    if (wide) hipLaunchKernelGGL(camera_leaf_box_kernel<true>, g, dim3(256), 0, s, scene, eyes, stride, pads, lstride, lbox);
+    else hipLaunchKernelGGL(camera_leaf_box_kernel<false>, g, dim3(256), 0, s, scene, eyes, stride, pads, lstride, lbox);
     return hipGetLastError();
 }
 
diff --git a/atray_amd/csrc/scan.h b/atray_amd/csrc/scan.h
--- a/atray_amd/csrc/scan.h
+++ b/atray_amd/csrc/scan.h
@@ -201,18 +201,18 @@
 #endif
 
 struct FlavCamera      { static constexpr bool HYB = true,  LDSB = true,  UO = true,  UT = true,  UV = true,
-                         NEAR = false, PADS = false, WCULL = false, SEED = false; static constexpr int EARLY = 2; };
+                         NEAR = false, PADS = false, WCULL = false, SEED = false, LBOX = false; static constexpr int EARLY = 2; };
 struct FlavPrimary     { static constexpr bool HYB = true,  LDSB = true,  UO = true,  UT = true,  UV = false,
-                         NEAR = false, PADS = false, WCULL = true,  SEED = false; static constexpr int EARLY = 1; };
+                         NEAR = false, PADS = false, WCULL = true,  SEED = false, LBOX = false; static constexpr int EARLY = 1; };
 struct FlavPrimaryPads { static constexpr bool HYB = true,  LDSB = true,  UO = true,  UT = true,  UV = false,
-                         NEAR = false, PADS = true,  WCULL = true,  SEED = false; static constexpr int EARLY = 8; };
+                         NEAR = false, PADS = true,  WCULL = true,  SEED = false, LBOX = true;  static constexpr int EARLY = 8; };
 struct FlavHybBounce   { static constexpr bool HYB = true,  LDSB = false, UO = false, UT = false, UV = true,
-                         NEAR = false, PADS = false, WCULL = false, SEED = false; static constexpr int EARLY = 4; };
+                         NEAR = false, PADS = false, WCULL = false, SEED = false, LBOX = false; static constexpr int EARLY = 4; };
 struct FlavBounce      { static constexpr bool HYB = ATR_BOUNCE_HYB != 0, LDSB = true, UO = false, UT = false,
-                         UV = true, NEAR = true, PADS = false, WCULL = false, SEED = false;
+                         UV = true, NEAR = true, PADS = false, WCULL = false, SEED = false, LBOX = false;
                          static constexpr int EARLY = 4; };
 struct FlavOcclusion   { static constexpr bool HYB = false, LDSB = true,  UO = false, UT = false, UV = false,
-                         NEAR = true,  PADS = false, WCULL = false, SEED = true;  static constexpr int EARLY = 1; };
+                         NEAR = true,  PADS = false, WCULL = false, SEED = true,  LBOX = false; static constexpr int EARLY = 1; };
 
 template <class F, bool COUNT, int K = kLeafBuf>
 __device__ __forceinline__ bool cand_test(const Ray& q, const DModel& m, int w, int32_t ow, uint32_t slot,
@@ -366,7 +366,9 @@
 }
 
 template <class F, bool COUNT, int K = kLeafBuf>
-__device__ __forceinline__ void flat_pass(const Ray& r, const DModel& m, int w, int ln, FlatQ& q, int& err, Ctr& ct) {
+__device__ __forceinline__ void flat_pass(const Ray& r, const DModel& m, int w, int ln, FlatQ& q, int& err, Ctr& ct,
+                                          const float4_t* lbox = nullptr) {
+    static_assert(!F::LBOX || (F::UT && F::PADS), "the boxes are sized by the table's growths; uniform leaf ranks");
     FlatLds<K, F::UV>& L = flat_lds<K, F::UV>();
     const float bd = q.rewalk ? L.lbd[w][K - 1][ln] : -__builtin_inff();
     const int32_t bi = q.rewalk ? L.lbl[w][K - 1][ln] : -1;
@@ -381,7 +383,7 @@
             LdsLeafBuf<K> lb;
             lb.d = &L.lbd[w][0][ln];
             lb.leaf = &L.lbl[w][0][ln];
-            const int32_t n = traverse_pass_wave<K, COUNT>(r, m.inner, lb, bd, bi, ct, q.need);
+            const int32_t n = traverse_pass_wave<K, COUNT, F::LBOX>(r, m.inner, lb, bd, bi, ct, q.need, lbox);
             if (q.need) took(n);
         }
     } else if (q.need) {
@@ -405,7 +407,8 @@
 template <class F, bool COUNT, int K = kLeafBuf>
 __device__ __forceinline__ void flat_leaf_step(const Ray& r, const DModel& m, int w, int ln, bool live, FlatQ& q,
                                                Ctr& ct, int32_t hyb_a, int32_t hyb_b, const float2_t* pads = nullptr,
-                                               float hv = 0.f, unsigned long long start = kKeyInit) {
+                                               float hv = 0.f, unsigned long long start = kKeyInit,
+                                               const float4_t* lbox = nullptr) {
     static_assert(!F::PADS || F::UO, "the table holds one origin per camera");
     static_assert(!F::WCULL || (F::UO && K >= 2), "the hull is of one origin's directions; sv's LDS slot");
     constexpr bool UO = F::UO, PADS = F::PADS, WCULL = F::WCULL;
@@ -418,6 +421,14 @@
         cf = cr.x;
         cn = cr.y;
         if constexpr (COUNT) { ct.leaf += 1; ct.cbox += cn; }
+    }
+    [[maybe_unused]] bool wskip = false;
+    if constexpr (COUNT && F::LBOX) {
+        if (live && lbox && !m.root_leaf && isfinite(r.inv.x) && isfinite(r.inv.y) && isfinite(r.inv.z)) {
+            const size_t lf = size_t(uint32_t(L.lbl[w][q.j][ln]));
+            wskip = leaf_box_miss(r, lbox[2 * lf], lbox[2 * lf + 1]);
+            ct.lb_skip += wskip ? 1u : 0u;
+        }
     }
     [[maybe_unused]] uint32_t sv = 0xFFFFFFFFu;
     if constexpr (WCULL) {
@@ -486,7 +497,7 @@
                 if constexpr (COUNT && WCULL) ct.ctest += 1;
                 const float bound = __uint_as_float(uint32_t(L.key[w][ln] >> 32));
                 cm = cluster_cands<COUNT, kEarly, PADS>(r, m, c, m.clus[kClusterBlock * size_t(c)],
-                                                m.clus[kClusterBlock * size_t(c) + 1], bound, ct, pads);
+                                                m.clus[kClusterBlock * size_t(c) + 1], bound, ct, pads, wskip);
             }
             cand_rounds<F, COUNT, true, K>(r, m, w, ln, cm, kMaxClusterSize * (cf + ci), ln, ct);
         }
@@ -522,8 +533,10 @@
         if (valid) {
             if constexpr (COUNT && WCULL) ct.ctest += 1;
             const float bound = __uint_as_float(uint32_t(L.key[w][own] >> 32));
+            bool oskip = false;
+            if constexpr (COUNT && F::LBOX) oskip = __shfl(int(wskip), own) != 0;
             cm = cluster_cands<COUNT, kEarly, PADS>(qr, m, c, m.clus[kClusterBlock * size_t(c)],
-                                                    m.clus[kClusterBlock * size_t(c) + 1], bound, ct, pads);
+                                                    m.clus[kClusterBlock * size_t(c) + 1], bound, ct, pads, oskip);
         }
         cand_rounds<F, COUNT, false, K>(r, m, w, ln, cm, kMaxClusterSize * c, own, ct);
     }
@@ -562,7 +575,8 @@
 template <class F, bool COUNT, int K = kLeafBuf>
 __device__ __forceinline__ void flat_query(const Ray& r, const DModel& m, bool active, int w, int ln, int& err, Ctr& ct,
                                            int32_t hyb_a = 0, int32_t hyb_b = 0, const float2_t* pads = nullptr,
-                                           int32_t wcull = 0, unsigned long long start = kKeyInit) {
+                                           int32_t wcull = 0, unsigned long long start = kKeyInit,
+                                           const float4_t* lbox = nullptr) {
     FlatQ q = flat_begin<F, COUNT, K>(r, m, active, w, ln, ct, start);
     [[maybe_unused]] float hv = __builtin_nanf("");
     if constexpr (F::WCULL) {
@@ -570,10 +584,10 @@
     }
     for (;;) {
         ATR_PCLK(uint64_t tc0 = 0; if constexpr (!F::SEED) tc0 = clock64());
-        flat_pass<F, COUNT, K>(r, m, w, ln, q, err, ct);
+        flat_pass<F, COUNT, K>(r, m, w, ln, q, err, ct, lbox);
         ATR_PCLK(if constexpr (!F::SEED) ct.t_pass += uint32_t(clock64() - tc0));
         if (__ballot(!q.done) == 0) break;
-        flat_leaf_step<F, COUNT, K>(r, m, w, ln, !q.done, q, ct, hyb_a, hyb_b, pads, hv, start);
+        flat_leaf_step<F, COUNT, K>(r, m, w, ln, !q.done, q, ct, hyb_a, hyb_b, pads, hv, start, lbox);
     }
 }
 
@@ -605,7 +619,8 @@
 template <int SCHED, class F, bool COUNT, int KB = kLeafBuf>
 __device__ __forceinline__ SceneHit intersect_models(const DScene* __restrict__ S, V3 o, V3 d, bool active, int& err,
                                                     Ctr& ct, int32_t hyb_a, int32_t hyb_b,
-                                                    const float2_t* pads = nullptr, int32_t wcull = 0) {
+                                                    const float2_t* pads = nullptr, int32_t wcull = 0,
+                                                    const float4_t* lbox = nullptr) {
     const Ray r = make_ray(o, d);
     SceneHit sh{kMaxFloat, 0.f, 0.f, 0u, -1};
     const int32_t nmodels = __builtin_amdgcn_readfirstlane(S->nmodels);
@@ -619,9 +634,11 @@
             } else {
                 const float2_t* mp = pads;
                 if constexpr (F::PADS) mp = pads + pads_entry<COUNT>(__builtin_amdgcn_readfirstlane(m.cl_base));
+                const float4_t* ml = lbox;
+                if constexpr (F::LBOX) { if (lbox) ml = lbox + 2 * size_t(__builtin_amdgcn_readfirstlane(m.lf_base)); }
                 const int w = threadIdx.x >> 6, ln = threadIdx.x & 63;
                 ATR_PCLK(uint64_t tcs = clock64());
-                flat_query<F, COUNT, KB>(r, m, active, w, ln, err, ct, hyb_a, hyb_b, mp, wcull);
+                flat_query<F, COUNT, KB>(r, m, active, w, ln, err, ct, hyb_a, hyb_b, mp, wcull, kKeyInit, ml);
                 flat_result<F, COUNT, KB>(m, active, w, ln, h);
                 ATR_PCLK(ct.t_scan += uint32_t(clock64() - tcs));
             }
@@ -646,8 +663,9 @@
 template <int SCHED, class F, bool COUNT>
 __device__ __forceinline__ void intersect_scene(const DScene* __restrict__ S, V3 o, V3 d, bool active, Isect& id,
                                                 int& err, Ctr& ct, int32_t hyb_a, int32_t hyb_b,
-                                                const float2_t* pads = nullptr, int32_t wcull = 0) {
-    const SceneHit sh = intersect_models<SCHED, F, COUNT>(S, o, d, active, err, ct, hyb_a, hyb_b, pads, wcull);
+                                                const float2_t* pads = nullptr, int32_t wcull = 0,
+                                                const float4_t* lbox = nullptr) {
+    const SceneHit sh = intersect_models<SCHED, F, COUNT>(S, o, d, active, err, ct, hyb_a, hyb_b, pads, wcull, lbox);
     if (!active) return;
     scene_finish(S, o, d, sh.best, sh.face, sh.fu, sh.fv, sh.nm, id);
 }
diff --git a/atray_amd/csrc/trace.h b/atray_amd/csrc/trace.h
--- a/atray_amd/csrc/trace.h
+++ b/atray_amd/csrc/trace.h
@@ -11,6 +11,7 @@
     uint32_t cand_wave = 0, node_wave = 0, node_lane = 0, round_wave = 0, round_items = 0;
     uint32_t culled = 0, lp_wave = 0, ctest = 0;
     uint32_t fold_box = 0, fold_screen = 0;
+    uint32_t lb_skip = 0, lb_unsound = 0;
 };
 
 __device__ __forceinline__ uint32_t first_active_lane() {
@@ -305,10 +306,32 @@
     return n;
 }
 
-template <int K, bool COUNT, class LB>
+constexpr uint32_t kLeafBoxTest = 0u, kLeafBoxEmpty = 1u, kLeafBoxKeep = 2u;
+
+__device__ __forceinline__ bool leaf_box_miss(const Ray& r, float4_t e0, float4_t e1) {
+    const uint32_t flag = __float_as_uint(e0.w);
+    if (flag != kLeafBoxTest) return flag == kLeafBoxEmpty;
+    const float x0 = (e0.x - r.o.x) * r.inv.x, x1 = (e1.x - r.o.x) * r.inv.x;
+    const float y0 = (e0.y - r.o.y) * r.inv.y, y1 = (e1.y - r.o.y) * r.inv.y;
+    const float z0 = (e0.z - r.o.z) * r.inv.z, z1 = (e1.z - r.o.z) * r.inv.z;
+    const float tn = fmaxf(fmaxf(fminf(x0, x1), fminf(y0, y1)), fminf(z0, z1));
+    const float tf = fminf(fminf(fmaxf(x0, x1), fmaxf(y0, y1)), fmaxf(z0, z1));
+    return tn > tf || tf < 0.f;
+}
+
+typedef float f32x8_t __attribute__((ext_vector_type(8)));
+__device__ __forceinline__ void load_leaf_box_uniform(const float4_t* p, float4_t& e0, float4_t& e1) {
+    using C = const __attribute__((address_space(4))) f32x8_t;
+    const f32x8_t v = *reinterpret_cast<C*>(reinterpret_cast<uint64_t>(p));
+    e0 = float4_t{v[0], v[1], v[2], v[3]};
+    e1 = float4_t{v[4], v[5], v[6], v[7]};
+}
+
+template <int K, bool COUNT, bool LBOX = false, class LB>
 __device__ __forceinline__ uint32_t examine_inner(const Ray& r, const Inner& n, LB& lb,
                                                   int32_t& ncand, float bd, int32_t bi, Ctr& ct,
-                                                  bool first_pass, bool cull = false) {
+                                                  bool first_pass, bool cull = false,
+                                                  const float4_t* lbox = nullptr) {
     const float X0 = (n.lx - r.o.x) * r.inv.x, X1 = (n.vx - r.o.x) * r.inv.x, X2 = (n.hx - r.o.x) * r.inv.x;
     const float Y0 = (n.ly - r.o.y) * r.inv.y, Y1 = (n.vy - r.o.y) * r.inv.y, Y2 = (n.hy - r.o.y) * r.inv.y;
     const float Z0 = (n.lz - r.o.z) * r.inv.z, Z1 = (n.vz - r.o.z) * r.inv.z, Z2 = (n.hz - r.o.z) * r.inv.z;
@@ -343,6 +366,13 @@
                 ++nodes_hit;
                 const int32_t id = n.leaf0 + __popc(n.bm & ((1u << i) - 1u) & 0xFFu);
                 if (dis > bd || (dis == bd && id > bi)) {
+                    if constexpr (LBOX && !COUNT) {
+                        if (lbox && cull) {
+                            float4_t e0, e1;
+                            load_leaf_box_uniform(lbox + 2 * size_t(uint32_t(id)), e0, e1);
+                            if (leaf_box_miss(r, e0, e1)) continue;
+                        }
+                    }
                     ++ncand;
                     lb_insert<K>(lb, dis, id);
                 }
@@ -502,9 +532,10 @@
     return skipped && ncand <= K ? K + 1 : ncand;
 }
 
-template <int K, bool COUNT, class LB>
+template <int K, bool COUNT, bool LBOX = false, class LB>
 __device__ __forceinline__ int32_t traverse_pass_wave(const Ray& r, const float4_t* __restrict__ tab, LB& lb,
-                                                      float bd, int32_t bi, Ctr& ct, bool part) {
+                                                      float bd, int32_t bi, Ctr& ct, bool part,
+                                                      const float4_t* lbox = nullptr) {
     const bool first_pass = bi < 0;
     if constexpr (COUNT) { if (part) ct.pass += 1; }
     if (part) lb_clear<K>(lb);
@@ -515,7 +546,8 @@
     const bool cull = isfinite(r.inv.x) && isfinite(r.inv.y) && isfinite(r.inv.z);
 #endif
     Inner cur = load_inner_uniform(tab, 0);
-    uint64_t lo = part ? uint64_t(examine_inner<K, COUNT>(r, cur, lb, ncand, bd, bi, ct, first_pass, cull)) : 0;
+    uint64_t lo = 0;
+    if (part) lo = examine_inner<K, COUNT, LBOX>(r, cur, lb, ncand, bd, bi, ct, first_pass, cull, lbox);
     uint64_t hi = 0;
     uint32_t bm = cur.bm;
     int32_t parent = -1, lvl = 0;
@@ -532,7 +564,8 @@
             const uint32_t innerm = ~bm & ((1u << s) - 1u);
             const int32_t id = int32_t(bm >> 8) + __popc(innerm);
             cur = load_inner_uniform(tab, id);
-            const uint64_t cm = act ? uint64_t(examine_inner<K, COUNT>(r, cur, lb, ncand, bd, bi, ct, first_pass, cull)) : 0;
+            uint64_t cm = 0;
+            if (act) cm = examine_inner<K, COUNT, LBOX>(r, cur, lb, ncand, bd, bi, ct, first_pass, cull, lbox);
             ++lvl;
             if (lvl >= kMaskLevels) return -1;
             if (lvl < 8) lo |= cm << (8 * lvl);
diff --git a/atray_amd/engine.py b/atray_amd/engine.py
--- a/atray_amd/engine.py
+++ b/atray_amd/engine.py
@@ -148,6 +148,7 @@
     "atr_trace_rays", "atr_occluded_rays", "atr_gather_occlusion", "atr_gather_directions",
     "atr_radiance_rays", "atr_gather_radiance", "atr_mesh_texels", "atr_texels_to_image",
     "atr_render_fold_counters", "atr_camera_pads_row", "atr_default_denoise_params", "atr_denoise",
+    "atr_render_leaf_box_counters", "atr_camera_leaf_boxes_row",
 ]
 DIAG_EXPORTS = ["atr_render_wave_trace", "atr_render_phase_clocks", "atr_render_path_counters",
                 "atr_render_simd_counters"]
@@ -217,6 +218,8 @@
         "atr_render_cull_counters": ([vp, P(atr_camera), vp, i32, C.c_uint64, i32, i64 * 5], C.c_int),
         "atr_render_fold_counters": ([vp, P(atr_camera), vp, i32, C.c_uint64, i32, i64 * 2], C.c_int),
         "atr_camera_pads_row": ([vp, C.c_float * 3, vp, vp, vp, i64], i64),
+        "atr_render_leaf_box_counters": ([vp, P(atr_camera), vp, i32, C.c_uint64, i32, i64 * 2], C.c_int),
+        "atr_camera_leaf_boxes_row": ([vp, C.c_float * 3, vp, vp, i64], i64),
         "atr_render_tile_costs": ([vp, P(atr_camera), vp, i32, C.c_uint64, vp], C.c_int),
         "atr_render_wave_trace": ([vp, P(atr_camera), vp, i32, C.c_uint64, i32, vp, i64, P(i64)], C.c_int),
         "atr_packed_pixel_map": ([vp, i32, i32, i32, vp, i64], i64),
@@ -994,6 +997,23 @@
                                                     edges.ctypes.data, n)), 0), "camera pads row")
         return row, boxes, edges
 
+    def leaf_box_counters(self, cam, tiles, seed, variant=ATR_KERNEL_AUTO):
+        arr, n = tiles if isinstance(tiles, tuple) else tiles_array(tiles)
+        out = (C.c_int64 * 2)()
+        check(lib().atr_render_leaf_box_counters(self.h, C.byref(cam), C.cast(arr, C.c_void_p), n,
+                                                 C.c_uint64(seed & (2**64 - 1)), int(variant), out), "leaf box counters")
+        return {"skipped_visits": int(out[0]), "unsound_skips": int(out[1])}
+
+    def camera_leaf_boxes_row(self, eye):
+        e = (C.c_float * 3)(*[float(x) for x in eye])
+        n = int(lib().atr_camera_leaf_boxes_row(self.h, e, None, None, 0))
+        check(min(n, 0), "camera leaf boxes row")
+        row, ranges = np.zeros((n, 8), np.float32), np.zeros((n, 2), np.int32)
+        if n:
+            check(min(int(lib().atr_camera_leaf_boxes_row(self.h, e, row.ctypes.data, ranges.ctypes.data, n)), 0),
+                  "camera leaf boxes row")
+        return row[:, 0:3].copy(), row[:, 4:7].copy(), row[:, 3].copy().view(np.uint32), ranges
+
     def tile_costs(self, cam, tiles, seed):
         arr, n = tiles if isinstance(tiles, tuple) else tiles_array(tiles)
         out = np.zeros(max(1, n), np.int64)
diff --git a/include/atray.h b/include/atray.h
--- a/include/atray.h
+++ b/include/atray.h
@@ -162,6 +162,9 @@
 int atr_render_fold_counters(atr_ctx* ctx, const atr_camera* cam, const atr_tile* tiles, int32_t ntiles,
                              uint64_t seed, int32_t variant, int64_t counters_out[2]);
 int64_t atr_camera_pads_row(atr_ctx* ctx, const float eye[3], float* row, float* boxes, float* edges, int64_t cap);
+int atr_render_leaf_box_counters(atr_ctx* ctx, const atr_camera* cam, const atr_tile* tiles, int32_t ntiles,
+                                 uint64_t seed, int32_t variant, int64_t counters_out[2]);
+int64_t atr_camera_leaf_boxes_row(atr_ctx* ctx, const float eye[3], float* row, int32_t* ranges, int64_t cap);
 int64_t atr_render_packed_size(const atr_tile* tiles, int32_t ntiles);
 int64_t atr_packed_pixel_map(const atr_tile* tiles, int32_t ntiles, int32_t width, int32_t height,
                              int64_t* out, int64_t cap);
```
